# DanielBrosch/SDPSymmetryReduction.jl

Hardware: AMD Instinct MI355X
Metric: N x N SDP reductions/sec (admissible_subspace+blockDiagonalize) at N=4096 (higher is better)
Workload: dtype int8 square (int32 acc) + f64 eigen

## Files before the change

### include/sdpsr.h

```cpp
#ifndef SDPSR_H
#define SDPSR_H

#include <stddef.h>
#include <stdint.h>

#ifdef __cplusplus
extern "C" {
#endif

#define SDPSR_VERSION_MAJOR 0
#define SDPSR_VERSION_MINOR 5

typedef struct sdpsr_ctx sdpsr_ctx;
typedef struct sdpsr_problem sdpsr_problem;

typedef enum sdpsr_status {
    SDPSR_OK = 0,
    SDPSR_INVALID_DECOMPOSITION_FIELD = 1,
    SDPSR_NUMERICAL_INCONSISTENCY = 2,
    SDPSR_DIMENSION_MISMATCH = 3,
    SDPSR_LABEL_OVERFLOW = 4,
    SDPSR_BAD_ARGUMENT = 5,
    SDPSR_HIP_ERROR = 6,
    SDPSR_SOLVER_ERROR = 7,
    SDPSR_OUT_OF_MEMORY = 8,
    SDPSR_NOT_CONVERGED = 9,
    SDPSR_BAD_STATE = 10
} sdpsr_status;

typedef enum sdpsr_mem { SDPSR_MEM_HOST = 0, SDPSR_MEM_DEVICE = 1 } sdpsr_mem;

typedef enum sdpsr_square_mode {
    SDPSR_SQUARE_AUTO = 0,
    SDPSR_SQUARE_I8 = 1,
    SDPSR_SQUARE_F32 = 2,
    SDPSR_SQUARE_F64 = 3
} sdpsr_square_mode;

typedef enum sdpsr_round_mode {
    SDPSR_ROUND_NEAREST = 0,
    SDPSR_ROUND_TRUNC = 1
} sdpsr_round_mode;

enum {
    SDPSR_FLAG_SEPARATE_REFINEMENTS = 1u << 0,
    SDPSR_FLAG_FRESH_IRREDUCIBLE_ELEMENT = 1u << 1,
    SDPSR_FLAG_ALWAYS_REORTHOGONALIZE = 1u << 2,
    SDPSR_FLAG_REFINE_NO_FUSE = 1u << 3,
    SDPSR_FLAG_UNPACK_EVERY_STEP = 1u << 4,
    SDPSR_FLAG_SPMM_ONE_BY_ONE = 1u << 5,
    SDPSR_FLAG_SINGLE_COUPLING_ELEMENT = 1u << 6,
    SDPSR_FLAG_SMALL_EIGEN_ON_DEVICE = 1u << 7,
    SDPSR_FLAG_NO_GRAPH = 1u << 8,
    SDPSR_FLAG_NO_VERIFY_SHORTCUT = 1u << 9,
    SDPSR_FLAG_FULL_BASIS_IMAGE = 1u << 10,
    SDPSR_FLAG_ALWAYS_PROJECT = 1u << 11,
    SDPSR_FLAG_SYTRD_PANELS = 1u << 12,
    SDPSR_FLAG_COUPLING_ON_HOST = 1u << 13,
    SDPSR_FLAG_SYTRD_ONE_LAUNCH = 1u << 14,
    SDPSR_FLAG_WAIT_FOR_EVERY_VERDICT = 1u << 15,
    SDPSR_FLAG_WIDE_LOOP_LABELS = 1u << 16,
    SDPSR_FLAG_MODULE_SCRATCH_FILLS = 1u << 17,
    SDPSR_FLAG_SQUARE_EVERY_VERDICT = 1u << 18
};

typedef struct sdpsr_opts {
    uint32_t struct_size;
    int32_t square_mode;
    int32_t channels;
    int32_t max_iters;
    int32_t confirm_rounds;
    int32_t eig_driver;
    uint32_t flags;
    int32_t round_mode;
    int32_t basis_image_kernel;
    int32_t refine_path;
    int32_t label_bits;
    int32_t insert_wgs_per_cu;
    int32_t square_kernel;
    int32_t reserved[3];
} sdpsr_opts;

enum {
    SDPSR_T_TOTAL = 0,
    SDPSR_T_PROJECT = 1,
    SDPSR_T_SQUARE = 2,
    SDPSR_T_REFINE = 3,
    SDPSR_T_EIGEN = 4,
    SDPSR_T_ISO = 5,
    SDPSR_T_IRRED = 6,
    SDPSR_T_IMAGE = 7,
    SDPSR_T_COUNT = 8
};

int sdpsr_create(int device_id, uint64_t seed, const sdpsr_opts* opts, sdpsr_ctx** out);
void sdpsr_destroy(sdpsr_ctx* ctx);
const char* sdpsr_last_error(const sdpsr_ctx* ctx);
const char* sdpsr_status_string(int status);
int sdpsr_version(void);
int sdpsr_set_stream(sdpsr_ctx* ctx, void* hip_stream);
int sdpsr_synchronize(sdpsr_ctx* ctx);
int sdpsr_wait_stream(sdpsr_ctx* ctx, void* hip_stream);
int sdpsr_hint_symmetric_basis(sdpsr_ctx* ctx, int yes);
int sdpsr_set_seed(sdpsr_ctx* ctx, uint64_t seed);
int sdpsr_dimension_trajectory(sdpsr_ctx* ctx, int64_t* dims, int32_t capacity, int32_t* count);

int sdpsr_set_label_width(sdpsr_ctx* ctx, int bits);
int sdpsr_label_width(sdpsr_ctx* ctx);
int sdpsr_labels_convert(sdpsr_ctx* ctx, int64_t len, const void* in, int in_bits, void* out, int out_bits, int mem);

int sdpsr_partition_from_f64(sdpsr_ctx* ctx, int64_t len, const double* M,
                             uint32_t* labels, int64_t* nparts, int mem);
int sdpsr_partition_from_u32(sdpsr_ctx* ctx, int64_t len, const uint32_t* in,
                             uint32_t* labels, int64_t* nparts, int mem);
int sdpsr_partition_from_u64(sdpsr_ctx* ctx, int64_t len, const uint64_t* in,
                             uint32_t* labels, int64_t* nparts, int mem);
int sdpsr_refine(sdpsr_ctx* ctx, int64_t len, uint32_t* p1, int64_t* d1,
                 const uint32_t* p2, int64_t d2, int mem);
int sdpsr_partition_checksum(sdpsr_ctx* ctx, int64_t len, const uint32_t* labels, uint64_t* out, int mem);
int sdpsr_fill(sdpsr_ctx* ctx, int64_t len, const uint32_t* labels, const double* values,
               int64_t d, double* M, int mem);
int sdpsr_randomize(sdpsr_ctx* ctx, int64_t len, const uint32_t* labels, double* M, int mem);
int sdpsr_clamp_round(sdpsr_ctx* ctx, int64_t len, double* a, double atol, int mem);
int sdpsr_project_out(sdpsr_ctx* ctx, int64_t len, double* x, const double* U, int64_t r,
                      int mem);

int sdpsr_square_f64(sdpsr_ctx* ctx, int64_t n, const double* X, double* X2, int mem);
int sdpsr_square_f32(sdpsr_ctx* ctx, int64_t n, const float* X, float* X2, int mem);
int sdpsr_square_i8(sdpsr_ctx* ctx, int64_t n, const int8_t* X, int32_t* X2, int mem);
int sdpsr_square_i8_symmetric(sdpsr_ctx* ctx, int64_t n, int64_t batch, const int8_t* X, int32_t* X2, int mem);
int sdpsr_gemm_tn_f64(sdpsr_ctx* ctx, int64_t m, int64_t n, int64_t k, const double* A,
                      int64_t lda, const double* B, int64_t ldb, double* C, int64_t ldc,
                      int mem);

int sdpsr_admissible_subspace(sdpsr_ctx* ctx, int64_t n, const double* CL, const double* X0L,
                              const double* U, int64_t r, double atol, uint32_t* P_out,
                              int64_t* dim_out, int32_t* iters_out, double* phase_ms, int mem);
int sdpsr_admissible_subspace_dense(sdpsr_ctx* ctx, int64_t n, int64_t m, const double* C,
                                    const double* A, const double* b, double atol,
                                    uint32_t* P_out, int64_t* dim_out, int32_t* iters_out,
                                    double* phase_ms, int mem_out);

typedef enum sdpsr_setup_path {
    SDPSR_SETUP_NO_CONSTRAINTS = 0,
    SDPSR_SETUP_CHOLESKY_QR2 = 1,
    SDPSR_SETUP_MGS = 2
} sdpsr_setup_path;
int sdpsr_admissible_setup_csr(sdpsr_ctx* ctx, int64_t n, int64_t m, const int64_t* rowptr, const int64_t* colind,
                               const double* val, int index_base, const double* b, const double* C, double atol,
                               double* CL, double* X0L, double* U, int64_t* r_out, int* hint_out, int32_t* info_out,
                               int mem_out);
int sdpsr_admissible_subspace_csr(sdpsr_ctx* ctx, int64_t n, int64_t m, const int64_t* rowptr, const int64_t* colind,
                                  const double* val, int index_base, const double* b, const double* C, double atol,
                                  uint32_t* P_out, int64_t* dim_out, int32_t* iters_out, double* phase_ms, int mem_out);

int sdpsr_desymmetrize(sdpsr_ctx* ctx, int64_t n, uint32_t* P, int64_t* dim, int32_t* iters, int mem);

int sdpsr_reduce_constraints(sdpsr_ctx* ctx, int64_t len, const uint32_t* labels, int64_t d, int64_t m,
                             const double* A, double* out, int mem);
int sdpsr_reduce_constraints_csr(sdpsr_ctx* ctx, int64_t len, const uint32_t* labels, int64_t d, int64_t m,
                                 const int64_t* rowptr, const int64_t* colind, const double* val, int index_base,
                                 double* out, int mem);

typedef struct sdpsr_sparse sdpsr_sparse;
int sdpsr_sparse_create(sdpsr_ctx* ctx, int64_t len, int64_t m, int64_t nnz, const int64_t* rowptr, const int64_t* colind,
                        const double* val, int index_base, int mem, sdpsr_sparse** out);
int sdpsr_sparse_destroy(sdpsr_sparse* A);
int sdpsr_sparse_info(const sdpsr_sparse* A, int64_t* len, int64_t* m, int64_t* nnz_canonical, int* rows_symmetric);
int sdpsr_sparse_export(sdpsr_ctx* ctx, const sdpsr_sparse* A, int index_base, int64_t* rowptr, int64_t* colind, double* val,
                        int mem);
int sdpsr_admissible_setup_sparse(sdpsr_ctx* ctx, int64_t n, const sdpsr_sparse* A, const double* b, const double* C,
                                  double atol, double* CL, double* X0L, double* U, int64_t* r_out, int* hint_out,
                                  int32_t* info_out, int mem_out);
int sdpsr_admissible_subspace_sparse(sdpsr_ctx* ctx, int64_t n, const sdpsr_sparse* A, const double* b, const double* C,
                                     double atol, uint32_t* P_out, int64_t* dim_out, int32_t* iters_out, double* phase_ms,
                                     int mem_out);
int sdpsr_reduce_constraints_sparse(sdpsr_ctx* ctx, const sdpsr_sparse* A, const uint32_t* labels, int64_t d, double* out,
                                    int mem);

int sdpsr_compress_constraints(sdpsr_ctx* ctx, int64_t m, int64_t d, const double* newA, const double* b, double rtol,
                               double droptol, double* out, int64_t* rank_out, double* sv, int64_t* nnz_out,
                               int32_t* passes_out, int mem);

int sdpsr_block_diagonalize(sdpsr_ctx* ctx, int64_t n, const uint32_t* P, int64_t d,
                            double epsilon, int32_t* nblocks, int64_t* sum_sq, int64_t* sum_s,
                            double* phase_ms, int mem);
int sdpsr_block_sizes(sdpsr_ctx* ctx, int32_t* blk_sizes);
int sdpsr_q_hat(sdpsr_ctx* ctx, double* Q_hat, int mem);
int sdpsr_block_images(sdpsr_ctx* ctx, double* blks, double* Q_hat, double* phase_ms, int mem);
enum {
    SDPSR_BI_ROUTE_COMMUTATIVE = 1,
    SDPSR_BI_ROUTE_BLOCKS = 2,
    SDPSR_BI_ROUTE_TWO_STAGE = 3,
    SDPSR_BI_ROUTE_OUTER = 4,
    SDPSR_BI_ROUTE_CHUNK = 5,
    SDPSR_BI_ROUTE_REPAIRED = 0x100,
    SDPSR_BI_ROUTE_SHORTCUT_REFUSED = 0x200
};
int sdpsr_basis_image(sdpsr_ctx* ctx, int64_t n, const uint32_t* P, int64_t d, int32_t nblocks, const int32_t* blk_sizes,
                      const double* Q_hat, int64_t class_first, int64_t class_count, double atol, double* blks, int32_t* route,
                      double* phase_ms, int mem);
int sdpsr_jordan_reduce(sdpsr_ctx* ctx, int64_t n, const double* CL, const double* X0L, const double* U, int64_t r,
                        double atol, double epsilon, uint32_t* P_out, int64_t* dim_out, int32_t* iters_out,
                        int32_t* nblocks, int64_t* sum_sq, int64_t* sum_s, double* blks, int64_t blks_capacity,
                        double* Q_hat, int64_t qhat_capacity, double* phase_ms, int mem);

int sdpsr_jordan_reduce_batch(sdpsr_ctx* ctx, int32_t R, const uint64_t* seeds, int64_t n, const double* CL, const double* X0L,
                              const double* U, int64_t r, double atol, double epsilon, uint32_t* const* P_out, int64_t* dim_out,
                              int32_t* iters_out, int32_t* nblocks, int64_t* sum_sq, int64_t* sum_s, double* const* blks,
                              const int64_t* blks_capacity, int32_t* status, int mem);
int sdpsr_batch_block_sizes(sdpsr_ctx* ctx, int32_t restart, int32_t* blk_sizes);

int sdpsr_problem_create(sdpsr_ctx* ctx, int64_t n, const double* CL, const double* X0L, const double* U, int64_t r, int hint,
                         int mem, sdpsr_problem** out);
int sdpsr_problem_destroy(sdpsr_problem* problem);
int sdpsr_problem_reduce(sdpsr_ctx* ctx, const sdpsr_problem* problem, double atol, double epsilon, uint32_t* P_out,
// ... 64 lines not shown
```

### include/sdpsr_prof.h

```cpp
#ifndef SDPSR_PROF_H
#define SDPSR_PROF_H

#include "sdpsr.h"

#ifdef __cplusplus
extern "C" {
#endif

int sdpsr_profile_kernel(sdpsr_ctx* ctx, int kind, int64_t n, int64_t aux, int reps,
                         double* ms_per_launch);
int sdpsr_profile_clock(sdpsr_ctx* ctx, int kind, int64_t n, int64_t aux, int reps, double* out);
int sdpsr_profile_host_waits(sdpsr_ctx* ctx, uint64_t* out);
int sdpsr_profile_loop_counts(sdpsr_ctx* ctx, int32_t restart, uint64_t* out);
int sdpsr_profile_band_chase(sdpsr_ctx* ctx, int64_t n, int b, const double* A_host, double* d_host, double* e_host, double* out);
int sdpsr_profile_band_reduce(sdpsr_ctx* ctx, int64_t n, int b, double* A_host, double* out);
int sdpsr_profile_sytrd_graphs(sdpsr_ctx* ctx, double* out);
int sdpsr_profile_gather_packed(sdpsr_ctx* ctx, int64_t n, int T, int64_t d, uint64_t key, const uint32_t* Lp_host, const uint32_t* Lfull_host,
                                int8_t* X_plain, int8_t* X_writing, int8_t* X_full, uint32_t* L_inout, int64_t guard);
int sdpsr_profile_verify(sdpsr_ctx* ctx, int64_t n, int T, int64_t d, int mode, const uint32_t* Lp_host, const uint32_t* first_idx_host,
                         const int32_t* C_host, const double* U_host, double coef, uint64_t key, double atol, uint32_t* out);
int sdpsr_profile_basis_constant(sdpsr_ctx* ctx, int64_t n, int r, int64_t d, const uint32_t* Lp_host, const uint32_t* first_idx_host,
                                 const double* U_host, double atol, uint32_t* out);
int sdpsr_profile_verify_pair(sdpsr_ctx* ctx, int64_t n, int64_t d, const uint32_t* Lp_host, const uint32_t* first_idx_host,
                              const double* a_host, const double* b_host, uint32_t* out);
int sdpsr_profile_initial_guess(sdpsr_ctx* ctx, int32_t restart, uint64_t* out);
int sdpsr_profile_narrow_labels(sdpsr_ctx* ctx, int32_t restart, uint64_t* out);
int sdpsr_profile_gather_packed_w(sdpsr_ctx* ctx, int64_t n, int T, int64_t d, uint64_t key, int width, const uint32_t* Lp_host, int8_t* X_plain,
                                  int8_t* X_writing, uint32_t* L_inout, int64_t guard);
int sdpsr_profile_verify_w(sdpsr_ctx* ctx, int64_t n, int T, int64_t d, int r, int width, const uint32_t* Lp_host, const uint32_t* first_idx_host,
                           const int32_t* C_host, const double* U_host, const double* coef_host, uint64_t key, double atol, uint32_t* out);
int sdpsr_profile_verify_pair_w(sdpsr_ctx* ctx, int64_t n, int64_t d, int width, const uint32_t* Lp_host, const uint32_t* first_idx_host,
                                const double* a_host, const double* b_host, uint32_t* out);
int sdpsr_profile_proj_coef_lower(sdpsr_ctx* ctx, int64_t n, int64_t r, uint64_t key, int width, const uint32_t* Lp_host, const double* U_host,
                                  double* partial_out, double* coef_out);
int sdpsr_profile_refine_source(sdpsr_ctx* ctx, int kind, int what, int64_t n, int64_t ld, int T, int r, int packed, int lab_packed, uint64_t key,
                                double atol, const double* a_host, const double* b_host, const double* U_host, const double* coef_host,
                                const void* C_host, uint32_t* L_inout, uint32_t* Lnew_inout, int64_t guard, int64_t prev_classes, int sym,
                                uint64_t* sig_out, int64_t* nparts, uint32_t* first_out, int32_t* report);
int sdpsr_profile_square_checks(sdpsr_ctx* ctx, int32_t restart, uint64_t* out);
int sdpsr_profile_square_check(sdpsr_ctx* ctx, int64_t n, int64_t d, int G, int T, const uint64_t* keys, int width, int write_full,
                               const uint32_t* Lp_host, const uint32_t* first_idx_host, uint8_t* ws_inout, uint64_t* layout,
                               uint32_t* verdicts_out, uint32_t* L_inout, int64_t guard);


int sdpsr_profile_gram(sdpsr_ctx* ctx, int mode, int64_t k, int64_t ma, int64_t nb, int64_t lda, int64_t ldb, int64_t mp, int64_t np,
                       const double* A_host, const double* B_host, double* C_inout, double* pinned_inout, int64_t guard, int32_t* report);
int sdpsr_profile_tall_times_small(sdpsr_ctx* ctx, int64_t n, int64_t ldi, int64_t kk, int64_t lds, int64_t ncols, double alpha, double beta,
                                   int64_t ldo, const double* In_host, const double* S_host, double* out_inout, int64_t guard);
int sdpsr_profile_label_product(sdpsr_ctx* ctx, int64_t n, int64_t d, int G, int64_t w, int64_t ldw, int64_t ldy, const uint64_t* keys,
                                const uint32_t* L_host, const double* W_host, double* Y_inout, int64_t guard, int32_t* report);
int sdpsr_profile_label_product_pair(sdpsr_ctx* ctx, int64_t n, int64_t d, int64_t w, int64_t ldw, int64_t ldy, const uint64_t* keys,
                                     const uint32_t* L_host, const double* W_host, double* Y0_inout, double* Y1_inout, int64_t guard,
                                     int32_t* report);
int sdpsr_profile_class_sums2(sdpsr_ctx* ctx, int64_t n, int64_t d, uint32_t first, int plain, const uint32_t* L_host, const double* X_host,
                              double* Y_inout, int64_t guard, int32_t* report);
int sdpsr_profile_class_sums(sdpsr_ctx* ctx, int64_t n, int64_t d, int64_t ldo, const uint32_t* L_host, const double* x_host,
                             double* out_inout, int64_t guard, int32_t* report);
int sdpsr_profile_symmetrize(sdpsr_ctx* ctx, int64_t m, int64_t ld, double* B_inout, int64_t guard);
int sdpsr_profile_extract_symmetric(sdpsr_ctx* ctx, int64_t m, int64_t mp, int64_t lds, const double* src_host, double* dst_inout, int64_t guard);
int sdpsr_profile_normalize_columns(sdpsr_ctx* ctx, int64_t n, int64_t ldx, int64_t hstride, int64_t nruns, const double* X_host,
                                    double* H_inout, double* norm_inout, int64_t guard);
int sdpsr_profile_random_vector(sdpsr_ctx* ctx, int64_t n, uint64_t key, double* x_inout, int64_t guard);


int sdpsr_profile_poison_scratch(sdpsr_ctx* ctx);
int sdpsr_profile_stacked_in_place(sdpsr_ctx* ctx, int64_t n, int64_t ldi, int64_t kk, int64_t lds, int64_t ncols, int64_t w, int64_t mcols,
                                   double* M_inout, const double* S_host, int64_t guard, int32_t* report);
int sdpsr_profile_lift(sdpsr_ctx* ctx, int64_t n, int64_t ldi, int64_t kk, int64_t lds, int64_t S1, double atol, const double* In_host,
                       const double* S_host, double* Qcm_inout, double* Qrm_inout, int64_t guard);
int sdpsr_profile_seed_vector(sdpsr_ctx* ctx, int64_t n, uint64_t key, double* x_inout, double* h_inout, double* norm_inout, int64_t guard);
int sdpsr_profile_qrm_current(sdpsr_ctx* ctx, int32_t* current);


int sdpsr_profile_cx_gather_herm(sdpsr_ctx* ctx, int64_t n, const uint32_t* L_host, uint64_t key, double* Hr_inout, double* Hi_inout, int64_t guard);
int sdpsr_profile_cx_heev(sdpsr_ctx* ctx, int route, int64_t n, const double* Hr_host, const double* Hi_host, double atol, double* w_inout,
                          double* Vr_inout, double* Vi_inout, int64_t guard, int32_t* info_out);
int sdpsr_profile_cx_block_norms(sdpsr_ctx* ctx, int route, int64_t n, const double* Hr_host, const double* Hi_host, const double* Vr_host,
                                 const double* Vi_host, const int32_t* space_of, int32_t neig, double* norms_inout, int64_t guard);
int sdpsr_profile_cx_irreducible(sdpsr_ctx* ctx, int route, int64_t n, int64_t vcols, const double* Hr_host, const double* Hi_host,
                                 const double* Vr_host, const double* Vi_host, const int32_t* desc, int32_t ncols, double atol,
                                 double* Qhat_inout, int64_t guard);


int sdpsr_profile_dense_block_norms(sdpsr_ctx* ctx, int route, int64_t n, int64_t ld, const double* A_host, const double* Q_host,
                                    const int32_t* space_of, int32_t neig, double* norms_inout, double* M_inout, double* T_inout, int64_t guard);
int sdpsr_profile_dense_cluster_norms(sdpsr_ctx* ctx, int64_t n, int64_t ld, const double* A_host, const double* Q_host,
                                      const double* evals_host, double atol, const int32_t* einfo, void* pack_inout, double* T_inout, int64_t guard);
int sdpsr_profile_dense_classes(sdpsr_ctx* ctx, int32_t neig, double* norms_inout, const int32_t* dims_host, double atol, uint64_t* stat_out,
                                double* edges_out, double* thr_out, uint64_t* bits_inout, int32_t* kpart_out, int64_t guard);
int sdpsr_profile_dense_irreducible(sdpsr_ctx* ctx, int route, int64_t n, int64_t ldq, int64_t vcols, const double* Q_host, const double* Bf_host,
                                    int64_t nf, const int32_t* desc, int32_t npairs, double* Qhat_inout, int64_t ncols, int64_t guard,
                                    int32_t* report);
int sdpsr_profile_copy_cols(sdpsr_ctx* ctx, int64_t n, int64_t count, const int32_t* src_cols, const int32_t* dst_cols, const double* src_host,
                            int64_t ld_src, int64_t scols, double* dst_inout, int64_t ld_dst, int64_t dcols, int64_t guard);
int sdpsr_profile_clamptol(sdpsr_ctx* ctx, int64_t len, double* a_inout, double atol, int64_t guard);


int sdpsr_profile_sytrd(sdpsr_ctx* ctx, int64_t n, int64_t ld, double* A_inout, double* d_inout, double* e_inout, double* tau_inout,
                        int64_t guard);
int sdpsr_profile_backtransform(sdpsr_ctx* ctx, int64_t n, int64_t ld, const double* A_host, const double* tau_host, double* Z_inout,
                                int64_t guard);
int sdpsr_profile_stedc(sdpsr_ctx* ctx, int64_t n, int64_t ld, const double* d_host, const double* e_host, double* w_inout, double* Z_inout,
                        int64_t guard);

#ifdef __cplusplus
}
#endif
#endif
```

### sdpsymmetryreduction.jl_amd/_lib.py

```python
from __future__ import annotations

import ctypes as C
import os
import re

import numpy as np

_HERE = os.path.dirname(os.path.abspath(__file__))
LIB_PATH = os.path.join(_HERE, "libsdpsr_hip.so")
PROF_LIB_PATH = os.path.join(_HERE, "libsdpsr_prof.so")
HEADER_PATH = os.path.join(os.path.dirname(_HERE), "include", "sdpsr.h")
PROF_HEADER_PATH = os.path.join(os.path.dirname(_HERE), "include", "sdpsr_prof.h")

MEM_HOST, MEM_DEVICE = 0, 1
SQUARE_AUTO, SQUARE_I8, SQUARE_F32, SQUARE_F64 = 0, 1, 2, 3
T_TOTAL, T_PROJECT, T_SQUARE, T_REFINE, T_EIGEN, T_ISO, T_IRRED, T_IMAGE, T_COUNT = range(9)
ROUND_NEAREST, ROUND_TRUNC = 0, 1
SETUP_NO_CONSTRAINTS, SETUP_CHOLESKY_QR2, SETUP_MGS = 0, 1, 2
FLAG_SEPARATE_REFINEMENTS = 1 << 0
FLAG_FRESH_IRREDUCIBLE_ELEMENT = 1 << 1
FLAG_ALWAYS_REORTHOGONALIZE = 1 << 2
FLAG_REFINE_NO_FUSE = 1 << 3
FLAG_UNPACK_EVERY_STEP = 1 << 4
FLAG_SPMM_ONE_BY_ONE = 1 << 5
FLAG_SINGLE_COUPLING_ELEMENT = 1 << 6
FLAG_SMALL_EIGEN_ON_DEVICE = 1 << 7
FLAG_NO_GRAPH = 1 << 8
FLAG_NO_VERIFY_SHORTCUT = 1 << 9
FLAG_FULL_BASIS_IMAGE = 1 << 10
FLAG_ALWAYS_PROJECT = 1 << 11
FLAG_SYTRD_PANELS = 1 << 12
FLAG_COUPLING_ON_HOST = 1 << 13
FLAG_SYTRD_ONE_LAUNCH = 1 << 14
FLAG_WAIT_FOR_EVERY_VERDICT = 1 << 15
FLAG_WIDE_LOOP_LABELS = 1 << 16
FLAG_MODULE_SCRATCH_FILLS = 1 << 17
FLAG_SQUARE_EVERY_VERDICT = 1 << 18
BASIS_IMAGE_KERNELS = {"auto": 0, "two_stage": 1, "outer": 2, "chunk": 3}
BI_ROUTE_COMMUTATIVE, BI_ROUTE_BLOCKS, BI_ROUTE_TWO_STAGE, BI_ROUTE_OUTER, BI_ROUTE_CHUNK = 1, 2, 3, 4, 5
BI_ROUTE_REPAIRED, BI_ROUTE_SHORTCUT_REFUSED = 0x100, 0x200
TRI_UPPER, TRI_FULL = 0, 1
REFINE_PATHS = {"auto": 0, "hash": 1, "sort": 2, "bucket": 3, "no_mid": 4, "mid_no_first": 6}

LABEL_DTYPES = {8: np.dtype(np.uint8), 16: np.dtype(np.uint16), 32: np.dtype(np.uint32)}


def label_dtype(bits):
    try:
        return LABEL_DTYPES[int(bits)]
    except KeyError:
        raise ValueError(f"label width must be 8, 16 or 32, not {bits!r}") from None


STATUS = {
    0: "OK", 1: "INVALID_DECOMPOSITION_FIELD", 2: "NUMERICAL_INCONSISTENCY", 3: "DIMENSION_MISMATCH",
    4: "LABEL_OVERFLOW", 5: "BAD_ARGUMENT", 6: "HIP_ERROR", 7: "SOLVER_ERROR", 8: "OUT_OF_MEMORY",
    9: "NOT_CONVERGED", 10: "BAD_STATE",
}


class Opts(C.Structure):
    _fields_ = [
        ("struct_size", C.c_uint32),
        ("square_mode", C.c_int32),
        ("channels", C.c_int32),
        ("max_iters", C.c_int32),
        ("confirm_rounds", C.c_int32),
        ("eig_driver", C.c_int32),
        ("flags", C.c_uint32),
        ("round_mode", C.c_int32),
        ("basis_image_kernel", C.c_int32),
        ("refine_path", C.c_int32),
        ("label_bits", C.c_int32),
        ("insert_wgs_per_cu", C.c_int32),
        ("square_kernel", C.c_int32),
        ("reserved", C.c_int32 * 3),
    ]


def declared_symbols(header_path=HEADER_PATH):
    txt = open(header_path).read()
    txt = re.sub(r"/\*.*?\*/", "", txt, flags=re.S)
    return sorted(set(re.findall(r"\b(sdpsr_[a-z0-9_]+)\s*\(", txt)))


_lib = None


def load_library():
    global _lib
    if _lib is not None:
        return _lib
    if not os.path.exists(LIB_PATH):
        raise RuntimeError(
            f"{LIB_PATH} is missing: build it with `make -C sdpsymmetryreduction.jl_amd/csrc` "
            "(there is no CPU fallback for the HIP path)")
    try:
        import torch
    except ImportError:
        pass
    lib = C.CDLL(LIB_PATH)
    vp, i64, i32, dbl = C.c_void_p, C.c_int64, C.c_int32, C.c_double
    pi64, pi32 = C.POINTER(C.c_int64), C.POINTER(C.c_int32)
    sigs = {
        "sdpsr_create": (C.c_int, [C.c_int, C.c_uint64, C.POINTER(Opts), C.POINTER(vp)]),
        "sdpsr_destroy": (None, [vp]),
        "sdpsr_last_error": (C.c_char_p, [vp]),
        "sdpsr_status_string": (C.c_char_p, [C.c_int]),
        "sdpsr_version": (C.c_int, []),
        "sdpsr_set_stream": (C.c_int, [vp, vp]),
        "sdpsr_synchronize": (C.c_int, [vp]),
        "sdpsr_wait_stream": (C.c_int, [vp, vp]),
        "sdpsr_set_seed": (C.c_int, [vp, C.c_uint64]),
        "sdpsr_dimension_trajectory": (C.c_int, [vp, vp, i32, pi32]),
        "sdpsr_partition_from_f64": (C.c_int, [vp, i64, vp, vp, pi64, C.c_int]),
        "sdpsr_partition_from_u32": (C.c_int, [vp, i64, vp, vp, pi64, C.c_int]),
        "sdpsr_partition_from_u64": (C.c_int, [vp, i64, vp, vp, pi64, C.c_int]),
        "sdpsr_refine": (C.c_int, [vp, i64, vp, pi64, vp, i64, C.c_int]),
        "sdpsr_partition_checksum": (C.c_int, [vp, i64, vp, vp, C.c_int]),
        "sdpsr_fill": (C.c_int, [vp, i64, vp, vp, i64, vp, C.c_int]),
        "sdpsr_randomize": (C.c_int, [vp, i64, vp, vp, C.c_int]),
        "sdpsr_clamp_round": (C.c_int, [vp, i64, vp, dbl, C.c_int]),
        "sdpsr_project_out": (C.c_int, [vp, i64, vp, vp, i64, C.c_int]),
        "sdpsr_square_f64": (C.c_int, [vp, i64, vp, vp, C.c_int]),
        "sdpsr_square_f32": (C.c_int, [vp, i64, vp, vp, C.c_int]),
        "sdpsr_square_i8": (C.c_int, [vp, i64, vp, vp, C.c_int]),
        "sdpsr_square_i8_symmetric": (C.c_int, [vp, i64, i64, vp, vp, C.c_int]),
        "sdpsr_gemm_tn_f64": (C.c_int, [vp, i64, i64, i64, vp, i64, vp, i64, vp, i64, C.c_int]),
        "sdpsr_admissible_subspace": (C.c_int, [vp, i64, vp, vp, vp, i64, dbl, vp, pi64, pi32, vp, C.c_int]),
        "sdpsr_admissible_subspace_dense": (C.c_int, [vp, i64, i64, vp, vp, vp, dbl, vp, pi64, pi32, vp, C.c_int]),
        "sdpsr_admissible_setup_csr": (C.c_int, [vp, i64, i64, vp, vp, vp, C.c_int, vp, vp, dbl, vp, vp, vp, pi64, C.POINTER(C.c_int),
                                                 pi32, C.c_int]),
        "sdpsr_admissible_subspace_csr": (C.c_int, [vp, i64, i64, vp, vp, vp, C.c_int, vp, vp, dbl, vp, pi64, pi32, vp, C.c_int]),
        "sdpsr_jordan_reduce": (C.c_int, [vp, i64, vp, vp, vp, i64, dbl, dbl, vp, pi64, pi32, pi32, pi64, pi64, vp, i64, vp, i64, vp, C.c_int]),
        "sdpsr_jordan_reduce_batch": (C.c_int, [vp, C.c_int32, vp, i64, vp, vp, vp, i64, dbl, dbl, vp, pi64, pi32, pi32, pi64, pi64, vp, vp, pi32,
                                                C.c_int]),
        "sdpsr_problem_create": (C.c_int, [vp, i64, vp, vp, vp, i64, C.c_int, C.c_int, C.POINTER(vp)]),
        "sdpsr_problem_destroy": (C.c_int, [vp]),
        "sdpsr_problem_reduce": (C.c_int, [vp, vp, dbl, dbl, vp, pi64, pi32, pi32, pi64, pi64, vp, i64, vp, i64, vp, C.c_int]),
        "sdpsr_problem_reduce_batch": (C.c_int, [vp, vp, C.c_int32, vp, dbl, dbl, vp, pi64, pi32, pi32, pi64, pi64, vp, vp, pi32, C.c_int]),
        "sdpsr_batch_block_sizes": (C.c_int, [vp, C.c_int32, vp]),
        "sdpsr_transfer_bytes": (C.c_int, [vp, C.POINTER(C.c_uint64), C.POINTER(C.c_uint64)]),
        "sdpsr_reduce_constraints": (C.c_int, [vp, i64, vp, i64, i64, vp, vp, C.c_int]),
        "sdpsr_reduce_constraints_csr": (C.c_int, [vp, i64, vp, i64, i64, vp, vp, vp, C.c_int, vp, C.c_int]),
        "sdpsr_sparse_create": (C.c_int, [vp, i64, i64, i64, vp, vp, vp, C.c_int, C.c_int, C.POINTER(vp)]),
        "sdpsr_sparse_destroy": (C.c_int, [vp]),
        "sdpsr_sparse_info": (C.c_int, [vp, pi64, pi64, pi64, C.POINTER(C.c_int)]),
        "sdpsr_sparse_export": (C.c_int, [vp, vp, C.c_int, vp, vp, vp, C.c_int]),
        "sdpsr_admissible_setup_sparse": (C.c_int, [vp, i64, vp, vp, vp, dbl, vp, vp, vp, pi64, C.POINTER(C.c_int), pi32, C.c_int]),
        "sdpsr_admissible_subspace_sparse": (C.c_int, [vp, i64, vp, vp, vp, dbl, vp, pi64, pi32, vp, C.c_int]),
        "sdpsr_reduce_constraints_sparse": (C.c_int, [vp, vp, vp, i64, vp, C.c_int]),
        "sdpsr_compress_constraints": (C.c_int, [vp, i64, i64, vp, vp, dbl, dbl, vp, pi64, vp, pi64, pi32, C.c_int]),
        "sdpsr_desymmetrize": (C.c_int, [vp, i64, vp, pi64, pi32, C.c_int]),
        "sdpsr_block_diagonalize": (C.c_int, [vp, i64, vp, i64, dbl, pi32, pi64, pi64, vp, C.c_int]),
        "sdpsr_block_sizes": (C.c_int, [vp, vp]),
        "sdpsr_q_hat": (C.c_int, [vp, vp, C.c_int]),
        "sdpsr_block_images": (C.c_int, [vp, vp, vp, vp, C.c_int]),
        "sdpsr_basis_image": (C.c_int, [vp, i64, vp, i64, i32, vp, vp, i64, i64, dbl, vp, pi32, vp, C.c_int]),
        "sdpsr_eigen_decomposition": (C.c_int, [vp, i64, vp, i64, dbl, pi32, pi32, C.c_int]),
        "sdpsr_block_diagonalize_complex": (C.c_int, [vp, i64, vp, i64, dbl, vp, pi64, pi32, pi64, pi64, C.c_int]),
        "sdpsr_block_sizes_complex": (C.c_int, [vp, vp]),
        "sdpsr_block_images_complex": (C.c_int, [vp, vp, vp, C.c_int]),
        "sdpsr_basis_image_complex": (C.c_int, [vp, i64, vp, i64, i32, vp, vp, i64, i64, dbl, vp, pi32, vp, C.c_int]),
        "sdpsr_block_images_sparse": (C.c_int, [vp, i32, vp, i64, vp, C.c_int, C.c_int, dbl, C.c_int, i64, vp, vp, vp, vp, vp, pi64,
                                                C.POINTER(C.c_double), C.c_int]),
        "sdpsr_eigen_decomposition_batched": (C.c_int, [vp, i64, vp, i64, dbl, i64, vp, vp, vp, vp, C.c_int]),
        "sdpsr_syev_f64": (C.c_int, [vp, i64, vp, vp, vp, C.c_int]),
        "sdpsr_hint_symmetric_basis": (C.c_int, [vp, C.c_int]),
        "sdpsr_set_label_width": (C.c_int, [vp, C.c_int]),
        "sdpsr_label_width": (C.c_int, [vp]),
        "sdpsr_labels_convert": (C.c_int, [vp, i64, vp, C.c_int, vp, C.c_int, C.c_int]),
        "sdpsr_meet_keys": (C.c_int, [vp, i32, vp, vp, i64, i64, vp, C.c_int]),
        "sdpsr_agree_partitions": (C.c_int, [vp, vp, i32, vp, vp, i64, pi64, pi32, C.c_int]),
        "sdpsr_agree_block_diagonalization": (C.c_int, [vp, vp, i32, i32, vp, pi32, pi32, vp, i32]),
        "sdpsr_comm_unique_id": (C.c_int, [vp]),
        "sdpsr_comm_create": (C.c_int, [vp, i32, i32, vp, C.POINTER(vp)]),
        "sdpsr_comm_rank": (C.c_int, [vp]),
        "sdpsr_comm_world": (C.c_int, [vp]),
        "sdpsr_comm_broadcast": (C.c_int, [vp, vp, vp, i64, i32, C.c_int]),
        "sdpsr_comm_destroy": (C.c_int, [vp]),
        "sdpsr_blockop_create": (C.c_int, [vp, i32, vp, i64, i64, vp, vp, vp, vp, vp, C.c_int, C.c_int, C.c_int, C.POINTER(vp)]),
        "sdpsr_blockop_destroy": (C.c_int, [vp]),
        "sdpsr_blockop_info": (C.c_int, [vp, pi64, pi32, pi64, pi64]),
        "sdpsr_blockop_apply": (C.c_int, [vp, vp, vp, vp, C.c_int]),
        "sdpsr_blockop_adjoint": (C.c_int, [vp, vp, vp, vp, C.c_int]),
        "sdpsr_blocks_syev": (C.c_int, [vp, i32, vp, vp, vp, vp, C.c_int]),
    }
    missing = [s for s in declared_symbols() if not hasattr(lib, s)]
    if missing:
        raise RuntimeError(f"libsdpsr_hip.so lacks symbols declared in include/sdpsr.h: {missing}")
    for name, (res, args) in sigs.items():
        fn = getattr(lib, name)
        fn.restype = res
        fn.argtypes = args
    _lib = lib
    return lib


_prof = None


def load_prof_library():
    global _prof
    if _prof is not None:
        return _prof
    load_library()
    if not os.path.exists(PROF_LIB_PATH):
        raise RuntimeError(f"{PROF_LIB_PATH} is missing: build it with `make -C sdpsymmetryreduction.jl_amd/csrc`")
    lib = C.CDLL(PROF_LIB_PATH)
    vp, i64 = C.c_void_p, C.c_int64
    for name in ("sdpsr_profile_kernel", "sdpsr_profile_clock"):
        fn = getattr(lib, name)
        fn.restype = C.c_int
        fn.argtypes = [vp, C.c_int, i64, i64, C.c_int, C.POINTER(C.c_double)]
    lib.sdpsr_profile_band_chase.restype = C.c_int
    lib.sdpsr_profile_band_chase.argtypes = [vp, i64, C.c_int, vp, vp, vp, C.POINTER(C.c_double)]
    lib.sdpsr_profile_band_reduce.restype = C.c_int
    lib.sdpsr_profile_band_reduce.argtypes = [vp, i64, C.c_int, vp, C.POINTER(C.c_double)]
    lib.sdpsr_profile_host_waits.restype = C.c_int
    lib.sdpsr_profile_host_waits.argtypes = [vp, C.POINTER(C.c_uint64)]
    lib.sdpsr_profile_loop_counts.restype = C.c_int
    lib.sdpsr_profile_loop_counts.argtypes = [vp, C.c_int32, C.POINTER(C.c_uint64)]
    lib.sdpsr_profile_sytrd_graphs.restype = C.c_int
    lib.sdpsr_profile_sytrd_graphs.argtypes = [vp, C.POINTER(C.c_double)]
    lib.sdpsr_profile_gather_packed.restype = C.c_int
    lib.sdpsr_profile_gather_packed.argtypes = [vp, i64, C.c_int, i64, C.c_uint64, vp, vp, vp, vp, vp, vp, i64]
    lib.sdpsr_profile_verify.restype = C.c_int
    lib.sdpsr_profile_verify.argtypes = [vp, i64, C.c_int, i64, C.c_int, vp, vp, vp, vp, C.c_double, C.c_uint64, C.c_double,
                                         C.POINTER(C.c_uint32)]
    lib.sdpsr_profile_basis_constant.restype = C.c_int
    lib.sdpsr_profile_basis_constant.argtypes = [vp, i64, C.c_int, i64, vp, vp, vp, C.c_double, C.POINTER(C.c_uint32)]
    lib.sdpsr_profile_verify_pair.restype = C.c_int
    lib.sdpsr_profile_verify_pair.argtypes = [vp, i64, i64, vp, vp, vp, vp, C.POINTER(C.c_uint32)]
    lib.sdpsr_profile_initial_guess.restype = C.c_int
    lib.sdpsr_profile_initial_guess.argtypes = [vp, C.c_int32, C.POINTER(C.c_uint64)]
    lib.sdpsr_profile_narrow_labels.restype = C.c_int
    lib.sdpsr_profile_narrow_labels.argtypes = [vp, C.c_int32, C.POINTER(C.c_uint64)]
    lib.sdpsr_profile_gather_packed_w.restype = C.c_int
    lib.sdpsr_profile_gather_packed_w.argtypes = [vp, i64, C.c_int, i64, C.c_uint64, C.c_int, vp, vp, vp, vp, i64]
    lib.sdpsr_profile_verify_w.restype = C.c_int
    lib.sdpsr_profile_verify_w.argtypes = [vp, i64, C.c_int, i64, C.c_int, C.c_int, vp, vp, vp, vp, vp, C.c_uint64, C.c_double, C.POINTER(C.c_uint32)]
    lib.sdpsr_profile_verify_pair_w.restype = C.c_int
    lib.sdpsr_profile_verify_pair_w.argtypes = [vp, i64, i64, C.c_int, vp, vp, vp, vp, C.POINTER(C.c_uint32)]
    lib.sdpsr_profile_square_checks.restype = C.c_int
    lib.sdpsr_profile_square_checks.argtypes = [vp, C.c_int32, C.POINTER(C.c_uint64)]
    lib.sdpsr_profile_square_check.restype = C.c_int
    lib.sdpsr_profile_square_check.argtypes = [vp, i64, i64, C.c_int, C.c_int, vp, C.c_int, C.c_int, vp, vp, vp, vp, vp, vp, i64]
    lib.sdpsr_profile_proj_coef_lower.restype = C.c_int
    lib.sdpsr_profile_proj_coef_lower.argtypes = [vp, i64, i64, C.c_uint64, C.c_int, vp, vp, vp, vp]
    lib.sdpsr_profile_refine_source.restype = C.c_int
    lib.sdpsr_profile_refine_source.argtypes = [vp, C.c_int, C.c_int, i64, i64, C.c_int, C.c_int, C.c_int, C.c_int, C.c_uint64, C.c_double,
                                                vp, vp, vp, vp, vp, vp, vp, i64, i64, C.c_int, vp, C.POINTER(i64), vp, C.POINTER(C.c_int32)]
    f64, rep = C.c_double, C.POINTER(C.c_int32)
    lib.sdpsr_profile_gram.restype = C.c_int
    lib.sdpsr_profile_gram.argtypes = [vp, C.c_int, i64, i64, i64, i64, i64, i64, i64, vp, vp, vp, vp, i64, rep]
    lib.sdpsr_profile_tall_times_small.restype = C.c_int
    lib.sdpsr_profile_tall_times_small.argtypes = [vp, i64, i64, i64, i64, i64, f64, f64, i64, vp, vp, vp, i64]
    lib.sdpsr_profile_label_product.restype = C.c_int
    lib.sdpsr_profile_label_product.argtypes = [vp, i64, i64, C.c_int, i64, i64, i64, vp, vp, vp, vp, i64, rep]
    lib.sdpsr_profile_label_product_pair.restype = C.c_int
    lib.sdpsr_profile_label_product_pair.argtypes = [vp, i64, i64, i64, i64, i64, vp, vp, vp, vp, vp, i64, rep]
    lib.sdpsr_profile_class_sums2.restype = C.c_int
    lib.sdpsr_profile_class_sums2.argtypes = [vp, i64, i64, C.c_uint32, C.c_int, vp, vp, vp, i64, rep]
    lib.sdpsr_profile_class_sums.restype = C.c_int
    lib.sdpsr_profile_class_sums.argtypes = [vp, i64, i64, i64, vp, vp, vp, i64, rep]
    lib.sdpsr_profile_symmetrize.restype = C.c_int
    lib.sdpsr_profile_symmetrize.argtypes = [vp, i64, i64, vp, i64]
    lib.sdpsr_profile_extract_symmetric.restype = C.c_int
    lib.sdpsr_profile_extract_symmetric.argtypes = [vp, i64, i64, i64, vp, vp, i64]
    lib.sdpsr_profile_normalize_columns.restype = C.c_int
    lib.sdpsr_profile_normalize_columns.argtypes = [vp, i64, i64, i64, i64, vp, vp, vp, i64]
    lib.sdpsr_profile_random_vector.restype = C.c_int
    lib.sdpsr_profile_random_vector.argtypes = [vp, i64, C.c_uint64, vp, i64]
    lib.sdpsr_profile_poison_scratch.restype = C.c_int
    lib.sdpsr_profile_poison_scratch.argtypes = [vp]
    lib.sdpsr_profile_stacked_in_place.restype = C.c_int
    lib.sdpsr_profile_stacked_in_place.argtypes = [vp, i64, i64, i64, i64, i64, i64, i64, vp, vp, i64, rep]
    lib.sdpsr_profile_lift.restype = C.c_int
    lib.sdpsr_profile_lift.argtypes = [vp, i64, i64, i64, i64, i64, f64, vp, vp, vp, vp, i64]
    lib.sdpsr_profile_seed_vector.restype = C.c_int
    lib.sdpsr_profile_seed_vector.argtypes = [vp, i64, C.c_uint64, vp, vp, vp, i64]
    lib.sdpsr_profile_qrm_current.restype = C.c_int
    lib.sdpsr_profile_qrm_current.argtypes = [vp, rep]
    lib.sdpsr_profile_cx_gather_herm.restype = C.c_int
    lib.sdpsr_profile_cx_gather_herm.argtypes = [vp, i64, vp, C.c_uint64, vp, vp, i64]
    lib.sdpsr_profile_cx_heev.restype = C.c_int
    lib.sdpsr_profile_cx_heev.argtypes = [vp, C.c_int, i64, vp, vp, f64, vp, vp, vp, i64, rep]
    lib.sdpsr_profile_cx_block_norms.restype = C.c_int
    lib.sdpsr_profile_cx_block_norms.argtypes = [vp, C.c_int, i64, vp, vp, vp, vp, vp, C.c_int32, vp, i64]
    lib.sdpsr_profile_cx_irreducible.restype = C.c_int
    lib.sdpsr_profile_cx_irreducible.argtypes = [vp, C.c_int, i64, i64, vp, vp, vp, vp, vp, C.c_int32, f64, vp, i64]
    lib.sdpsr_profile_dense_block_norms.restype = C.c_int
    lib.sdpsr_profile_dense_block_norms.argtypes = [vp, C.c_int, i64, i64, vp, vp, vp, C.c_int32, vp, vp, vp, i64]
    lib.sdpsr_profile_dense_cluster_norms.restype = C.c_int
    lib.sdpsr_profile_dense_cluster_norms.argtypes = [vp, i64, i64, vp, vp, vp, f64, vp, vp, vp, i64]
    lib.sdpsr_profile_dense_classes.restype = C.c_int
    lib.sdpsr_profile_dense_classes.argtypes = [vp, C.c_int32, vp, vp, f64, vp, vp, vp, vp, vp, i64]
    lib.sdpsr_profile_dense_irreducible.restype = C.c_int
    lib.sdpsr_profile_dense_irreducible.argtypes = [vp, C.c_int, i64, i64, i64, vp, vp, i64, vp, C.c_int32, vp, i64, i64, rep]
    lib.sdpsr_profile_copy_cols.restype = C.c_int
    lib.sdpsr_profile_copy_cols.argtypes = [vp, i64, i64, vp, vp, vp, i64, i64, vp, i64, i64, i64]
    lib.sdpsr_profile_clamptol.restype = C.c_int
    lib.sdpsr_profile_clamptol.argtypes = [vp, i64, vp, f64, i64]
    lib.sdpsr_profile_sytrd.restype = C.c_int
    lib.sdpsr_profile_sytrd.argtypes = [vp, i64, i64, vp, vp, vp, vp, i64]
    lib.sdpsr_profile_backtransform.restype = C.c_int
    lib.sdpsr_profile_backtransform.argtypes = [vp, i64, i64, vp, vp, vp, i64]
    lib.sdpsr_profile_stedc.restype = C.c_int
    lib.sdpsr_profile_stedc.argtypes = [vp, i64, i64, vp, vp, vp, vp, i64]
    _prof = lib
    return lib
```

### sdpsymmetryreduction.jl_amd/csrc/compress.cpp

```cpp
#include <algorithm>
#include <cmath>
#include <cstdio>
#include <cstring>
#include <functional>

#include "host_internal.h"
#include "module_select.h"

using namespace sdpsr;

namespace {

struct Rider { double *dBs, *gps; bool have_t; };

struct Module {
    sdpsr_ctx* c;
    int64_t n, ld, d;
    const uint32_t* L;
    int wmax;
    int64_t wcap, ycap, wtot;
    double *W = nullptr, *T = nullptr, *zy = nullptr, *dout = nullptr, *Cc = nullptr, *dSm = nullptr, *Q1 = nullptr;
    int w = 1;
    std::vector<double> hG;
    int64_t saved_ld = 0;
    bool first_product_intact = false;
    bool have_saved = false;
    bool spec_b2 = false;
    bool sym_pre = false, sym_trusted = false, sym_checked = false;
    bool forked = false;
    bool lean = false;
    int live = 0;
    bool parent_form() const { return (c->opts.flags & SDPSR_FLAG_MODULE_SCRATCH_FILLS) != 0; }
    int restore_fills();

    bool fused_product(int wcols) const { return wcols <= 64 && d <= 4000; }
    bool small_on_host() const { return w <= 64 && !(c->opts.flags & SDPSR_FLAG_SMALL_EIGEN_ON_DEVICE) && (c->opts.eig_driver == 0 || c->opts.eig_driver >= 4); }
    size_t spec_b2_offset() const { return ((size_t)round_up(2 * w, 128) * (size_t)round_up(w, 128) * 8 + 255) & ~size_t(255); }
    double* spec_b2_pinned() const { return (double*)((char*)c->pinned + spec_b2_offset()); }

    int setup();
    int seed_basis();
    int apply_generic(int wcols, double* dst);
    int ortho_step(int mc, double tol, bool take_ref, const Rider* rider, Selection& sel);
    int apply_stacked(int mc, const Selection& sel);
    int absorb(int m, const Rider* rider, int& got);
    int class_sum_round();
    int growth_round(int& got);
    int grow(PhaseTimer& tm);
    int small_host_tail(PhaseTimer& tm, double atol, std::vector<int32_t>& sizes, int64_t& S1, int64_t& S, std::vector<double>& Qs);
    int make_element(double* dst);
    int prefetch_element(double* dst);
    int device_tail(PhaseTimer& tm, double atol, EigInfo& info, std::vector<int32_t>& sizes, int64_t& S1, int64_t& S);
    int lift(PhaseTimer& tm, const double* Qs_host, int64_t S1, double atol);
};

int Module::setup() {
    uint32_t* flag = (uint32_t*)ctx_buf(c, "bd_flag", 64);
    W = (double*)ctx_buf(c, "cm_w", (size_t)ld * wtot * 8);
    T = (double*)ctx_buf(c, "cm_t", (size_t)ld * wcap * 8);
    zy = (double*)ctx_buf(c, "cm_zy", (size_t)ld * 2 * 8);
    dout = (double*)ctx_buf(c, "cm_out", 64);
    if (!flag || !W || !T || !zy || !dout) return SDPSR_OUT_OF_MEMORY;
    if (!c->pinned_small) return SDPSR_OUT_OF_MEMORY;
    sym_pre = c->bd_sym_epoch != 0 && c->bd_sym_labels == L;
    sym_trusted = c->bd_trusted_symmetric == L;
    c->pinned_small[0] = 0;
    if (!sym_trusted) {
        if (!sym_pre) launch_check_symmetric(c->stream, n, L, flag);
        HIP_TRY(c, hipMemcpyAsync(c->pinned_small, sym_pre ? (const uint32_t*)ctx_buf(c, "bd_symflag", 64) : flag, 4,
                                  hipMemcpyDeviceToHost, c->stream));
    }
    sym_checked = sym_trusted;
    dbg_mark(c, "compressed: buffers + symmetric check done");
    return SDPSR_OK;
}

int Module::restore_fills() {
    if (!lean) return SDPSR_OK;
    lean = false;
    HIP_TRY(c, hipMemsetAsync(W + (size_t)(w + live) * ld, 0, (size_t)ld * (wtot - w - live) * 8, c->stream));
    HIP_TRY(c, hipMemsetAsync(Q1, 0, (size_t)ld * ycap * 8, c->stream));
    return SDPSR_OK;
}

int Module::seed_basis() {
    lean = !parent_form() && small_on_host();
    if (lean) launch_pad_rows(c->stream, n, ld, wtot, W);
    else HIP_TRY(c, hipMemsetAsync(W, 0, (size_t)ld * wtot * 8, c->stream));
    if (parent_form()) {
        launch_random_vector(c->stream, n, next_key(c), zy);
        launch_normalize_columns(c->stream, n, ld, W, 0, zy, ld, 1, dout);
    } else {
        launch_seed_vector(c->stream, n, next_key(c), zy, W, dout);
    }
    Cc = (double*)ctx_buf(c, "cm_c", (size_t)(wcap + ycap + 128) * ycap * 8);
    dSm = (double*)ctx_buf(c, "cm_sm", (size_t)(wcap + ycap) * ycap * 8);
    Q1 = (double*)ctx_buf(c, "cm_q1", (size_t)ld * ycap * 8);
    if (!Cc || !dSm || !Q1) return SDPSR_OUT_OF_MEMORY;
    if (!lean) HIP_TRY(c, hipMemsetAsync(Q1, 0, (size_t)ld * ycap * 8, c->stream));
    return SDPSR_OK;
}

int Module::apply_generic(int wcols, double* dst) {
    const uint64_t key = next_key(c);
    if (fused_product(wcols)) {
        double* part = (double*)ctx_buf(c, "cm_part", label_spmm_pair_partial_doubles(n) * 8);
        if (!part) return SDPSR_OUT_OF_MEMORY;
        if (launch_label_spmm(c->stream, n, L, key, d, W, ld, wcols, part, dst, ld)) return SDPSR_OK;
    }
    { int e0 = restore_fills(); if (e0) return e0; }
    double* Afull = (double*)ctx_buf(c, "cm_a", (size_t)ld * ld * 8);
    const int64_t wcp = round_up(wcols, 128);
    double* tmpo = (double*)ctx_buf(c, "cm_tmpo", (size_t)ld * wcp * 8);
    if (!Afull || !tmpo) return SDPSR_OUT_OF_MEMORY;
    launch_gather_f64_padded(c->stream, n, ld, L, key, Afull);
    int e3 = gemm_tn_splitk(c, ld, wcp, ld, Afull, ld, W, ld, tmpo, ld);
    if (e3) return e3;
    HIP_TRY(c, hipMemcpyAsync(dst, tmpo, (size_t)ld * wcols * 8, hipMemcpyDeviceToDevice, c->stream));
    return SDPSR_OK;
}

int Module::ortho_step(int mc, double tol, bool take_ref, const Rider* rider, Selection& sel) {
    const int64_t ap = round_up(w + mc, 128), mp = round_up(mc, 128);
    double* hpin = (double*)ctx_pinned(c, (size_t)ap * mp * 8);
    bool host_filled = false;
    const bool ride = take_ref && hpin && deferred_tail_pending(c) && small_on_host() && gram_tn_is_skinny(w + mc, mc);
    if (!ride) flush_deferred_tail(c);
    if (lean && !gram_tn_is_skinny(w + mc, mc)) {
        const int e0 = restore_fills();
        if (e0) return e0;
    }
    int st = hpin ? gram_tn(c, w + mc, mc, ld, W, ld, W + (size_t)w * ld, ld, Cc, ap, mp, hpin, &host_filled) : SDPSR_OUT_OF_MEMORY;
    if (st) return st;
    if (rider && (rider->have_t || apply_generic(w, T) == SDPSR_OK)) {
        launch_gram_small(c->stream, n, w, w, W, ld, T, ld, rider->gps, rider->dBs, w, w, w, spec_b2_pinned());
        spec_b2 = true;
    }
    hG.resize((size_t)ap * mp);
    if (host_filled && ride) {
        uint32_t* stamp = c->pinned_small + PINNED_SMALL_GRAM_STAMP.first;
        const uint32_t seq = ++c->report_seq ? c->report_seq : ++c->report_seq;
        *(volatile uint32_t*)stamp = 0;
        launch_report_stamp(c->stream, stamp, seq);
        flush_deferred_tail(c, 1);
        if (ctx_wait_word(c, c->stream, stamp, seq) != hipSuccess) return ctx_fail(c, SDPSR_HIP_ERROR, "report wait (module growth)");
        memcpy(hG.data(), hpin, (size_t)ap * mc * 8);
    } else if (host_filled) {
        if (ctx_sync_stream(c, c->stream) != hipSuccess) return ctx_fail(c, SDPSR_HIP_ERROR, "hipStreamSynchronize (module growth)");
        memcpy(hG.data(), hpin, (size_t)ap * mc * 8);
    } else {
        st = d2h_sync(c, hG.data(), Cc, (size_t)ap * mc * 8);
        if (st) return st;
    }
    if (!sym_checked) {
        sym_checked = true;
        if (sym_pre ? c->pinned_small[0] == c->bd_sym_epoch : c->pinned_small[0] != 0)
            return ctx_fail(c, SDPSR_INVALID_DECOMPOSITION_FIELD,
                            "partition is not symmetric: decomposition over Float64 requested but the generic element has a complex spectrum");
    }
    sel = select_directions(hG.data(), ap, w, mc, tol, take_ref);
    return SDPSR_OK;
}

int Module::apply_stacked(int mc, const Selection& sel) {
    int e2 = h2d_sync(c, dSm, sel.coef.data(), (size_t)(w + mc) * sel.rank * 8);
    if (e2) return e2;
    double* V = W + (size_t)w * ld;
    const bool in_place = !parent_form() && launch_tall_times_small_rows(c->stream, n, ld, W, w + mc, dSm, w + mc, sel.rank, 1.0, 0.0, V, ld);
    if (!in_place) {
        live = mc;
        e2 = restore_fills();
        if (e2) return e2;
        launch_tall_times_small(c->stream, n, ld, W, w + mc, dSm, w + mc, sel.rank, 1.0, 0.0, Q1, ld);
        HIP_TRY(c, hipMemcpyAsync(V, Q1, (size_t)ld * sel.rank * 8, hipMemcpyDeviceToDevice, c->stream));
    }
    live = sel.rank;
    return SDPSR_OK;
}

int Module::absorb(int m, const Rider* rider, int& got) {
    got = 0;
    Selection s1, s2;
    int st = ortho_step(m, 1e-10, true, rider, s1);
    if (st) return st;
    if (dbg_on() && s1.rank > 0) fprintf(stderr, "[sdpsr] absorb(%d): rank %d, pivots %.3e .. %.3e (ratio %.1e)\n", m, s1.rank, s1.piv_max, s1.piv_min, s1.piv_max / s1.piv_min);
    first_product_intact = (s1.rank == 0);
    if (s1.rank == 0) return SDPSR_OK;
    if (w + s1.rank >= wmax) return driver_fallback(c, "module dimension exceeds " + std::to_string(wmax));
    st = apply_stacked(m, s1);
    if (st) return st;
    const double worst = std::max(s1.piv_max, s1.ref) / s1.piv_min;
    got = s1.rank;
    if (!(worst <= 1e3) || (c->opts.flags & SDPSR_FLAG_ALWAYS_REORTHOGONALIZE)) {
        st = ortho_step(s1.rank, 1e-6, false, nullptr, s2);
        got = s2.rank;
        if (st || got == 0) return st;
        st = apply_stacked(s1.rank, s2);
        if (st) return st;
    }
    w += got;
    live = 0;
    return SDPSR_OK;
}

int Module::class_sum_round() {
    if (!(class_sums_supports(n, d, ld) && basis_image_two_stage_fits(n, d, 1) && d <= ycap && d + 1 < wmax)) {
        flush_deferred_tail(c);
        return SDPSR_OK;
    }
    launch_class_sums(c->stream, n, d, L, W, W + (size_t)w * ld, ld);
    int got;
    live = (int)d;
    return absorb((int)d, nullptr, got);
}

int Module::growth_round(int& got) {
    const bool fused = fused_product(w);
    int G = (fused && w <= 16) ? 4 : 2;
    while (G > 2 && (int64_t)G * w > ycap) --G;
    if ((int64_t)G * w > ycap || w >= d) G = 1;
    const int m = G * w;
    double* Y = W + (size_t)w * ld;
    live = 0;
    if (lean && !(fused && small_on_host())) {
        const int e0 = restore_fills();
        if (e0) return e0;
    }
    if (!lean) HIP_TRY(c, hipMemsetAsync(Y, 0, (size_t)ld * round_up(m, 128) * 8, c->stream));
    bool batched = false;
    if (fused && G > 1 && G != 3 && G * w <= 64 && !(c->opts.flags & SDPSR_FLAG_SPMM_ONE_BY_ONE)) {
        double* part = (double*)ctx_buf(c, "cm_part", label_spmm_pair_partial_doubles(n) * 8);
        if (!part) return SDPSR_OUT_OF_MEMORY;
        uint64_t keys[4];
        const uint64_t save = c->stream_counter;
        for (int gidx = 0; gidx < G; ++gidx) keys[gidx] = next_key(c);
        batched = launch_label_spmm_multi(c->stream, n, L, keys, G, d, W, ld, w, part, Y, ld);
        if (!batched) c->stream_counter = save;
    }
    spec_b2 = false;
    Rider rider{};
    bool armed = false;
    if (G == 1 && small_on_host()) {
        char* pinb = (char*)ctx_pinned(c, spec_b2_offset() + (size_t)w * w * 8);
        rider.dBs = (double*)ctx_buf(c, "cm_bsmall", (size_t)64 * 64 * 8);
        rider.gps = (double*)ctx_buf(c, "gram_partials", gram_small_partial_doubles(n, 128, 128) * 8);
        armed = pinb && rider.dBs && rider.gps;
    }
    if (armed && fused && !(c->opts.flags & SDPSR_FLAG_SPMM_ONE_BY_ONE)) {
        double* part = (double*)ctx_buf(c, "cm_part", label_spmm_pair_partial_doubles(n) * 8);
        if (!part) return SDPSR_OUT_OF_MEMORY;
        uint64_t keys[2];
        const uint64_t save = c->stream_counter;
        keys[0] = next_key(c);
        keys[1] = next_key(c);
        rider.have_t = launch_label_spmm_pair(c->stream, n, L, keys, d, W, ld, w, part, Y, ld, T, ld);
        if (!rider.have_t) c->stream_counter = save;
    }
    for (int gidx = 0; gidx < G && !batched && !rider.have_t; ++gidx) {
        live = gidx * w;
        int e2 = apply_generic(w, Y + (size_t)gidx * w * ld);
        if (e2) return e2;
    }
    live = m;
    int st = absorb(m, armed ? &rider : nullptr, got);
    if (st) return st;
    if (got != 0) spec_b2 = false;
    if (got == 0) {
        saved_ld = round_up(w + m, 128);
        have_saved = first_product_intact;
    }
    return SDPSR_OK;
}

int Module::grow(PhaseTimer& tm) {
    PhaseScope phase{tm, SDPSR_T_EIGEN, true};
    int st = seed_basis(), got = 1;
    if (!st) st = class_sum_round();
    for (int round = 0; round < 40 && !st && got != 0; ++round) {
        if (round >= 1) flush_deferred_tail(c);
        st = growth_round(got);
    }
    flush_deferred_tail(c);
    if (st) return st;
    if (got != 0) return driver_fallback(c, "module growth did not close within 40 rounds");
    live = 0;
    if (!small_on_host()) {
        st = restore_fills();
        if (st) return st;
        HIP_TRY(c, hipMemsetAsync(W + (size_t)w * ld, 0, (size_t)ld * (wtot - w) * 8, c->stream));
    }
    return SDPSR_OK;
}

int Module::small_host_tail(PhaseTimer& tm, double atol, std::vector<int32_t>& sizes, int64_t& S1, int64_t& S, std::vector<double>& Qs) {
    PhaseScope phase{tm, SDPSR_T_ISO, false};
    const size_t bbytes = (size_t)w * w * 8;
    double* dB = (double*)ctx_buf(c, "cm_bsmall", bbytes);
    double* gp = (double*)ctx_buf(c, "gram_partials", gram_small_partial_doubles(n, w, w) * 8);
    double* pin = (double*)ctx_pinned(c, bbytes);
    if (!dB || !gp || !pin) return SDPSR_OUT_OF_MEMORY;
    auto enqueue_element = [&]() -> int {
        const int e2 = apply_generic(w, T);
        if (e2) return e2;
        launch_gram_small(c->stream, n, w, w, W, ld, T, ld, gp, dB, w, w, w, pin);
        return SDPSR_OK;
    };
    auto fetch = [&](double* dst) -> int {
        HIP_TRY(c, ctx_sync_stream(c, c->stream));
        symmetrize_copy(pin, w, w, dst);
        return SDPSR_OK;
    };
    std::vector<double> B1((size_t)w * w);
    if (have_saved) {
        symmetrize_copy(hG.data(), saved_ld, w, B1.data());
    } else {
        int e2 = enqueue_element();
        if (!e2) e2 = fetch(B1.data());
        if (e2) return e2;
    }
    bool spec_avail = spec_b2 && have_saved;
    bool pending = spec_avail ? false : enqueue_element() == SDPSR_OK;
    const std::function<int(double*)> next_element = [&](double* dst) -> int {
        if (spec_avail) {
            spec_avail = false;
            symmetrize_copy(spec_b2_pinned(), w, w, dst);
            return SDPSR_OK;
        }
        if (!pending) {
            const int e2 = enqueue_element();
            if (e2) return e2;
        }
        pending = false;
        return fetch(dst);
    };
    const int st = murota_small_host(c, w, B1.data(), next_element, atol, d, sizes, S1, S, Qs);
    if (pending) ctx_sync_stream(c, c->stream);
    phase.collect = st != 0;
    return st;
}

int Module::make_element(double* dst) {
    const int64_t wp = round_up(w, 128);
    if (have_saved) {
        have_saved = false;
        launch_extract_symmetric(c->stream, w, wp, Cc, saved_ld, dst);
        return SDPSR_OK;
    }
    HIP_TRY(c, hipMemsetAsync(T, 0, (size_t)ld * wp * 8, c->stream));
    { int e2 = apply_generic(w, T); if (e2) return e2; }
    gram_tn(c, w, w, ld, W, ld, T, ld, dst, wp, wp);
    launch_symmetrize(c->stream, w, wp, dst);
    return SDPSR_OK;
}

int Module::prefetch_element(double* dst) {
    if (!ctx_ensure_side(c)) return SDPSR_HIP_ERROR;
    if (have_saved) return SDPSR_BAD_STATE;
    hipStream_t main_stream = c->stream;
    if (!forked && hipEventRecord(c->ev_fork, main_stream) != hipSuccess) return SDPSR_HIP_ERROR;
    forked = false;
    if (hipStreamWaitEvent(c->side_stream, c->ev_fork, 0) != hipSuccess) return SDPSR_HIP_ERROR;
    c->stream = c->side_stream;
    c->main_shadow = main_stream;
    const int e2 = make_element(dst);
    const bool rec = hipEventRecord(c->ev_join, c->side_stream) == hipSuccess;
    c->stream = main_stream;
    c->main_shadow = nullptr;
    if (e2 || !rec) {
        ctx_sync_stream(c, c->side_stream);
        return e2 ? e2 : SDPSR_HIP_ERROR;
    }
    return SDPSR_OK;
}

int Module::device_tail(PhaseTimer& tm, double atol, EigInfo& info, std::vector<int32_t>& sizes, int64_t& S1, int64_t& S) {
    if (dbg_on()) fprintf(stderr, "[sdpsr] module compression: n=%lld dim(P)=%lld -> w=%d\n", (long long)n, (long long)d, w);
    dbg_mark(c, "compressed: module grown");
    ElemGen gen;
    gen.make = [this](double* dst) { return make_element(dst); };
    gen.prefetch = [this](double* dst) { return prefetch_element(dst); };
    gen.fork = [this]() -> int {
        forked = false;
        if (have_saved) return SDPSR_BAD_STATE;
        if (!ctx_ensure_side(c) || hipEventRecord(c->ev_fork, c->stream) != hipSuccess) return SDPSR_HIP_ERROR;
        forked = true;
        return SDPSR_OK;
    };
    gen.join = [this]() -> int {
        HIP_TRY(c, hipStreamWaitEvent(c->stream, c->ev_join, 0));
        return SDPSR_OK;
    };
    if (!ctx_buf(c, "bd_qhat", (size_t)n * wmax * 8)) return SDPSR_OUT_OF_MEMORY;
    int st = dense_diagonalize(c, w, nullptr, &gen, atol, info, sizes, S1, S, tm, d);
    if (st) return st;
    dbg_mark(c, "compressed: small dense diagonalize done");
    st = lift(tm, nullptr, S1, atol);
    if (st) return st;
    HIP_TRY(c, ctx_sync_stream(c, c->stream));
    HIP_TRY(c, hipGetLastError());
    dbg_mark(c, "compressed: lifted");
    return SDPSR_OK;
}

int Module::lift(PhaseTimer& tm, const double* Qs_host, int64_t S1, double atol) {
    PhaseScope phase{tm, SDPSR_T_IRRED, false};
    double* qs = (double*)ctx_buf(c, "cm_qsmall", (size_t)w * S1 * 8);
    double* Qhat = (double*)ctx_buf(c, "bd_qhat", (size_t)n * S1 * 8);
    if (!qs || !Qhat) return SDPSR_OUT_OF_MEMORY;
    if (Qs_host) {
        const int st = h2d_sync(c, qs, Qs_host, (size_t)w * S1 * 8);
        if (st) return st;
    } else {
        HIP_TRY(c, hipMemcpyAsync(qs, Qhat, (size_t)w * S1 * 8, hipMemcpyDeviceToDevice, c->stream));
    }
    if (!parent_form() && tall_times_small_rows_supports((int)S1)) {
        double* Qrm = (double*)ctx_buf(c, "bd_qrm", (size_t)n * S1 * 8);
        if (!Qrm) return SDPSR_OUT_OF_MEMORY;
        launch_lift_clamped(c->stream, n, ld, W, w, qs, w, (int)S1, atol, Qhat, Qrm);
        c->bd_qrm_current = true;
        return SDPSR_OK;
    }
    launch_tall_times_small(c->stream, n, ld, W, w, qs, w, (int)S1, 1.0, 0.0, Qhat, n);
    launch_clamptol(c->stream, n * S1, Qhat, atol);
    return SDPSR_OK;
}

}

namespace sdpsr {

int compressed_diagonalize(sdpsr_ctx* c, int64_t n, const uint32_t* L, int64_t d, double atol, EigInfo& info,
                           std::vector<int32_t>& sizes, int64_t& S1, int64_t& S, PhaseTimer& tm) {
    const int wmax = (int)std::min<int64_t>(std::min<int64_t>(n / 2, 500), 2 * d + 8);
    if (wmax < 2) return driver_fallback(c, "module too small to compress");
    const int64_t wcap = round_up(wmax + 2, 128), ycap = 2 * wcap;
    Module m{c, n, round_up(n, 128), d, L, wmax, wcap, ycap, wcap + ycap + 128};
    int st = m.setup();
    if (!st) st = m.grow(tm);
    if (st) return st;
    if (!m.small_on_host()) return m.device_tail(tm, atol, info, sizes, S1, S);
    std::vector<double> Qs;
    st = m.small_host_tail(tm, atol, sizes, S1, S, Qs);
    if (!st) st = m.lift(tm, Qs.data(), S1, atol);
    if (st) return st;
    HIP_TRY(c, hipGetLastError());
    dbg_mark(c, "compressed: small problem solved on the host, lift enqueued");
    return SDPSR_OK;
}

bool compression_eligible(const sdpsr_ctx* c, int64_t n, int64_t d) {
    if (c->opts.eig_driver == 6) return true;
    if (c->opts.eig_driver != 0) return false;
    return n >= 512 && 2 * d + 8 <= std::min<int64_t>(n / 2, 500);
}

}
```

### sdpsymmetryreduction.jl_amd/csrc/ctx.cpp

```cpp
#include <algorithm>
#include <cmath>
#include <complex>
#include <cstdio>
#include <cstdlib>
#include <cstring>
#include <chrono>
#include <functional>
#include <numeric>

#include "host_internal.h"

using namespace sdpsr;
int ctx_fail(sdpsr_ctx* c, int status, const std::string& msg) {
    if (c) c->err = std::string(sdpsr_status_string(status)) + ": " + msg;
    return status;
}

void* ctx_buf(sdpsr_ctx* c, const char* name, size_t bytes) {
    if (bytes == 0) bytes = 16;
    auto it = c->bufs.find(std::string_view(name));
    if (it != c->bufs.end() && it->second.bytes >= bytes) return it->second.p;
    DevBuf& b = it != c->bufs.end() ? it->second : c->bufs[std::string(name)];
    const std::string_view nm(name);
    if (nm == "adm_lpacked" || nm == "adm_lpacked8" || nm == "ref_first") c->initial_record = InitialRecord{};
    if (nm == "adm_symflag") c->symflag_zero = false;
    if (nm == "bd_qhat" || nm == "bd_qrm") c->bd_qrm_current = false;
    if (b.p) {
        ctx_sync_stream(c, c->stream);
        hipFree(b.p);
        b.p = nullptr;
        b.bytes = 0;
    }
    size_t want = bytes + (bytes >> 3);
    want = (want + 255) & ~size_t(255);
    if (hipMalloc(&b.p, want) != hipSuccess) {
        b.p = nullptr;
        if (hipMalloc(&b.p, bytes) != hipSuccess) {
            b.p = nullptr;
            ctx_fail(c, SDPSR_OUT_OF_MEMORY, std::string("hipMalloc ") + name + " " + std::to_string(bytes));
            return nullptr;
        }
        want = bytes;
    }
    b.bytes = want;
    return b.p;
}


namespace sdpsr {
void* ctx_pinned(sdpsr_ctx* c, size_t bytes) {
    if (c->pinned_bytes >= bytes) return c->pinned;
    ctx_sync_stream(c, c->stream);
    if (c->pinned) hipHostFree(c->pinned);
    c->pinned = nullptr;
    c->pinned_bytes = 0;
    size_t want = std::max<size_t>(bytes + bytes / 4, 1 << 16);
    if (hipHostMalloc(&c->pinned, want, hipHostMallocCoherent) != hipSuccess) {
        c->pinned = nullptr;
        return nullptr;
    }
    c->pinned_bytes = want;
    return c->pinned;
}

bool ctx_ensure_side(sdpsr_ctx* c) {
    if (!c->side_stream && hipStreamCreateWithFlags(&c->side_stream, hipStreamNonBlocking) != hipSuccess) {
        c->side_stream = nullptr;
        (void)hipGetLastError();
        return false;
    }
    hipEvent_t* evs[] = {&c->ev_fork, &c->ev_join, &c->ev_bt_fork, &c->ev_bt_join};
    for (hipEvent_t* e : evs)
        if (!*e && hipEventCreateWithFlags(e, hipEventDisableTiming) != hipSuccess) {
            *e = nullptr;
            (void)hipGetLastError();
            return false;
        }
    return true;
}

bool dbg_on() { return getenv("SDPSR_DEBUG") != nullptr; }
void dbg_mark(sdpsr_ctx* c, const char* what) {
    if (!dbg_on()) return;
    const double now = std::chrono::duration<double, std::milli>(std::chrono::steady_clock::now().time_since_epoch()).count();
    fprintf(stderr, "[sdpsr] +%8.3f ms  %s\n", c && c->dbg_last_ms > 0 ? now - c->dbg_last_ms : 0.0, what);
    if (c) c->dbg_last_ms = now;
}

int d2h_sync(sdpsr_ctx* c, void* host, const void* dev, size_t bytes) {
    void* p = ctx_pinned(c, bytes);
    if (!p) return ctx_fail(c, SDPSR_OUT_OF_MEMORY, "pinned staging");
    HIP_TRY(c, hipMemcpyAsync(p, dev, bytes, hipMemcpyDeviceToHost, c->stream));
    HIP_TRY(c, ctx_sync_stream(c, c->stream));
    c->d2h_bytes += bytes;
    memcpy(host, p, bytes);
    return SDPSR_OK;
}
constexpr size_t H2D_SLOT = 32 * 1024;
constexpr int H2D_SLOTS = 32;
int h2d_sync(sdpsr_ctx* c, void* dev, const void* host, size_t bytes) {
    c->h2d_bytes += bytes;
    if (bytes <= H2D_SLOT) {
        if (!c->h2d_ring && hipHostMalloc(&c->h2d_ring, H2D_SLOT * H2D_SLOTS, hipHostMallocDefault) != hipSuccess) {
            c->h2d_ring = nullptr;
            return ctx_fail(c, SDPSR_OUT_OF_MEMORY, "pinned upload ring");
        }
        if (c->h2d_ring_next == H2D_SLOTS) {
            HIP_TRY(c, ctx_sync_stream(c, c->stream));
            if (c->side_stream && c->side_stream != c->stream) HIP_TRY(c, ctx_sync_stream(c, c->side_stream));
            if (c->main_shadow && c->main_shadow != c->stream) HIP_TRY(c, ctx_sync_stream(c, c->main_shadow));
            c->h2d_ring_next = 0;
        }
        void* slot = (char*)c->h2d_ring + (size_t)c->h2d_ring_next++ * H2D_SLOT;
        memcpy(slot, host, bytes);
        HIP_TRY(c, hipMemcpyAsync(dev, slot, bytes, hipMemcpyHostToDevice, c->stream));
        return SDPSR_OK;
    }
    void* p = ctx_pinned(c, bytes);
    if (!p) return ctx_fail(c, SDPSR_OUT_OF_MEMORY, "pinned staging");
    memcpy(p, host, bytes);
    HIP_TRY(c, hipMemcpyAsync(dev, p, bytes, hipMemcpyHostToDevice, c->stream));
    HIP_TRY(c, ctx_sync_stream(c, c->stream));
    return SDPSR_OK;
}
double round_scale(const sdpsr_ctx* c, double atol) {
    const double sc = std::pow(10.0, std::floor(-std::log10(atol)));
    return c->opts.round_mode == SDPSR_ROUND_TRUNC ? -sc : sc;
}

bool label_overflows(const sdpsr_ctx* c, uint64_t value) {
    const int b = c->opts.label_bits;
    return b > 0 && b < 64 && value > ((uint64_t(1) << b) - 1);
}
int label_overflow_fail(sdpsr_ctx* c, const char* where, uint64_t value) {
    return ctx_fail(c, SDPSR_LABEL_OVERFLOW, std::string(where) + ": " + std::to_string(value) + " does not fit the " +
                                                 std::to_string(c->opts.label_bits) + "-bit label type (InexactError in the reference)");
}

uint64_t next_key(sdpsr_ctx* c) { return sdpsr_stream_key(c->seed, c->stream_counter++); }

int check_len(sdpsr_ctx* c, int64_t len) {
    if (len < 1 || len >= (int64_t)0xFFFFFFF0ll)
        return ctx_fail(c, SDPSR_BAD_ARGUMENT, "len out of range [1, 2^32-16)");
    return SDPSR_OK;
}

}

extern "C" {

const char* sdpsr_status_string(int s) {
    switch (s) {
        case SDPSR_OK: return "OK";
        case SDPSR_INVALID_DECOMPOSITION_FIELD: return "INVALID_DECOMPOSITION_FIELD";
        case SDPSR_NUMERICAL_INCONSISTENCY: return "NUMERICAL_INCONSISTENCY";
        case SDPSR_DIMENSION_MISMATCH: return "DIMENSION_MISMATCH";
        case SDPSR_LABEL_OVERFLOW: return "LABEL_OVERFLOW";
        case SDPSR_BAD_ARGUMENT: return "BAD_ARGUMENT";
        case SDPSR_HIP_ERROR: return "HIP_ERROR";
        case SDPSR_SOLVER_ERROR: return "SOLVER_ERROR";
        case SDPSR_OUT_OF_MEMORY: return "OUT_OF_MEMORY";
        case SDPSR_NOT_CONVERGED: return "NOT_CONVERGED";
        case SDPSR_BAD_STATE: return "BAD_STATE";
    }
    return "UNKNOWN";
}

int sdpsr_version(void) { return SDPSR_VERSION_MAJOR * 1000 + SDPSR_VERSION_MINOR; }

int sdpsr_create(int device_id, uint64_t seed, const sdpsr_opts* opts, sdpsr_ctx** out) {
    if (!out) return SDPSR_BAD_ARGUMENT;
    *out = nullptr;
    int ndev = 0;
    if (hipGetDeviceCount(&ndev) != hipSuccess || ndev <= 0) return SDPSR_HIP_ERROR;
    if (device_id < 0 || device_id >= ndev) return SDPSR_BAD_ARGUMENT;
    sdpsr_ctx* c = new sdpsr_ctx();
    c->device = device_id;
    c->seed = seed;
    if (opts) {
        size_t sz = std::min<size_t>(opts->struct_size ? opts->struct_size : sizeof(sdpsr_opts), sizeof(sdpsr_opts));
        memcpy(&c->opts, opts, sz);
    }
    c->opts.struct_size = sizeof(sdpsr_opts);
    if (c->opts.square_mode == SDPSR_SQUARE_AUTO) c->opts.square_mode = SDPSR_SQUARE_I8;
    if (c->opts.channels <= 0) {
        c->opts.channels = 2;
        if (c->opts.confirm_rounds < 1 && c->opts.square_mode != SDPSR_SQUARE_F64) c->opts.confirm_rounds = 1;
    }
    if (c->opts.channels > 8) c->opts.channels = 8;
    if (c->opts.confirm_rounds < 0) c->opts.confirm_rounds = 0;
    if (c->opts.round_mode != SDPSR_ROUND_NEAREST && c->opts.round_mode != SDPSR_ROUND_TRUNC) {
        delete c;
        return SDPSR_BAD_ARGUMENT;
    }
    if (c->opts.label_bits != 0 && c->opts.label_bits != 8 && c->opts.label_bits != 16 && c->opts.label_bits != 32) {
        delete c;
        return SDPSR_BAD_ARGUMENT;
    }
    if (c->opts.max_iters <= 0) c->opts.max_iters = 10000;
    DeviceGuard dg(device_id);
    if (hipStreamCreateWithFlags(&c->stream, hipStreamNonBlocking) != hipSuccess) {
        delete c;
        return SDPSR_HIP_ERROR;
    }
    c->own_stream = true;
    if (hipDeviceGetAttribute(&c->num_cus, hipDeviceAttributeMultiprocessorCount, device_id) != hipSuccess || c->num_cus < 1)
        c->num_cus = 256;
    bool attrs_ok = true;
    attrs_ok &= gemm_set_device_attributes();
    attrs_ok &= gemm_sym_set_device_attributes();
    attrs_ok &= refine_bucket_set_device_attributes();
    attrs_ok &= blockdiag_set_device_attributes();
    attrs_ok &= module_set_device_attributes();
    attrs_ok &= dense_setup_set_device_attributes();
    attrs_ok &= insert_array_pair_set_device_attributes();
    attrs_ok &= insert_proj_set_device_attributes();
    attrs_ok &= insert_chan_set_device_attributes();
    attrs_ok &= insert_joint_set_device_attributes();
    attrs_ok &= sytrd_set_device_attributes();
    attrs_ok &= small_syev_set_device_attributes();
    attrs_ok &= stedc_set_device_attributes();
    attrs_ok &= batched_set_device_attributes();
    attrs_ok &= backtransform_set_device_attributes();
    attrs_ok &= complex_set_device_attributes();
    if (hipGetLastError() != hipSuccess || !attrs_ok) {
        hipStreamDestroy(c->stream);
        delete c;
        return SDPSR_HIP_ERROR;
    }
    c->pinned_bytes = 1 << 16;
    if (hipHostMalloc((void**)&c->pinned_small, 256, hipHostMallocCoherent) != hipSuccess) c->pinned_small = nullptr;
    if (hipHostMalloc(&c->pinned, c->pinned_bytes, hipHostMallocCoherent) != hipSuccess) {
        hipStreamDestroy(c->stream);
        delete c;
        return SDPSR_OUT_OF_MEMORY;
    }
    *out = c;
    return SDPSR_OK;
}

void sdpsr_destroy(sdpsr_ctx* c) {
    if (!c) return;
    for (sdpsr_ctx* ch : c->batch_children) sdpsr_destroy(ch);
    c->batch_children.clear();
    DeviceGuard dg(c->device);
    ctx_sync_stream(c, c->stream);
    destroy_handle(c);
    sytrd_graph_cache_destroy(c->sytrd_graphs);
    for (auto& kv : c->bufs)
        if (kv.second.p) hipFree(kv.second.p);
    if (c->pinned) hipHostFree(c->pinned);
    if (c->h2d_ring) hipHostFree(c->h2d_ring);
    if (c->pinned_small) hipHostFree(c->pinned_small);
// ... 76 lines not shown
```

### sdpsymmetryreduction.jl_amd/csrc/loop.cpp

```cpp
#include <algorithm>
#include <cmath>

#include "host_internal.h"

using namespace sdpsr;

namespace {
class LoopLabels {
public:
    uint32_t* L = nullptr;
    uint32_t* Lp = nullptr;
    uint8_t* Lp8 = nullptr;
    int sym = 0;
    void init(sdpsr_ctx* ctx, int64_t order, uint32_t* symflag_dev, bool keep, bool early) { c = ctx, n = order, symflag = symflag_dev, keep_packed = keep, early_ok = early; }
    bool packed() const { return packed_valid; }
    const uint32_t* current(bool from_packed) const { return from_packed ? Lp : L; }
    void need_full() {
        if (!full_valid) launch_unpack_symmetric_labels(c->stream, n, Lp, L);
        full_valid = true;
    }
    uint32_t* full_from_gather() {
        if (full_valid || !packed_valid) return nullptr;
        full_valid = true;
        return L;
    }
    void packed_refined() { packed_valid = true, full_valid = false, narrow_valid = false; }
    void shadow_current() { narrow_valid = packed_valid && Lp8 != nullptr; }
    bool narrow() const { return narrow_valid; }
    const uint8_t* shadow(bool from_packed = true) const { return from_packed && packed_valid && narrow_valid ? Lp8 : nullptr; }
    int refine_packed(const SigSource& src, int64_t* d) {
        const int st = refine_signatures(c, n * (n + 1) / 2, src, Lp, d, 0, nullptr, nullptr, early_ok);
        packed_refined();
        if (!st && !keep_packed) need_full();
        return st;
    }
    int refine_full(const SigSource& src, int64_t* d, bool with_symmetry_verdict) {
        if (with_symmetry_verdict) c->symflag_zero = false;
        const int st = with_symmetry_verdict ? refine_signatures(c, n * n, src, L, d, n, symflag, &sym) : refine_signatures(c, n * n, src, L, d);
        full_valid = true, packed_valid = false, narrow_valid = false;
        return st;
    }
private:
    sdpsr_ctx* c = nullptr;
    int64_t n = 0;
    uint32_t* symflag = nullptr;
    bool keep_packed = false, early_ok = false, full_valid = true, packed_valid = false, narrow_valid = false;
};

bool another_confirm_round(bool refined, int& confirm_left, bool spec_confirmed = false) {
    if (refined || confirm_left <= 0) return false;
    --confirm_left;
    if (!spec_confirmed) return true;
    if (confirm_left == 0) return false;
    --confirm_left;
    return true;
}

struct Verdict {
    bool unchanged = false;
    bool spec_confirmed = false;
};

struct Loop {
    Loop(sdpsr_ctx* ctx, PhaseTimer& timer) : c(ctx), s(ctx->stream), tm(timer) {}
    sdpsr_ctx* c;
    hipStream_t s;
    PhaseTimer& tm;
    int64_t n, len, ld, r;
    double atol, scale;
    int mode, T, vmax = 0;
    bool int_mode, keep_packed, early_ok;
    const double* dU;
    uint64_t* sig;
    static constexpr int nblk = 2048;
    double *partial, *coef, *Y = nullptr;
    void *Xp = nullptr, *Cp = nullptr;
    uint32_t* symflag;
    const uint32_t* zero_flag;
    LoopLabels lab;
    int64_t current = 0;
    int it = 0, confirm_left = 0;
    uint64_t key = 0;
    bool packed_proj = false;
    bool proj_dead = false;
    bool basis_sym = false, probe_pending = false;
    SigSource proj_source(const uint32_t* labels, int packed, int lab_packed) {
        SigSource q;
        q.kind = SIG_PROJ, q.sig = sig, q.U = dU, q.coef = coef, q.r = (int)r, q.key = key, q.atol = atol, q.scale = scale, q.n = n;
        q.L = labels, q.packed = packed, q.lab_packed = lab_packed;
        return q;
    }
    SigSource chan_source(int kind, const uint32_t* labels, int packed, int lab_packed) {
        SigSource q;
        q.kind = kind, q.sig = sig, q.n = n, q.ld = ld, q.T = T, q.C = Cp;
        q.L = labels, q.packed = packed, q.lab_packed = lab_packed;
        return q;
    }
    SigSource joint_source(bool from_packed) {
        SigSource q = proj_source(lab.current(from_packed), 1, from_packed ? 1 : 0);
        q.kind = proj_dead ? SIG_CHAN_I32 : SIG_JOINT_I32, q.ld = ld, q.T = T, q.C = Cp;
        q.L8 = lab.shadow(from_packed);
        return q;
    }
    void launch_square(bool from_packed, uint64_t key, void* X, void* C, int64_t dim, bool write_full = false, bool gather_only = false) {
        if (from_packed) launch_gather_i8_sym_packed(s, n, ld, T, lab.Lp, key, (int8_t*)X, dim, write_full ? lab.full_from_gather() : nullptr, lab.shadow());
        else launch_gather_i8(s, n, ld, T, lab.L, key, (int8_t*)X, dim);
        if (gather_only) return;
        launch_gemm_tn_i8_sym(s, ld, ld, (const int8_t*)X, ld, (int32_t*)C, ld, T, ld * ld, ld * ld, zero_flag, c->num_cus, c->opts.square_kernel);
        ++c->squares_launched;
    }
    int check_projection_dead() {
        void* uref = ctx_buf(c, "adm_uref", uconst_ref_bytes(current, r));
        const uint32_t* first = (const uint32_t*)ctx_buf(c, "ref_first", (size_t)refine_first_cap() * 4);
        uint32_t* hv = pinned_report(c, PINNED_BASIS_CONSTANT);
        if (!uref || !first || !hv) return SDPSR_OUT_OF_MEMORY;
        if (launch_basis_constant_on_classes(s, n, r, dU, lab.Lp, current, first, atol, scale, uref, hv)) {
            HIP_TRY(c, ctx_sync_stream(c, s));
            HIP_TRY(c, hipGetLastError());
            proj_dead = hv[0] == 0;
        }
        return SDPSR_OK;
    }
    bool verify_applies(bool confirming, bool from_packed) const {
        return (it == 1 || confirming) && from_packed && c->first_idx_labels == lab.Lp && current >= 1 && current <= (int64_t)refine_first_cap() &&
               !(c->opts.flags & SDPSR_FLAG_NO_VERIFY_SHORTCUT);
    }
    bool guess_applies(bool confirming) const { return it == 1 && !confirming && confirm_left > 0 && c->predict_closed && c->predict_n == n && early_ok; }
    bool tail_applies(const SigSource& qj, bool confirming, bool from_packed) {
        if (!verify_applies(confirming, from_packed) || !guess_applies(confirming) || confirm_left != 1 || !c->allow_deferred_verdict || !c->pinned_small || tm.enabled) return false;
        SigSource q2 = qj;
        q2.kind = SIG_CHAN_I32;
        if (!verify_no_split_supports(qj, current) || !verify_no_split_supports(q2, current)) return false;
        return ctx_buf(c, "adm_vref", verify_ref_bytes(current)) && ctx_buf(c, "ref_first", (size_t)refine_first_cap() * 4) &&
               pinned_report(c, PINNED_VERIFY) && ctx_buf(c, "adm_xi8_spec", (size_t)T * ld * ld) &&
               ctx_buf(c, "adm_ci32_spec", (size_t)T * ld * ld * 4) && ctx_buf(c, "adm_vref2", verify_ref_bytes(current));
    }
    bool check_applies(bool confirming, bool from_packed) const {
        return guess_applies(confirming) && verify_applies(confirming, from_packed) && lab.sym && mode == SDPSR_SQUARE_I8 &&
               square_check_supports(n, current, 2, T) && !(c->opts.flags & SDPSR_FLAG_SQUARE_EVERY_VERDICT) &&
               (proj_dead || r == 0 || current <= (int64_t)verify_lds_cap());
    }
    int check_round(const SigSource& qj, uint64_t key2, Verdict* v) {
        SquareCheck q;
        q.n = n, q.d = current, q.G = 2, q.T = T;
        void* ws = ctx_buf(c, "adm_sqcheck", square_check_ws_bytes(n, current, 2, T));
        const uint32_t* first = (const uint32_t*)ctx_buf(c, "ref_first", (size_t)refine_first_cap() * 4);
        uint32_t* hv = pinned_report(c, PINNED_VERIFY);
        uint32_t* hv2 = pinned_report(c, PINNED_SPECULATIVE);
        if (!ws || !first || !hv || !hv2) return SDPSR_OUT_OF_MEMORY;
        const bool defer = c->allow_deferred_verdict && c->pinned_small != nullptr;
        if (defer) hv = c->pinned_small + PINNED_SMALL_DEFERRED_VERIFY.first, hv2 = c->pinned_small + PINNED_SMALL_DEFERRED_SPECULATIVE.first;
        square_check_ws_carve(q, ws);
        q.key[0] = key2, q.key[1] = next_key(c);
        q.Lp = lab.Lp, q.Lp8 = lab.shadow(), q.first_idx = first, q.Lfull = lab.full_from_gather();
        q.flag[0] = hv, q.flag[1] = hv2;
        *(volatile uint32_t*)hv = 0u;
        *(volatile uint32_t*)hv2 = 0u;
        launch_square_check_ref_and_pass(s, q);
        if (qj.kind == SIG_JOINT_I32 && r >= 1) launch_verify_projection(s, qj, current, first, hv);
        launch_square_check_verdict(s, q);
        c->squares_launched += 2, ++c->squares_speculative, ++c->square_checks;
        if (defer) {
            c->deferred_verdict = true;
            HIP_TRY(c, hipGetLastError());
            v->unchanged = v->spec_confirmed = true;
            return SDPSR_OK;
        }
        HIP_TRY(c, ctx_sync_stream(c, s));
        HIP_TRY(c, hipGetLastError());
        v->unchanged = hv[0] == 0;
        v->spec_confirmed = v->unchanged && hv2[0] == 0;
        if (!v->spec_confirmed) --c->stream_counter;
        if (!v->unchanged) {
            ++c->square_check_fallbacks;
            --c->squares_launched;
            launch_square(true, key2, Xp, Cp, current);
        }
        return SDPSR_OK;
    }
    int verify_round(const SigSource& qj, bool confirming, bool from_packed, bool tail, Verdict* v) {
        if (!verify_applies(confirming, from_packed)) return SDPSR_OK;
        SigSource qv = qj;
        if (confirming) qv.kind = SIG_CHAN_I32;
        void* vref = ctx_buf(c, "adm_vref", verify_ref_bytes(current));
        const uint32_t* first = (const uint32_t*)ctx_buf(c, "ref_first", (size_t)refine_first_cap() * 4);
        uint32_t* hv = pinned_report(c, PINNED_VERIFY);
        uint32_t* hv2 = pinned_report(c, PINNED_SPECULATIVE);
        if (!vref || !first || !hv) return SDPSR_OUT_OF_MEMORY;
        const bool guess = guess_applies(confirming);
        const bool defer = guess && c->allow_deferred_verdict && c->pinned_small != nullptr;
        if (defer) hv = c->pinned_small + PINNED_SMALL_DEFERRED_VERIFY.first, hv2 = c->pinned_small + PINNED_SMALL_DEFERRED_SPECULATIVE.first;
        if (tail) {
            int8_t* Xs = (int8_t*)ctx_buf(c, "adm_xi8_spec", (size_t)T * ld * ld);
            int32_t* Cs = (int32_t*)ctx_buf(c, "adm_ci32_spec", (size_t)T * ld * ld * 4);
            void* vref2 = ctx_buf(c, "adm_vref2", verify_ref_bytes(current));
            if (!Xs || !Cs || !vref2) return SDPSR_OUT_OF_MEMORY;
            launch_square(true, next_key(c), Xs, Cs, current, true, true);
            DeferredTail& t = c->deferred_tail;
            t.ld = ld, t.d = current, t.T = T, t.zero_flag = zero_flag, t.first = first;
            t.seg[0].X = (const int8_t*)Xp, t.seg[0].C = (int32_t*)Cp, t.seg[0].q = qv, t.seg[0].vref = vref, t.seg[0].flag = hv, t.seg[0].speculative = false;
            t.seg[1].X = Xs, t.seg[1].C = Cs, t.seg[1].q = qj, t.seg[1].vref = vref2, t.seg[1].flag = hv2, t.seg[1].speculative = true;
            t.seg[1].q.kind = SIG_CHAN_I32, t.seg[1].q.C = Cs;
            *(volatile uint32_t*)hv = DEFERRED_NEVER_RAN;
            *(volatile uint32_t*)hv2 = DEFERRED_NEVER_RAN;
            t.next = 0, t.count = DEFERRED_SEGMENTS;
            c->deferred_verdict = true;
            HIP_TRY(c, hipGetLastError());
            v->unchanged = v->spec_confirmed = true;
            return SDPSR_OK;
        }
        if (!launch_verify_no_split(s, qv, current, first, vref, hv)) return SDPSR_OK;
        bool spec = false;
        if (guess) {
            void* Xs = ctx_buf(c, "adm_xi8_spec", (size_t)T * ld * ld);
            void* Cs = ctx_buf(c, "adm_ci32_spec", (size_t)T * ld * ld * 4);
            void* vref2 = ctx_buf(c, "adm_vref2", verify_ref_bytes(current));
            if (Xs && Cs && vref2) {
                launch_square(true, next_key(c), Xs, Cs, current, true);
                ++c->squares_speculative;
                SigSource q2 = qj;
                q2.kind = SIG_CHAN_I32, q2.C = Cs;
                spec = launch_verify_no_split(s, q2, current, first, vref2, hv2);
            }
        }
        if (defer && spec) {
            c->deferred_verdict = true;
            HIP_TRY(c, hipGetLastError());
            v->unchanged = v->spec_confirmed = true;
        } else {
            HIP_TRY(c, ctx_sync_stream(c, s));
            HIP_TRY(c, hipGetLastError());
            v->unchanged = hv[0] == 0;
            v->spec_confirmed = spec && v->unchanged && hv2[0] == 0;
            if (spec && !v->spec_confirmed) --c->stream_counter;
        }
        return SDPSR_OK;
    }
    int joint_iteration(int64_t* d_out) {
        int st = SDPSR_OK;
        const bool jl = lab.packed();
        if (!jl) lab.need_full();
        if (!proj_dead && it >= 2 && it <= 4 && r >= 1 && jl && c->first_idx_labels == lab.Lp && current >= 1 &&
            current <= (int64_t)refine_first_cap() && !(c->opts.flags & SDPSR_FLAG_ALWAYS_PROJECT)) {
            st = check_projection_dead();
            if (st) return st;
        }
        if (!proj_dead) launch_proj_coef_lower(s, n, r, dU, lab.current(jl), jl ? 1 : 0, key, partial, nblk, coef, lab.shadow(jl));
        tm.end();
        int64_t dj = current;
        bool confirming = false;
        for (;;) {
            flush_deferred_tail(c);
            tm.begin(SDPSR_T_SQUARE);
            const uint64_t key2 = next_key(c);
            const bool jl2 = lab.packed();
            const SigSource qj = joint_source(jl2);
            const bool check = check_applies(confirming, jl2);
            const bool tail = !check && tail_applies(qj, confirming, jl2);
            if (!check) launch_square(jl2, key2, Xp, Cp, current, confirming && verify_applies(confirming, jl2), tail);
            tm.end();
            tm.begin(SDPSR_T_REFINE);
            Verdict v;
            st = check ? check_round(qj, key2, &v) : verify_round(qj, confirming, jl2, tail, &v);
            if (st) return st;
            if (v.unchanged) dj = current;
            else if (!(st = initial_guess_settled())) st = lab.refine_packed(qj, &dj);
            tm.end();
            if (st) return st;
            tm.collect();
            if (!another_confirm_round(dj != current, confirm_left, v.spec_confirmed)) break;
            confirming = true;
        }
        *d_out = dj;
        return SDPSR_OK;
    }
    int launch_separate_square(uint64_t key2, int64_t d1, int64_t d2, SigSource* qs) {
        const bool slab = keep_packed && lab.sym && lab.packed();
        if (!slab) lab.need_full();
        const uint32_t* L = lab.L;
        *qs = chan_source(SIG_ARRAY, lab.current(slab), lab.sym, slab ? 1 : 0);
        const uint32_t* Lleft = L;
        if (int_mode && !lab.sym) {
            uint32_t* Lt = (uint32_t*)ctx_buf(c, "des_lt", len * 4);
            if (!Lt) return SDPSR_OUT_OF_MEMORY;
            launch_transpose_labels(s, n, L, Lt);
            Lleft = Lt;
        }
        switch (mode) {
        case SDPSR_SQUARE_I8:
            qs->kind = SIG_CHAN_I32;
            if (lab.sym) return launch_square(slab, key2, Xp, Cp, d2), SDPSR_OK;
            launch_gather_i8(s, n, ld, T, L, key2, (int8_t*)Xp, d2);
            if (int8_t* Xl = (int8_t*)ctx_buf(c, "des_yi8", (size_t)T * ld * ld)) {
                launch_gather_i8(s, n, ld, T, Lleft, key2, Xl, d2);
                launch_gemm_tn_i8(s, ld, ld, ld, Xl, ld, (const int8_t*)Xp, ld, (int32_t*)Cp, ld, T, ld * ld, ld * ld, ld * ld);
                break;
            }
            return SDPSR_OUT_OF_MEMORY;
        case SDPSR_SQUARE_F32:
            qs->kind = SIG_CHAN_F32;
            launch_gather_f32(s, n, ld, T, vmax, L, key2, (float*)Xp);
            if (!lab.sym) {
                float* Xl = (float*)ctx_buf(c, "adm_xlf32", (size_t)T * ld * ld * 4);
                if (!Xl) return SDPSR_OUT_OF_MEMORY;
                launch_gather_f32(s, n, ld, T, vmax, Lleft, key2, Xl);
                launch_gemm_tn_f32(s, ld, ld, ld, Xl, ld, (const float*)Xp, ld, (float*)Cp, ld, T, ld * ld, ld * ld, ld * ld);
            } else {
                launch_gemm_tn_f32_sym(s, ld, ld, (const float*)Xp, ld, (float*)Cp, ld, T, ld * ld, ld * ld, zero_flag);
            }
            break;
        default:
            if (d1 != current || confirm_left != c->opts.confirm_rounds) launch_gather_f64_padded(s, n, ld, L, key2, (double*)Xp);
            else launch_pad_copy(s, n, ld, Y, Xp, 8);
            launch_gemm_tn_f64(s, ld, ld, ld, (const double*)Xp, ld, (const double*)Xp, ld, (double*)Cp, ld, 1, 0, 0, 0);
            launch_sig_f64_rounded(s, n, ld, L, (const double*)Cp, atol, scale, sig);
        }
        ++c->squares_launched;
        return SDPSR_OK;
    }
    int separate_iteration(int64_t* d_out) {
        int st = SDPSR_OK;
        double* probe_host = nullptr;
        const bool plab = packed_proj && lab.packed();
        if (!plab) lab.need_full();
        if (packed_proj) {
            launch_proj_coef_lower(s, n, r, dU, lab.current(plab), plab ? 1 : 0, key, partial, nblk, coef);
        } else if (probe_pending && int_mode && len < (int64_t(1) << 32)) {
            launch_proj_coef_probe(s, len, n, r, dU, lab.L, key, partial, nblk, coef);
            if (PINNED_FIXED_BYTES + (size_t)r * 8 <= c->pinned_bytes) {
                probe_host = (double*)((char*)c->pinned + PINNED_FIXED_BYTES);
                HIP_TRY(c, hipMemcpyAsync(probe_host, coef + r, (size_t)r * 8, hipMemcpyDeviceToHost, s));
            }
        } else {
            launch_proj_coef(s, len, r, dU, lab.L, key, nullptr, partial, nblk, coef);
        }
        SigSource qp;
        if (Y) {
            qp.sig = sig;
            launch_proj_apply(s, len, r, dU, lab.L, key, nullptr, coef, atol, scale, 1, Y, sig);
        } else {
            qp = proj_source(lab.current(plab), packed_proj ? 1 : 0, plab ? 1 : 0);
        }
        tm.end();
        tm.begin(SDPSR_T_REFINE);
        int64_t d1 = 0;
        st = packed_proj ? lab.refine_packed(qp, &d1) : lab.refine_full(qp, &d1, int_mode);
        tm.end();
        if (st) return st;
        if (probe_host) {
            probe_pending = false, basis_sym = true;
            for (int64_t k = 0; k < r; ++k)
                if (!(std::fabs(probe_host[k]) <= 1e-10)) basis_sym = false;
        }
        int64_t d2 = d1;
        for (;;) {
            tm.begin(SDPSR_T_SQUARE);
            SigSource qs;
            st = launch_separate_square(next_key(c), d1, d2, &qs);
            if (st) return st;
            tm.end();
            tm.begin(SDPSR_T_REFINE);
            st = (int_mode && lab.sym) ? lab.refine_packed(qs, &d2) : lab.refine_full(qs, &d2, false);
            tm.end();
            if (st) return st;
            tm.collect();
            if (!another_confirm_round(d2 != current, confirm_left)) break;
        }
        *d_out = d2;
        return SDPSR_OK;
    }
    int initial_partition(const double* dCL, const double* dX0, int hint, const InitialRecord* guess, int64_t* d) {
        SigSource q;
        q.kind = SIG_PAIR, q.sig = sig, q.a = dCL, q.b = dX0;
        if (!((hint & 2) && lab.Lp && len < (int64_t(1) << 32))) return lab.refine_full(q, d, true);
        q.n = n, q.packed = 1, lab.sym = 1;
        initial_packed = true;
        const uint8_t* Lp8 = guess ? lab.Lp8 : nullptr;
        if (guess) {
            uint32_t* over = c->pinned_small + PINNED_SMALL_DEFERRED_NARROW.first;
            *(volatile uint32_t*)over = 0u;
            if (Lp8 && !(guess->narrow && guess->Lp8 == Lp8)) {
                launch_labels_narrow(s, n * (n + 1) / 2, lab.Lp, lab.Lp8, 8, over, c->num_cus);
                ++c->label_narrowings;
            }
        }
        if (guess && launch_verify_pair(s, n, dCL, dX0, lab.Lp, guess->d0, guess->first, c->pinned_small + PINNED_SMALL_DEFERRED_INITIAL.first, Lp8)) {
            c->initial_guess_pending = true;
            ++c->initial_guesses;
            HIP_TRY(c, hipGetLastError());
            *d = guess->d0;
            lab.packed_refined();
            lab.shadow_current();
            c->table_log2_hint = refine_table_hint(n * (n + 1) / 2, (uint64_t)guess->d0);
            return SDPSR_OK;
        }
        return lab.refine_packed(q, d);
    }
    int initial_guess_settled() {
        if (!c->initial_guess_pending) return SDPSR_OK;
        HIP_TRY(c, ctx_sync_stream(c, s));
        HIP_TRY(c, hipGetLastError());
        if (initial_guess_violated(c) != 0) return STATUS_REPEAT_REDUCTION;
        c->initial_guess_pending = false;
        return SDPSR_OK;
    }
    bool initial_packed = false;
    int square_buffers() {
        static const struct { const char *x, *c; size_t xb, cb; } B[] = {{"adm_xi8", "adm_ci32", 1, 4}, {"adm_xf32", "adm_cf32", 4, 4}, {"adm_xf64", "adm_cf64", 8, 8}};
        if (mode < SDPSR_SQUARE_I8 || mode > SDPSR_SQUARE_F64) return ctx_fail(c, SDPSR_BAD_ARGUMENT, "unknown square_mode");
        const size_t e = (size_t)T * ld * ld;
        Xp = ctx_buf(c, B[mode - SDPSR_SQUARE_I8].x, e * B[mode - SDPSR_SQUARE_I8].xb);
        Cp = ctx_buf(c, B[mode - SDPSR_SQUARE_I8].c, e * B[mode - SDPSR_SQUARE_I8].cb);
        if (mode == SDPSR_SQUARE_F32) {
            vmax = std::min(127, (int)std::floor(std::sqrt(16777216.0 / (double)n)));
            if (vmax < 1) return ctx_fail(c, SDPSR_BAD_ARGUMENT, "n too large for the exact fp32 square");
        }
        if (mode == SDPSR_SQUARE_F64 && !(Y = (double*)ctx_buf(c, "adm_y", (size_t)len * 8))) return SDPSR_OUT_OF_MEMORY;
        return (Xp && Cp) ? SDPSR_OK : SDPSR_OUT_OF_MEMORY;
    }
};
}

namespace sdpsr {
void flush_deferred_tail(sdpsr_ctx* c, int max_segments) {
    DeferredTail& t = c->deferred_tail;
    for (; max_segments > 0 && t.next < t.count; --max_segments, ++t.next) {
        const DeferredSegment& g = t.seg[t.next];
        launch_gemm_tn_i8_sym(c->stream, t.ld, t.ld, g.X, t.ld, g.C, t.ld, t.T, t.ld * t.ld, t.ld * t.ld, t.zero_flag, c->num_cus, c->opts.square_kernel);
        ++c->squares_launched;
        if (g.speculative) ++c->squares_speculative;
        launch_verify_no_split(c->stream, g.q, t.d, t.first, g.vref, g.flag);
    }
}

int admissible_subspace_impl(sdpsr_ctx* c, int64_t n, const double* CL, const double* X0L, const double* U, int64_t r, double atol,
                             uint32_t* P_out, int64_t* dim_out, int32_t* iters_out, double* phase_ms, int mem, int mem_out,
                             bool final_sync, int* labels_sym_out) {
    CHECK_CTX(c);
    const int hint = c->hint_symmetric_basis;
    c->hint_symmetric_basis = 0;
    c->hint_used = hint;
    c->adm_dims.clear();
    const InitialRecord rec = c->initial_record;
    c->initial_record = InitialRecord{};
    if (!CL || !X0L || !P_out || !dim_out || n < 1 || r < 0 || (r > 0 && !U) || !(atol > 0))
        return ctx_fail(c, SDPSR_BAD_ARGUMENT, "bad arguments");
    const int64_t len = n * n;
    int st = check_len(c, len);
    if (st) return st;
    hipStream_t s = c->stream;
    PhaseTimer tm(c, phase_ms != nullptr);
    TotalEvents ev_total(phase_ms != nullptr, s);

    c->table_log2_hint = 12;
    Loop lp(c, tm);
    lp.n = n, lp.len = len, lp.ld = round_up(n, 128), lp.r = r, lp.atol = atol;
    lp.early_ok = !(c->opts.flags & SDPSR_FLAG_WAIT_FOR_EVERY_VERDICT);
    const double* dCL = in_dev(c, "adm_cl", CL, len, mem, &st);
    const double* dX0 = in_dev(c, "adm_x0", X0L, len, mem, &st);
    lp.dU = in_dev(c, "adm_u", U, (size_t)len * std::max<int64_t>(r, 1), mem, &st);
    lp.lab.L = out_dev(c, "adm_labels", P_out, len, mem_out, &st);
    lp.sig = (uint64_t*)ctx_buf(c, "sig", len * 8);
    lp.partial = (double*)ctx_buf(c, "proj_partial", (size_t)2 * std::max<int64_t>(r, 1) * lp.nblk * 8);
    lp.coef = (double*)ctx_buf(c, "proj_coef", (size_t)2 * std::max<int64_t>(r, 1) * 8);
    lp.symflag = (uint32_t*)ctx_buf(c, "adm_symflag", 64);
    if (st || !lp.sig || !lp.partial || !lp.coef || !lp.symflag) return st ? st : SDPSR_OUT_OF_MEMORY;
    if (!c->symflag_zero) HIP_TRY(c, hipMemsetAsync(lp.symflag, 0, 64, s));
    c->symflag_zero = true;
    lp.zero_flag = lp.symflag + 8;
    lp.mode = c->opts.square_mode, lp.T = (lp.mode == SDPSR_SQUARE_F64) ? 1 : c->opts.channels;
    st = lp.square_buffers();
    if (st) return st;
    lp.scale = round_scale(c, atol);
    lp.int_mode = (lp.mode == SDPSR_SQUARE_I8 || lp.mode == SDPSR_SQUARE_F32);
    lp.lab.Lp = lp.int_mode ? (uint32_t*)ctx_buf(c, "adm_lpacked", (size_t)(n * (n + 1) / 2) * 4) : nullptr;
    if (lp.int_mode && !lp.lab.Lp) return SDPSR_OUT_OF_MEMORY;
    lp.keep_packed = lp.mode == SDPSR_SQUARE_I8 && (lp.T == 1 || lp.T == 2 || lp.T == 4) && !(c->opts.flags & SDPSR_FLAG_UNPACK_EVERY_STEP);
    lp.lab.init(c, n, lp.symflag, lp.keep_packed, lp.early_ok);

    const bool first_joint = !(c->opts.flags & (SDPSR_FLAG_SEPARATE_REFINEMENTS | SDPSR_FLAG_NO_VERIFY_SHORTCUT)) && lp.keep_packed && (lp.T == 2 || lp.T == 4) &&
                             (r == 0 || (hint & 1)) && r <= 4 && len < (int64_t(1) << 32) && c->opts.max_iters >= 1;
    const bool guess_initial = c->allow_deferred_verdict && c->pinned_small && lp.early_ok && c->predict_closed && c->predict_n == n && (hint & 2) && first_joint &&
                               rec.valid && rec.n == n && rec.Lp == lp.lab.Lp && rec.sym == 1 && rec.d0 >= 1 && rec.d0 <= (int64_t)verify_lds_cap() &&
                               c->first_idx_labels == lp.lab.Lp && rec.first == (const uint32_t*)ctx_buf(c, "ref_first", (size_t)refine_first_cap() * 4);
    if (dbg_on() && c->allow_deferred_verdict && !guess_initial)
        fprintf(stderr, "[sdpsr] loop: initial partition not guessed (predicted closed %d at n %lld, hint %d, joint first iteration %d, record %d: n %lld, d0 %lld, "
                        "labels %d, representatives of them %d)\n", (int)c->predict_closed, (long long)c->predict_n, hint, (int)first_joint, (int)rec.valid,
                (long long)rec.n, (long long)rec.d0, (int)(rec.Lp == lp.lab.Lp), (int)(c->first_idx_labels == lp.lab.Lp));
    if (guess_initial && rec.d0 <= 255 && !(c->opts.flags & SDPSR_FLAG_WIDE_LOOP_LABELS))
        lp.lab.Lp8 = (uint8_t*)ctx_buf(c, "adm_lpacked8", (size_t)(n * (n + 1) / 2));
    int64_t d = 0;
    tm.begin(SDPSR_T_REFINE);
    st = lp.initial_partition(dCL, dX0, hint, guess_initial ? &rec : nullptr, &d);
    tm.end();
    if (st) return st;
    tm.collect();
    c->adm_dims.assign(1, d);
    if (label_overflows(c, (uint64_t)d)) return label_overflow_fail(c, "admissible_subspace: dim(S)", (uint64_t)d);
    lp.basis_sym = (r == 0) || (hint & 1) != 0, lp.probe_pending = !lp.basis_sym;

    const int64_t maximal = (len + n) / 2;
    lp.current = d, lp.confirm_left = c->opts.confirm_rounds;
    bool converged = lp.current >= maximal;
    const bool separate = (c->opts.flags & SDPSR_FLAG_SEPARATE_REFINEMENTS) != 0;
    while (lp.current < maximal) {
        if (lp.it >= c->opts.max_iters) break;
        ++lp.it;
        tm.begin(SDPSR_T_PROJECT);
        lp.key = next_key(c);
        lp.packed_proj = lp.int_mode && lp.lab.sym && lp.basis_sym && r <= 4 && len < (int64_t(1) << 32);
        const bool joint = !separate && lp.packed_proj && lp.keep_packed && (lp.T == 2 || lp.T == 4) && c->table_log2_hint < 21;
        int64_t dn = lp.current;
        st = joint ? lp.joint_iteration(&dn) : lp.separate_iteration(&dn);
        if (st) return st;
        c->adm_dims.push_back(dn);
        if (label_overflows(c, (uint64_t)dn)) return label_overflow_fail(c, "admissible_subspace: dim(S)", (uint64_t)dn);
        if (dn == lp.current) {
            converged = true;
            break;
        }
        lp.confirm_left = c->opts.confirm_rounds;
        lp.current = dn;
        if (lp.current >= maximal) converged = true;
    }
    lp.lab.need_full();
    HIP_TRY(c, hipGetLastError());
    c->predict_closed = converged && lp.it == 1 && c->adm_dims.size() == 2 && c->adm_dims[0] == c->adm_dims[1];
    c->predict_n = n;
    if (converged && lp.initial_packed && c->first_idx_labels == lp.lab.Lp && c->adm_dims[0] >= 1 && c->adm_dims[0] <= (int64_t)verify_lds_cap() &&
        std::all_of(c->adm_dims.begin(), c->adm_dims.end(), [&](int64_t x) { return x == c->adm_dims[0]; })) {
        InitialRecord& ir = c->initial_record;
        ir.first = (const uint32_t*)ctx_buf(c, "ref_first", (size_t)refine_first_cap() * 4);
        ir.n = n, ir.d0 = c->adm_dims[0], ir.Lp = lp.lab.Lp, ir.sym = lp.lab.sym;
        ir.narrow = lp.lab.narrow(), ir.Lp8 = ir.narrow ? lp.lab.Lp8 : nullptr;
        ir.valid = ir.first != nullptr;
    }
    *dim_out = lp.current;
    if (iters_out) *iters_out = lp.it;
    if (labels_sym_out) *labels_sym_out = lp.lab.sym;
    if (final_sync || mem_out != SDPSR_MEM_DEVICE) {
        st = out_finish(c, P_out, lp.lab.L, len, mem_out);
        if (st) return st;
    }
    if (phase_ms) {
        const float ms = ev_total.stop(s);
        tm.collect();
        for (int i = 0; i < SDPSR_T_COUNT; ++i) phase_ms[i] = tm.acc[i];
        phase_ms[SDPSR_T_TOTAL] = ms;
    }
    if (!converged) return ctx_fail(c, SDPSR_NOT_CONVERGED, "max_iters reached");
    return SDPSR_OK;
}
}

extern "C" {
int sdpsr_admissible_subspace(sdpsr_ctx* c, int64_t n, const double* CL, const double* X0L,
                              const double* U, int64_t r, double atol, uint32_t* P_out,
                              int64_t* dim_out, int32_t* iters_out, double* phase_ms, int mem) {
    if (!c || c->label_width == 32 || !P_out || !dim_out || n < 1)
        return admissible_subspace_impl(c, n, CL, X0L, U, r, atol, P_out, dim_out, iters_out, phase_ms, mem, mem, true, nullptr);
    CHECK_CTX(c);
    uint32_t* L = (uint32_t*)ctx_buf(c, "adm_labels", (size_t)n * n * 4);
    if (!L) return SDPSR_OUT_OF_MEMORY;
    const int st = admissible_subspace_impl(c, n, CL, X0L, U, r, atol, L, dim_out, iters_out, phase_ms, mem, SDPSR_MEM_DEVICE, true, nullptr);
    if (st && st != SDPSR_NOT_CONVERGED) return st;
    if (label_width_overflows(c, (uint64_t)*dim_out)) return label_width_fail(c, "admissible_subspace", (uint64_t)*dim_out);
    const int st_out = labels_out_finish(c, P_out, L, (size_t)n * n, mem);
    return st_out ? st_out : st;
}

int sdpsr_desymmetrize(sdpsr_ctx* c, int64_t n, uint32_t* P, int64_t* dim, int32_t* iters, int mem) {
    CHECK_CTX(c);
    if (!P || !dim || n < 1) return ctx_fail(c, SDPSR_BAD_ARGUMENT, "bad arguments");
    const int64_t len = n * n;
    int st = check_len(c, len);
    if (st) return st;
    uint32_t* L = (mem == SDPSR_MEM_DEVICE && c->label_width == 32) ? P : (uint32_t*)labels_in_dev(c, "adm_labels", (const uint32_t*)P, len, mem, &st);
    if (st) return st;
    st = desymmetrize_device(c, n, L, dim, iters);
    if (st) return st;
// ... 44 lines not shown
```

### sdpsymmetryreduction.jl_amd/csrc/prof/prof.cpp

```cpp
#include <algorithm>
#include <cmath>
#include <complex>
#include <cstdio>
#include <cstdlib>
#include <cstring>
#include <chrono>
#include <functional>
#include <numeric>

#include <rocblas/rocblas.h>
#include <rocsolver/rocsolver.h>

#include "../host_internal.h"
#include "../../../include/sdpsr_prof.h"

using namespace sdpsr;

namespace sdpsr {
void launch_fill_test_sig(hipStream_t s, int64_t len, int64_t nclasses, uint64_t* sig);
void launch_clock_sampler(hipStream_t s, long long* buf, int ns, const unsigned* flag, long long max_ticks, int* count);
void launch_wall_marker(hipStream_t s, long long* out);
bool launch_band_chase(hipStream_t s, int n, int b, double* A, int64_t ld, unsigned* progress, unsigned* abort_flag, double* d, double* e, int max_wgs);
void launch_band_panel_split(hipStream_t s, int64_t m, int b, double* P, int64_t ldp, double* V, int64_t ldv);
}
// ... 178 lines not shown
    if (!p->Lp || !p->first || !p->flag) return SDPSR_OUT_OF_MEMORY;
    HIP_TRY(c, hipMemcpyAsync(p->Lp, Lp_host, (size_t)np * 4, hipMemcpyHostToDevice, c->stream));
    HIP_TRY(c, hipMemcpyAsync(p->first, first_idx_host, (size_t)d * 4, hipMemcpyHostToDevice, c->stream));
    const int st = prof_label_shadow(c, p->Lp, np, d, width, &p->Lp8);
    if (st) return st;
    HIP_TRY(c, hipStreamSynchronize(c->stream));
    p->flag[0] = 0xDEADu;
    return SDPSR_OK;
}
int prof_verdict_down(sdpsr_ctx* c, bool ran, const ProfClasses& p, uint32_t* out) {
    HIP_TRY(c, hipStreamSynchronize(c->stream));
    HIP_TRY(c, hipGetLastError());
    if (!ran) return ctx_fail(c, SDPSR_BAD_ARGUMENT, "no check for this shape");
    out[0] = ((const volatile uint32_t*)p.flag)[0];
    out[1] = (uint32_t)verify_lds_cap();
    return SDPSR_OK;
}

int prof_gather_packed(sdpsr_ctx* c, int64_t n, int T, int64_t d, uint64_t key, int width, const uint32_t* Lp_host, const uint32_t* Lfull_host,
                       int8_t* X_plain, int8_t* X_writing, int8_t* X_full, uint32_t* L_inout, int64_t guard) {
    CHECK_CTX(c);
    if (!Lp_host || !X_plain || !X_writing || !L_inout || !Lfull_host != !X_full || n < 1 || n > 8192 || d < 0 || guard < 0 ||
        (T != 1 && T != 2 && T != 4))
        return ctx_fail(c, SDPSR_BAD_ARGUMENT, "bad arguments");
    hipStream_t s = c->stream;
    const int64_t ld = round_up(n, 128), np = n * (n + 1) / 2;
    const size_t xb = (size_t)T * ld * ld;
    uint32_t* Lp = (uint32_t*)ctx_buf(c, "prof_lp", (size_t)np * 4);
    uint32_t* Lf = (uint32_t*)ctx_buf(c, "prof_lfull", (size_t)n * n * 4);
    uint32_t* Lw = (uint32_t*)ctx_buf(c, "prof_lwritten", (size_t)(n * n + guard) * 4);
    int8_t* X = (int8_t*)ctx_buf(c, "prof_gx", 3 * xb);
    if (!Lp || !Lf || !Lw || !X) return SDPSR_OUT_OF_MEMORY;
    HIP_TRY(c, hipMemcpyAsync(Lp, Lp_host, (size_t)np * 4, hipMemcpyHostToDevice, s));
    HIP_TRY(c, hipMemcpyAsync(Lw, L_inout, (size_t)(n * n + guard) * 4, hipMemcpyHostToDevice, s));
    HIP_TRY(c, hipMemsetAsync(X, 0x5A, 3 * xb, s));
    const uint8_t* Lp8 = nullptr;
    const int st = prof_label_shadow(c, Lp, np, d, width, &Lp8);
    if (st) return st;
    launch_gather_i8_sym_packed(s, n, ld, T, Lp, key, X, d, nullptr, Lp8);
    launch_gather_i8_sym_packed(s, n, ld, T, Lp, key, X + xb, d, Lw, Lp8);
    if (X_full) {
        HIP_TRY(c, hipMemcpyAsync(Lf, Lfull_host, (size_t)n * n * 4, hipMemcpyHostToDevice, s));
        launch_gather_i8(s, n, ld, T, Lf, key, X + 2 * xb, d);
        HIP_TRY(c, hipMemcpyAsync(X_full, X + 2 * xb, xb, hipMemcpyDeviceToHost, s));
    }
    HIP_TRY(c, hipMemcpyAsync(X_plain, X, xb, hipMemcpyDeviceToHost, s));
    HIP_TRY(c, hipMemcpyAsync(X_writing, X + xb, xb, hipMemcpyDeviceToHost, s));
    HIP_TRY(c, hipMemcpyAsync(L_inout, Lw, (size_t)(n * n + guard) * 4, hipMemcpyDeviceToHost, s));
    HIP_TRY(c, hipStreamSynchronize(s));
    HIP_TRY(c, hipGetLastError());
    return SDPSR_OK;
}

int prof_verify(sdpsr_ctx* c, int64_t n, int T, int64_t d, int r, int width, const uint32_t* Lp_host, const uint32_t* first_idx_host,
                const int32_t* C_host, const double* U_host, const double* coef_host, uint64_t key, double atol, uint32_t* out) {
    CHECK_CTX(c);
    if (!Lp_host || !first_idx_host || !C_host || !out || n < 1 || n > 8192 || d < 1 || d > (int64_t)refine_first_cap() || r < -1 || r > 4 ||
        (T != 2 && T != 4) || (r > 0 && (!U_host || !coef_host)) || !(atol > 0))
        return ctx_fail(c, SDPSR_BAD_ARGUMENT, "bad arguments");
    hipStream_t s = c->stream;
    const int64_t ld = round_up(n, 128), rr = r > 0 ? r : 0;
    const size_t cb = (size_t)T * ld * ld * 4;
    int32_t* Cd = (int32_t*)ctx_buf(c, "prof_vc", cb);
    double* Ud = (double*)ctx_buf(c, "prof_vu", (size_t)(n * n + 1) * 4 * 8);
    void* ref = ctx_buf(c, "prof_vref", verify_ref_bytes(d));
    if (!Cd || !Ud || !ref) return SDPSR_OUT_OF_MEMORY;
    double* coef = Ud + 4 * n * n;
    ProfClasses p;
    const int st = prof_classes_up(c, n, d, width, Lp_host, first_idx_host, &p);
    if (st) return st;
    HIP_TRY(c, hipMemcpyAsync(Cd, C_host, cb, hipMemcpyHostToDevice, s));
    if (rr > 0) {
        HIP_TRY(c, hipMemcpyAsync(Ud, U_host, (size_t)rr * n * n * 8, hipMemcpyHostToDevice, s));
        HIP_TRY(c, hipMemcpyAsync(coef, coef_host, (size_t)rr * 8, hipMemcpyHostToDevice, s));
    }
    SigSource q;
    q.kind = r >= 0 ? SIG_JOINT_I32 : SIG_CHAN_I32, q.U = Ud, q.coef = coef, q.r = (int)rr, q.key = key, q.atol = atol, q.scale = round_scale(c, atol);
    q.n = n, q.ld = ld, q.T = T, q.C = Cd, q.L = p.Lp, q.L8 = p.Lp8, q.packed = 1, q.lab_packed = 1;
    return prof_verdict_down(c, launch_verify_no_split(s, q, d, p.first, ref, p.flag), p, out);
}

int prof_basis_constant(sdpsr_ctx* c, int64_t n, int r, int64_t d, const uint32_t* Lp_host, const uint32_t* first_idx_host, const double* U_host,
                        double atol, uint32_t* out) {
    CHECK_CTX(c);
    if (!Lp_host || !first_idx_host || !U_host || !out || n < 1 || n > 8192 || d < 1 || d > (int64_t)refine_first_cap() || r < 1 || r > 4 ||
        !(atol > 0))
        return ctx_fail(c, SDPSR_BAD_ARGUMENT, "bad arguments");
    double* Ud = (double*)ctx_buf(c, "prof_vu", (size_t)(n * n + 1) * 4 * 8);
    void* ref = ctx_buf(c, "prof_vref", uconst_ref_bytes(d, r));
    if (!Ud || !ref) return SDPSR_OUT_OF_MEMORY;
    HIP_TRY(c, hipMemcpyAsync(Ud, U_host, (size_t)r * n * n * 8, hipMemcpyHostToDevice, c->stream));
    ProfClasses p;
    const int st = prof_classes_up(c, n, d, 32, Lp_host, first_idx_host, &p);
    if (st) return st;
    const bool ran = launch_basis_constant_on_classes(c->stream, n, r, Ud, p.Lp, d, p.first, atol, round_scale(c, atol), ref, p.flag);
    return prof_verdict_down(c, ran, p, out);
}

int prof_verify_pair(sdpsr_ctx* c, int64_t n, int64_t d, int width, const uint32_t* Lp_host, const uint32_t* first_idx_host, const double* a_host,
                     const double* b_host, uint32_t* out) {
    CHECK_CTX(c);
    if (!Lp_host || !first_idx_host || !a_host || !b_host || !out || n < 1 || n > 8192 || d < 1 || d > (int64_t)verify_lds_cap())
        return ctx_fail(c, SDPSR_BAD_ARGUMENT, "bad arguments");
    double* ab = (double*)ctx_buf(c, "prof_pair_ab", (size_t)2 * n * n * 8);
    if (!ab) return SDPSR_OUT_OF_MEMORY;
    HIP_TRY(c, hipMemcpyAsync(ab, a_host, (size_t)n * n * 8, hipMemcpyHostToDevice, c->stream));
    HIP_TRY(c, hipMemcpyAsync(ab + n * n, b_host, (size_t)n * n * 8, hipMemcpyHostToDevice, c->stream));
    ProfClasses p;
    const int st = prof_classes_up(c, n, d, width, Lp_host, first_idx_host, &p);
    if (st) return st;
    return prof_verdict_down(c, launch_verify_pair(c->stream, n, ab, ab + n * n, p.Lp, d, p.first, p.flag, p.Lp8), p, out);
}
}

extern "C" int sdpsr_profile_gather_packed(sdpsr_ctx* c, int64_t n, int T, int64_t d, uint64_t key, const uint32_t* Lp_host, const uint32_t* Lfull_host,
                                           int8_t* X_plain, int8_t* X_writing, int8_t* X_full, uint32_t* L_inout, int64_t guard) {
    if (!Lfull_host || !X_full) return c ? ctx_fail(c, SDPSR_BAD_ARGUMENT, "bad arguments") : SDPSR_BAD_ARGUMENT;
    return prof_gather_packed(c, n, T, d, key, 32, Lp_host, Lfull_host, X_plain, X_writing, X_full, L_inout, guard);
}
extern "C" int sdpsr_profile_gather_packed_w(sdpsr_ctx* c, int64_t n, int T, int64_t d, uint64_t key, int width, const uint32_t* Lp_host,
                                             int8_t* X_plain, int8_t* X_writing, uint32_t* L_inout, int64_t guard) {
    return prof_gather_packed(c, n, T, d, key, width, Lp_host, nullptr, X_plain, X_writing, nullptr, L_inout, guard);
}
extern "C" int sdpsr_profile_verify(sdpsr_ctx* c, int64_t n, int T, int64_t d, int mode, const uint32_t* Lp_host, const uint32_t* first_idx_host,
                                    const int32_t* C_host, const double* U_host, double coef, uint64_t key, double atol, uint32_t* out) {
    if (mode == 2) return prof_basis_constant(c, n, 1, d, Lp_host, first_idx_host, U_host, atol, out);
    if (mode != 0 && mode != 1) return c ? ctx_fail(c, SDPSR_BAD_ARGUMENT, "bad arguments") : SDPSR_BAD_ARGUMENT;
    return prof_verify(c, n, T, d, mode == 1 ? 1 : -1, 32, Lp_host, first_idx_host, C_host, U_host, &coef, key, atol, out);
}
extern "C" int sdpsr_profile_verify_w(sdpsr_ctx* c, int64_t n, int T, int64_t d, int r, int width, const uint32_t* Lp_host,
                                      const uint32_t* first_idx_host, const int32_t* C_host, const double* U_host, const double* coef_host,
                                      uint64_t key, double atol, uint32_t* out) {
    return prof_verify(c, n, T, d, r, width, Lp_host, first_idx_host, C_host, U_host, coef_host, key, atol, out);
}
extern "C" int sdpsr_profile_basis_constant(sdpsr_ctx* c, int64_t n, int r, int64_t d, const uint32_t* Lp_host, const uint32_t* first_idx_host,
                                            const double* U_host, double atol, uint32_t* out) {
    return prof_basis_constant(c, n, r, d, Lp_host, first_idx_host, U_host, atol, out);
}
extern "C" int sdpsr_profile_verify_pair(sdpsr_ctx* c, int64_t n, int64_t d, const uint32_t* Lp_host, const uint32_t* first_idx_host,
                                         const double* a_host, const double* b_host, uint32_t* out) {
    return prof_verify_pair(c, n, d, 32, Lp_host, first_idx_host, a_host, b_host, out);
}
extern "C" int sdpsr_profile_verify_pair_w(sdpsr_ctx* c, int64_t n, int64_t d, int width, const uint32_t* Lp_host, const uint32_t* first_idx_host,
                                           const double* a_host, const double* b_host, uint32_t* out) {
    return prof_verify_pair(c, n, d, width, Lp_host, first_idx_host, a_host, b_host, out);
}

extern "C" int sdpsr_profile_square_checks(sdpsr_ctx* c, int32_t restart, uint64_t* out) {
    CHECK_CTX(c);
    if (!out || restart < 0 || restart > (int32_t)c->batch_children.size()) return ctx_fail(c, SDPSR_BAD_ARGUMENT, "bad arguments");
    const sdpsr_ctx* ci = restart == 0 ? c : c->batch_children[restart - 1];
    out[0] = ci->square_checks;
    out[1] = ci->square_check_fallbacks;
    return SDPSR_OK;
}

extern "C" int sdpsr_profile_square_check(sdpsr_ctx* c, int64_t n, int64_t d, int G, int T, const uint64_t* keys, int width, int write_full,
                                          const uint32_t* Lp_host, const uint32_t* first_idx_host, uint8_t* ws_inout, uint64_t* layout,
                                          uint32_t* verdicts_out, uint32_t* L_inout, int64_t guard) {
    CHECK_CTX(c);
    constexpr size_t gap = 64;
    if (!layout || !square_check_supports(n, d, G, T) || n > 8192 || (width != 8 && width != 32) || guard < 0 || guard > (int64_t(1) << 20))
        return ctx_fail(c, SDPSR_BAD_ARGUMENT, "bad arguments");
    SquareCheck q;
    q.n = n, q.d = d, q.G = G, q.T = T;
    const size_t bytes = square_check_ws_carve(q, nullptr, gap);
    void* ws = ctx_buf(c, "prof_sqcheck", bytes);
    if (!ws) return SDPSR_OUT_OF_MEMORY;
    square_check_ws_carve(q, ws, gap);
    const void* parts[7] = {q.c, q.part_x, q.part_c, q.y, q.w, q.esum, q.bits};
    for (int k = 0; k < 7; ++k) layout[k] = (uint64_t)((const char*)parts[k] - (const char*)ws);
    layout[7] = bytes;
    if (!ws_inout) return SDPSR_OK;
    if (!keys || !Lp_host || !first_idx_host || !verdicts_out || (write_full && !L_inout)) return ctx_fail(c, SDPSR_BAD_ARGUMENT, "null pointer");
    hipStream_t s = c->stream;
    uint32_t* Lw = write_full ? (uint32_t*)ctx_buf(c, "prof_lwritten", (size_t)(n * n + guard) * 4) : nullptr;
    uint32_t* flag1 = pinned_report(c, PINNED_SPECULATIVE);
    if ((write_full && !Lw) || !flag1) return SDPSR_OUT_OF_MEMORY;
    ProfClasses p;
    const int st = prof_classes_up(c, n, d, width, Lp_host, first_idx_host, &p);
    if (st) return st;
    HIP_TRY(c, hipMemcpyAsync(ws, ws_inout, bytes, hipMemcpyHostToDevice, s));
    if (write_full) HIP_TRY(c, hipMemcpyAsync(Lw, L_inout, (size_t)(n * n + guard) * 4, hipMemcpyHostToDevice, s));
    for (int g = 0; g < G; ++g) q.key[g] = keys[g];
    q.Lp = p.Lp, q.Lp8 = p.Lp8, q.first_idx = p.first, q.Lfull = Lw;
    q.flag[0] = p.flag, q.flag[1] = flag1;
    *(volatile uint32_t*)q.flag[0] = 0u;
    *(volatile uint32_t*)q.flag[1] = 0u;
    launch_square_check_ref_and_pass(s, q);
    launch_square_check_verdict(s, q);
    HIP_TRY(c, hipMemcpyAsync(ws_inout, ws, bytes, hipMemcpyDeviceToHost, s));
    if (write_full) HIP_TRY(c, hipMemcpyAsync(L_inout, Lw, (size_t)(n * n + guard) * 4, hipMemcpyDeviceToHost, s));
    HIP_TRY(c, hipStreamSynchronize(s));
    HIP_TRY(c, hipGetLastError());
    verdicts_out[0] = ((const volatile uint32_t*)q.flag[0])[0];
    verdicts_out[1] = ((const volatile uint32_t*)q.flag[1])[0];
    return SDPSR_OK;
}

extern "C" int sdpsr_profile_proj_coef_lower(sdpsr_ctx* c, int64_t n, int64_t r, uint64_t key, int width, const uint32_t* Lp_host,
                                             const double* U_host, double* partial_out, double* coef_out) {
    CHECK_CTX(c);
    if (!Lp_host || !U_host || !partial_out || !coef_out || n < 1 || n > 8192 || r < 1 || r > 4) return ctx_fail(c, SDPSR_BAD_ARGUMENT, "bad arguments");
    constexpr int nblk = 2048;
    hipStream_t s = c->stream;
    const int64_t np = n * (n + 1) / 2;
    uint32_t* Lp = (uint32_t*)ctx_buf(c, "prof_lp", (size_t)np * 4);
    double* Ud = (double*)ctx_buf(c, "prof_vu", (size_t)(n * n + 1) * 4 * 8);
    double* partial = (double*)ctx_buf(c, "prof_partial", (size_t)(r * nblk + r) * 8);
    if (!Lp || !Ud || !partial) return SDPSR_OUT_OF_MEMORY;
    double* coef = partial + r * nblk;
    HIP_TRY(c, hipMemcpyAsync(Lp, Lp_host, (size_t)np * 4, hipMemcpyHostToDevice, s));
    HIP_TRY(c, hipMemcpyAsync(Ud, U_host, (size_t)r * n * n * 8, hipMemcpyHostToDevice, s));
    HIP_TRY(c, hipMemsetAsync(partial, 0xFF, (size_t)(r * nblk + r) * 8, s));
    const uint8_t* Lp8 = nullptr;
    const int st = prof_label_shadow(c, Lp, np, 0, width, &Lp8);
    if (st) return st;
    launch_proj_coef_lower(s, n, r, Ud, Lp, 1, key, partial, nblk, coef, Lp8);
    HIP_TRY(c, hipMemcpyAsync(partial_out, partial, (size_t)r * nblk * 8, hipMemcpyDeviceToHost, s));
    HIP_TRY(c, hipMemcpyAsync(coef_out, coef, (size_t)r * 8, hipMemcpyDeviceToHost, s));
    HIP_TRY(c, hipStreamSynchronize(s));
    HIP_TRY(c, hipGetLastError());
    return SDPSR_OK;
}

extern "C" int sdpsr_profile_refine_source(sdpsr_ctx* c, int kind, int what, int64_t n, int64_t ld, int T, int r, int packed, int lab_packed,
                                           uint64_t key, double atol, const double* a_host, const double* b_host, const double* U_host,
                                           const double* coef_host, const void* C_host, uint32_t* L_inout, uint32_t* Lnew_inout, int64_t guard,
                                           int64_t prev_classes, int sym, uint64_t* sig_out, int64_t* nparts, uint32_t* first_out, int32_t* report) {
    CHECK_CTX(c);
    enum { RS_PAIR = 0, RS_PROJ = 1, RS_CHAN_I32 = 2, RS_CHAN_F32 = 3, RS_JOINT = 4 };
    const bool pair = kind == RS_PAIR, proj = kind == RS_PROJ || kind == RS_JOINT, chan = kind == RS_CHAN_I32 || kind == RS_CHAN_F32 || kind == RS_JOINT;
    if (kind < RS_PAIR || kind > RS_JOINT || (what != 0 && what != 1) || n < 1 || n > 2048 || guard < 0 || guard > (int64_t(1) << 20) ||
        prev_classes < 0 || prev_classes > (int64_t(1) << 32) || !L_inout || !nparts || !report || (packed != 0 && packed != 1) ||
        (lab_packed != 0 && lab_packed != 1) || (lab_packed && !packed) || (sym && packed))
        return ctx_fail(c, SDPSR_BAD_ARGUMENT, "refine_source: bad arguments");
    if (pair && (!a_host || !b_host || lab_packed != packed)) return ctx_fail(c, SDPSR_BAD_ARGUMENT, "refine_source: bad pair source");
    if (proj && (r < 0 || r > 8 || (r > 0 && (!U_host || !coef_host)) || !(atol > 0))) return ctx_fail(c, SDPSR_BAD_ARGUMENT, "refine_source: bad projection");
    if (chan && (!C_host || T < 1 || T > 8 || ld < n || ld > 2048 || ld % 128)) return ctx_fail(c, SDPSR_BAD_ARGUMENT, "refine_source: bad channels");
    const bool apart = !pair && packed && !lab_packed;
    if (apart != (Lnew_inout != nullptr)) return ctx_fail(c, SDPSR_BAD_ARGUMENT, "refine_source: Lnew_inout goes with packed and not lab_packed");
    hipStream_t s = c->stream;
    const int64_t np = n * (n + 1) / 2, len = packed ? np : n * n, lablen = lab_packed ? np : n * n;
    const int64_t rr = proj ? r : 0;
    const size_t cb = chan ? (size_t)T * ld * ld * 4 : 0;
    double* ab = pair ? (double*)ctx_buf(c, "prof_rs_ab", (size_t)2 * n * n * 8) : nullptr;
    double* Ud = proj ? (double*)ctx_buf(c, "prof_rs_u", (size_t)(rr * n * n + rr + 1) * 8) : nullptr;
    void* Cd = chan ? ctx_buf(c, "prof_rs_c", cb) : nullptr;
    uint32_t* Ld = (uint32_t*)ctx_buf(c, "prof_rs_l", (size_t)(lablen + guard) * 4);
    uint32_t* Lnew = apart ? (uint32_t*)ctx_buf(c, "prof_rs_lnew", (size_t)(np + guard) * 4) : nullptr;
    uint64_t* sig = (uint64_t*)ctx_buf(c, "prof_rs_sig", (size_t)len * 8);
    uint64_t* sig2 = (sig_out && what == 0) ? (uint64_t*)ctx_buf(c, "prof_rs_sig2", (size_t)len * 8) : nullptr;
    uint32_t* symflag = sym ? (uint32_t*)ctx_buf(c, "prof_rs_symflag", 64) : nullptr;
    if ((pair && !ab) || (proj && !Ud) || (chan && !Cd) || !Ld || (apart && !Lnew) || !sig || (sig_out && what == 0 && !sig2) || (sym && !symflag))
        return SDPSR_OUT_OF_MEMORY;
    double* coef = proj ? Ud + rr * n * n : nullptr;
    SigSource q;
    q.sig = sig;
    if (pair) {
        q.kind = SIG_PAIR, q.a = ab, q.b = ab + n * n;
        if (packed) q.n = n, q.packed = 1;
    } else {
        if (proj) q.kind = SIG_PROJ, q.U = Ud, q.coef = coef, q.r = (int)rr, q.key = key, q.atol = atol, q.scale = round_scale(c, atol), q.n = n;
        if (chan) q.kind = kind == RS_JOINT ? SIG_JOINT_I32 : (kind == RS_CHAN_F32 ? SIG_CHAN_F32 : SIG_CHAN_I32), q.n = n, q.ld = ld, q.T = T, q.C = Cd;
        q.L = Ld, q.packed = packed, q.lab_packed = lab_packed;
    }
    const bool standalone = (chan && kind != RS_JOINT) || (kind == RS_PROJ && !packed);
    if (what == 0 ? !(sig_source_fusable(q) || standalone) : !standalone)
        return ctx_fail(c, SDPSR_BAD_ARGUMENT, "refine_source: no kernel for this source's shape");
    if (pair) {
        HIP_TRY(c, hipMemcpyAsync(ab, a_host, (size_t)n * n * 8, hipMemcpyHostToDevice, s));
        HIP_TRY(c, hipMemcpyAsync(ab + n * n, b_host, (size_t)n * n * 8, hipMemcpyHostToDevice, s));
    }
    if (rr > 0) {
        HIP_TRY(c, hipMemcpyAsync(Ud, U_host, (size_t)rr * n * n * 8, hipMemcpyHostToDevice, s));
        HIP_TRY(c, hipMemcpyAsync(coef, coef_host, (size_t)rr * 8, hipMemcpyHostToDevice, s));
    }
    if (chan) HIP_TRY(c, hipMemcpyAsync(Cd, C_host, cb, hipMemcpyHostToDevice, s));
    HIP_TRY(c, hipMemcpyAsync(Ld, L_inout, (size_t)(lablen + guard) * 4, hipMemcpyHostToDevice, s));
    if (apart) HIP_TRY(c, hipMemcpyAsync(Lnew, Lnew_inout, (size_t)(np + guard) * 4, hipMemcpyHostToDevice, s));
    uint32_t* labels = apart ? Lnew : Ld;
    c->table_log2_hint = refine_table_hint(len, (uint64_t)prev_classes);
    const uint64_t passes0 = c->refine_passes;
    int64_t d = 0;
    int symv = -1, st;
    if (what == 0) {
        if (sig_out) {
            if (!launch_sig_materialize(s, len, q, sig2)) return ctx_fail(c, SDPSR_BAD_ARGUMENT, "refine_source: nothing writes this source out");
            HIP_TRY(c, hipMemcpyAsync(sig_out, sig2, (size_t)len * 8, hipMemcpyDeviceToHost, s));
        }
        st = sym ? refine_signatures(c, len, q, labels, &d, n, symflag, &symv) : refine_signatures(c, len, q, labels, &d);
    } else {
        if (kind == RS_PROJ) launch_proj_apply(s, len, rr, Ud, Ld, key, nullptr, coef, atol, q.scale, 1, nullptr, sig);
        else if (kind == RS_CHAN_I32) launch_sig_i32(s, n, ld, T, Ld, (const int32_t*)Cd, sig, packed, lab_packed);
        else launch_sig_f32(s, n, ld, T, Ld, (const float*)Cd, sig, packed, lab_packed);
        if (sig_out) HIP_TRY(c, hipMemcpyAsync(sig_out, sig, (size_t)len * 8, hipMemcpyDeviceToHost, s));
        st = sym ? refine_signatures(c, len, sig, labels, &d, n, symflag, &symv) : refine_signatures(c, len, sig, labels, &d);
    }
    if (st) return st;
    HIP_TRY(c, hipMemcpyAsync(L_inout, Ld, (size_t)(lablen + guard) * 4, hipMemcpyDeviceToHost, s));
    if (apart) HIP_TRY(c, hipMemcpyAsync(Lnew_inout, Lnew, (size_t)(np + guard) * 4, hipMemcpyDeviceToHost, s));
    const uint32_t* first = (const uint32_t*)ctx_buf(c, "ref_first", (size_t)refine_first_cap() * 4);
    if (first_out && first && d > 0)
        HIP_TRY(c, hipMemcpyAsync(first_out, first, (size_t)std::min<int64_t>(d, refine_first_cap()) * 4, hipMemcpyDeviceToHost, s));
    HIP_TRY(c, hipStreamSynchronize(s));
    HIP_TRY(c, hipGetLastError());
// ... 1059 lines not shown
```

### sdpsymmetryreduction.jl_amd/csrc/reduce.cpp

```cpp
#include <algorithm>
#include <cstring>
#include <new>

#include "host_internal.h"

using namespace sdpsr;

namespace sdpsr {
int jordan_reduce_impl(sdpsr_ctx* c, int64_t n, const double* CL, const double* X0L, const double* U, int64_t r, double atol, double epsilon,
                       uint32_t* P_out, int64_t* dim_out, int32_t* iters_out, int32_t* nblocks, int64_t* sum_sq, int64_t* sum_s, double* blks,
                       int64_t blks_capacity, double* Q_hat, int64_t qhat_capacity, double* phase_ms, int mem_in, int mem_out) {
    const int mem = mem_out;
    CHECK_CTX(c);
    if (!dim_out || n < 1 || !(epsilon > 0) || blks_capacity < 0 || qhat_capacity < 0 || (blks_capacity > 0 && !blks) ||
        (qhat_capacity > 0 && !Q_hat))
        return ctx_fail(c, SDPSR_BAD_ARGUMENT, "bad arguments");
    const int64_t len = n * n;
    int st = check_len(c, len);
    if (st) return st;
    hipStream_t s = c->stream;
    const uint64_t stream_at_entry = c->stream_counter;
    const int hint_at_entry = c->hint_symmetric_basis;
    const bool in_place = mem == SDPSR_MEM_DEVICE && P_out != nullptr && c->label_width == 32;
    uint32_t* L = in_place ? P_out : (uint32_t*)ctx_buf(c, "bd_labels", (size_t)len * 4);
    if (!L) return SDPSR_OUT_OF_MEMORY;
    c->bd_valid = false;
    c->bd_q_valid = false;
    c->bd_qrm_current = false;
    c->bd_labels_ext = nullptr;
    double pm_a[SDPSR_T_COUNT] = {}, pm_b[SDPSR_T_COUNT] = {}, pm_i[SDPSR_T_COUNT] = {};
    int labels_sym = 0;
    c->deferred_verdict = false;
    c->initial_guess_pending = false;
    struct DropTail {
        sdpsr_ctx* c;
        ~DropTail() { c->deferred_tail.count = c->deferred_tail.next = 0; }
    } drop_tail{c};
    auto repeat_without_guesses = [&](uint32_t dv, uint32_t dv_spec, uint32_t dv_init) -> int {
        c->predict_closed = false;
        c->initial_record = InitialRecord{};
        if (dv_init != 0) ++c->initial_guesses_violated;
        if (dbg_on())
            fprintf(stderr, "[sdpsr] jordan_reduce: %s%s%s (deferred verdicts: verify %u, speculative %u, initial partition %u): reduction repeated\n",
                    dv_init != 0 ? "the initial partition was not the recorded one" : "", dv_init != 0 && (dv != 0 || dv_spec != 0) ? "; " : "",
                    dv != 0 ? "the input was not closed after all" : (dv_spec != 0 ? "the confirm round found a split" : ""), dv, dv_spec, dv_init);
        c->stream_counter = stream_at_entry;
        c->hint_symmetric_basis = hint_at_entry;
        if (mem_in != SDPSR_MEM_DEVICE) {
            CL = (const double*)ctx_buf(c, "adm_cl", (size_t)len * 8);
            X0L = (const double*)ctx_buf(c, "adm_x0", (size_t)len * 8);
            if (U) U = (const double*)ctx_buf(c, "adm_u", (size_t)len * std::max<int64_t>(r, 1) * 8);
            if (!CL || !X0L || (r > 0 && !U)) return SDPSR_OUT_OF_MEMORY;
            mem_in = SDPSR_MEM_DEVICE;
        }
        return jordan_reduce_impl(c, n, CL, X0L, U, r, atol, epsilon, P_out, dim_out, iters_out, nblocks, sum_sq, sum_s, blks, blks_capacity, Q_hat,
                                  qhat_capacity, phase_ms, mem_in, mem_out);
    };
    auto leave = [&](int st_err) -> int {
        if (!c->initial_guess_pending) return st_err;
        c->initial_guess_pending = false;
        c->deferred_verdict = false;
        flush_deferred_tail(c);
        if (ctx_sync_stream(c, s) != hipSuccess) return st_err == STATUS_REPEAT_REDUCTION ? ctx_fail(c, SDPSR_HIP_ERROR, "hipStreamSynchronize failed") : st_err;
        const uint32_t dv_init = initial_guess_violated(c);
        if (dv_init != 0) return repeat_without_guesses(0, 0, dv_init);
        return st_err == STATUS_REPEAT_REDUCTION ? ctx_fail(c, SDPSR_BAD_STATE, "jordan_reduce: a repeat was asked for without a violated verdict") : st_err;
    };
    c->allow_deferred_verdict = !(c->opts.flags & SDPSR_FLAG_WAIT_FOR_EVERY_VERDICT);
    st = admissible_subspace_impl(c, n, CL, X0L, U, r, atol, L, dim_out, iters_out, phase_ms ? pm_a : nullptr, mem_in, SDPSR_MEM_DEVICE,
                                  false, &labels_sym);
    c->allow_deferred_verdict = false;
    const int st_loop = st;
    if (st && st != SDPSR_NOT_CONVERGED) return leave(st);
    const bool overflow = P_out && label_width_overflows(c, (uint64_t)*dim_out);
    if (P_out && !in_place && !overflow) {
        st = labels_deliver(c, P_out, L, (size_t)len, mem);
        if (st) return leave(st);
    }
    const int64_t d = *dim_out;
    int32_t nb = 0;
    int64_t S = 0, S1 = 0;
    st = overflow ? SDPSR_OK
                  : block_diagonalize_impl(c, n, L, d, epsilon, &nb, &S, &S1, phase_ms ? pm_b : nullptr, SDPSR_MEM_DEVICE, labels_sym != 0,
                                           false, in_place);
    flush_deferred_tail(c);
    if (nblocks) *nblocks = nb;
    if (sum_sq) *sum_sq = S;
    if (sum_s) *sum_s = S1;
    bool images_done = false;
    if (st == SDPSR_OK && !overflow && blks && d * S <= blks_capacity && (!Q_hat || n * S1 <= qhat_capacity)) {
        st = sdpsr_block_images(c, blks, (Q_hat && n * S1 <= qhat_capacity) ? Q_hat : nullptr, phase_ms ? pm_i : nullptr, mem);
        images_done = st == SDPSR_OK;
    }
    if (in_place) {
        struct Forget {
            sdpsr_ctx* c;
            bool ok = false;
            ~Forget() {
                c->bd_labels_ext = nullptr;
                c->bd_trusted_symmetric = nullptr;
                if (!ok) c->bd_valid = false;
            }
        } forget{c};
        if (!images_done && c->bd_valid) {
            uint32_t* keep = (uint32_t*)ctx_buf(c, "bd_labels", (size_t)len * 4);
            if (!keep) return leave(SDPSR_OUT_OF_MEMORY);
            const hipError_t ek = hipMemcpyAsync(keep, P_out, (size_t)len * 4, hipMemcpyDeviceToDevice, s);
            if (ek != hipSuccess) return leave(ctx_fail(c, SDPSR_HIP_ERROR, std::string("hipMemcpyAsync: ") + hipGetErrorString(ek)));
        } else if (images_done) {
            c->bd_valid = false;
        }
        forget.ok = true;
    }
    if (!images_done) {
        flush_deferred_tail(c);
        const hipError_t e = ctx_sync_stream(c, s);
        if (e != hipSuccess && st == SDPSR_OK) st = ctx_fail(c, SDPSR_HIP_ERROR, std::string("hipStreamSynchronize: ") + hipGetErrorString(e));
    }
    if (c->deferred_verdict || c->initial_guess_pending) {
        const volatile uint32_t* ps = c->pinned_small;
        const uint32_t dv = c->deferred_verdict ? ps[PINNED_SMALL_DEFERRED_VERIFY.first] : 0u;
        const uint32_t dv_spec = c->deferred_verdict ? ps[PINNED_SMALL_DEFERRED_SPECULATIVE.first] : 0u;
        const uint32_t dv_init = c->initial_guess_pending ? initial_guess_violated(c) : 0u;
        c->deferred_verdict = false;
        c->initial_guess_pending = false;
        if (dv != 0 || dv_spec != 0 || dv_init != 0) {
            const int st2 = repeat_without_guesses(dv, dv_spec, dv_init);
            if (phase_ms)
                for (int i = 0; i < SDPSR_T_COUNT; ++i) phase_ms[i] += pm_a[i] + pm_b[i] + pm_i[i];
            return st2;
        }
    }
    if (phase_ms) {
        for (int i = 0; i < SDPSR_T_COUNT; ++i) phase_ms[i] = pm_a[i] + pm_b[i] + pm_i[i];
    }
    if (overflow && st == SDPSR_OK) return label_width_fail(c, "jordan_reduce: admissible_subspace", (uint64_t)d);
    if (st == SDPSR_OK && P_out && !in_place) st = labels_delivered(c);
    return st ? st : st_loop;
}
}

extern "C" int sdpsr_jordan_reduce(sdpsr_ctx* c, int64_t n, const double* CL, const double* X0L, const double* U, int64_t r,
                                   double atol, double epsilon, uint32_t* P_out, int64_t* dim_out, int32_t* iters_out,
                                   int32_t* nblocks, int64_t* sum_sq, int64_t* sum_s, double* blks, int64_t blks_capacity,
                                   double* Q_hat, int64_t qhat_capacity, double* phase_ms, int mem) {
    return jordan_reduce_impl(c, n, CL, X0L, U, r, atol, epsilon, P_out, dim_out, iters_out, nblocks, sum_sq, sum_s, blks, blks_capacity, Q_hat,
                              qhat_capacity, phase_ms, mem, mem);
}

extern "C" int sdpsr_problem_create(sdpsr_ctx* c, int64_t n, const double* CL, const double* X0L, const double* U, int64_t r, int hint, int mem,
                                    sdpsr_problem** out) {
    CHECK_CTX(c);
    if (!out || !CL || !X0L || n < 1 || r < 0 || (r > 0 && !U)) return ctx_fail(c, SDPSR_BAD_ARGUMENT, "bad arguments");
    *out = nullptr;
    const int64_t len = n * n;
    int st = check_len(c, len);
    if (st) return st;
    DeviceGuard dg(c->device);
    sdpsr_problem* p = new (std::nothrow) sdpsr_problem();
    if (!p) return SDPSR_OUT_OF_MEMORY;
    p->device = c->device;
    p->n = n;
    p->r = r;
    p->hint = hint & 3;
    const size_t vb = (size_t)len * 8;
    auto fail = [&](int code, const char* what) {
        sdpsr_problem_destroy(p);
        return ctx_fail(c, code, what);
    };
    if (hipMalloc((void**)&p->CL, vb) != hipSuccess || hipMalloc((void**)&p->X0, vb) != hipSuccess ||
        (r > 0 && hipMalloc((void**)&p->U, vb * (size_t)r) != hipSuccess))
        return fail(SDPSR_OUT_OF_MEMORY, "sdpsr_problem_create: device memory");
    const hipMemcpyKind kind = mem == SDPSR_MEM_DEVICE ? hipMemcpyDeviceToDevice : hipMemcpyHostToDevice;
    if (hipMemcpyAsync(p->CL, CL, vb, kind, c->stream) != hipSuccess || hipMemcpyAsync(p->X0, X0L, vb, kind, c->stream) != hipSuccess ||
        (r > 0 && hipMemcpyAsync(p->U, U, vb * (size_t)r, kind, c->stream) != hipSuccess))
        return fail(SDPSR_HIP_ERROR, "sdpsr_problem_create: copy");
    if (mem != SDPSR_MEM_DEVICE) c->h2d_bytes += vb * (size_t)(2 + r);
    if (ctx_sync_stream(c, c->stream) != hipSuccess) return fail(SDPSR_HIP_ERROR, "sdpsr_problem_create: synchronisation");
    *out = p;
    return SDPSR_OK;
}

extern "C" int sdpsr_problem_destroy(sdpsr_problem* p) {
    if (!p) return SDPSR_OK;
    DeviceGuard dg(p->device);
    if (p->CL) hipFree(p->CL);
    if (p->X0) hipFree(p->X0);
    if (p->U) hipFree(p->U);
    delete p;
    return SDPSR_OK;
}

extern "C" int sdpsr_problem_reduce(sdpsr_ctx* c, const sdpsr_problem* p, double atol, double epsilon, uint32_t* P_out, int64_t* dim_out,
                                    int32_t* iters_out, int32_t* nblocks, int64_t* sum_sq, int64_t* sum_s, double* blks, int64_t blks_capacity,
// ... 17 lines not shown
```

### sdpsymmetryreduction.jl_amd/csrc/sdpsr_internal.h

```cpp
#pragma once
#include <hip/hip_runtime.h>
#include <stdint.h>
#include <stddef.h>

#include <map>
#include <functional>
#include <string>
#include <string_view>
#include <vector>

#include "../../include/sdpsr.h"
#include "sdpsr_hash.h"

namespace sdpsr { struct SytrdGraphCache; }

struct DevBuf {
    void* p = nullptr;
    size_t bytes = 0;
};

namespace sdpsr {
enum { SIG_ARRAY = 0, SIG_PAIR = 1, SIG_PROJ = 2, SIG_CHAN_I32 = 3, SIG_CHAN_F32 = 4, SIG_JOINT_I32 = 5 };
struct SigSource {
    int kind = SIG_ARRAY;
    uint64_t* sig = nullptr;
    const double *a = nullptr, *b = nullptr;
    const double *U = nullptr, *coef = nullptr;
    const uint32_t* L = nullptr;
    int r = 0;
    uint64_t key = 0;
    double atol = 0, scale = 1;
    int64_t n = 0, ld = 0;
    int T = 0;
    const void* C = nullptr;
    int packed = 0;
    int lab_packed = 0;
    const uint8_t* L8 = nullptr;
};

struct DeferredSegment {
    const int8_t* X = nullptr;
    int32_t* C = nullptr;
    SigSource q;
    void* vref = nullptr;
    uint32_t* flag = nullptr;
    bool speculative = false;
};
constexpr int DEFERRED_SEGMENTS = 2;
struct DeferredTail {
    DeferredSegment seg[DEFERRED_SEGMENTS];
    int count = 0, next = 0;
    int64_t ld = 0, d = 0;
    int T = 0;
    const uint32_t* zero_flag = nullptr;
    const uint32_t* first = nullptr;
};
constexpr uint32_t DEFERRED_NEVER_RAN = 0xDEFE44EDu;
struct InitialRecord {
    bool valid = false;
    int64_t n = 0, d0 = 0;
    const uint32_t *Lp = nullptr, *first = nullptr;
    int sym = 0;
    bool narrow = false;
    const uint8_t* Lp8 = nullptr;
};
constexpr int STATUS_REPEAT_REDUCTION = -0x5250;
}

struct sdpsr_ctx {
    int device = 0;
    int num_cus = 256;
    uint64_t seed = 0;
    uint64_t stream_counter = 0;
    sdpsr_opts opts{};
    int label_width = 32;
    hipStream_t stream = nullptr;
    hipStream_t side_stream = nullptr;
    hipEvent_t ev_fork = nullptr, ev_join = nullptr, ev_wait = nullptr;
    hipEvent_t ev_bt_fork = nullptr, ev_bt_join = nullptr;
    hipStream_t main_shadow = nullptr;
    bool own_stream = false;
    std::string err;
    double dbg_last_ms = 0;
    std::map<std::string, DevBuf, std::less<>> bufs;
    void* pinned = nullptr;
    size_t pinned_bytes = 0;
    uint32_t* pinned_small = nullptr;
    void* h2d_ring = nullptr;
    int h2d_ring_next = 0;
    void* rocblas = nullptr;
    sdpsr::SytrdGraphCache* sytrd_graphs = nullptr;
    int64_t bd_n = 0, bd_d = 0;
    std::vector<int32_t> bd_sizes;
    int64_t bd_sum_s = 0, bd_sum_sq = 0;
    bool bd_valid = false;
    int64_t bdc_n = 0, bdc_d = 0, bdc_sum_s = 0, bdc_sum_sq = 0;
    std::vector<int32_t> bdc_sizes;
    bool bdc_valid = false;
    uint32_t bd_sym_epoch = 0;
    const uint32_t* bd_sym_labels = nullptr;
    const uint32_t* bd_labels_ext = nullptr;
    const uint32_t* bd_trusted_symmetric = nullptr;
    uint32_t epoch_counter = 0;
    const uint32_t* first_idx_labels = nullptr;
    int hint_symmetric_basis = 0;
    std::vector<int64_t> adm_dims;
    bool bd_q_valid = false;
    bool bd_labels_owned = false;
    bool bd_qrm_current = false;
    int table_log2_hint = 12;
    uint64_t refine_passes = 0;
    hipEvent_t ev[2 * SDPSR_T_COUNT] = {};
    void (*yield_fn)(void*) = nullptr;
    void* yield_arg = nullptr;
    std::vector<sdpsr_ctx*> batch_children;
    uint64_t h2d_bytes = 0, d2h_bytes = 0;
    bool predict_closed = false;
    int64_t predict_n = 0;
    uint64_t squares_launched = 0, squares_speculative = 0;
    uint64_t square_checks = 0, square_check_fallbacks = 0;
    int hint_used = 0;
    uint64_t host_waits = 0;
    uint32_t report_seq = 0;
    bool allow_deferred_verdict = false;
    bool deferred_verdict = false;
    sdpsr::DeferredTail deferred_tail;
    sdpsr::InitialRecord initial_record;
    bool initial_guess_pending = false;
    uint64_t initial_guesses = 0, initial_guesses_violated = 0;
    uint64_t label_narrowings = 0;
    bool symflag_zero = false;
};

struct sdpsr_problem {
    int device = 0;
    int64_t n = 0, r = 0;
    double *CL = nullptr, *X0 = nullptr, *U = nullptr;
    int hint = 0;
};

struct sdpsr_sparse {
    int device = 0;
    int64_t len = 0, m = 0, nnz = 0;
    int64_t* rowptr = nullptr;
    uint32_t* col = nullptr;
    double* val = nullptr;
    int rows_symmetric = 0;
};

struct sdpsr_blockop {
    int device = 0;
    int64_t d = 0, sum_sq = 0, nnz_full = 0;
    std::vector<int32_t> sizes;
    void* by_class = nullptr;
    void* by_pos = nullptr;
};

struct BlocksSyevJob {
    int64_t zoff, woff;
    int32_t n, pad;
};

inline hipError_t ctx_sync_stream(sdpsr_ctx* c, hipStream_t s) {
    if (c) ++c->host_waits;
    if (!c || !c->yield_fn) return hipStreamSynchronize(s);
    const hipError_t before = hipPeekAtLastError();
    for (;;) {
        const hipError_t e = hipStreamQuery(s);
        if (e != hipErrorNotReady) {
            if (hipPeekAtLastError() == hipErrorNotReady) (void)hipGetLastError();
            if (e == hipSuccess && before != hipSuccess && before != hipErrorNotReady) return before;
            return e;
        }
        c->yield_fn(c->yield_arg);
    }
}

inline hipError_t ctx_wait_word(sdpsr_ctx* c, hipStream_t s, const volatile uint32_t* w, uint32_t seq) {
    ++c->host_waits;
    const hipError_t before = hipPeekAtLastError();
    bool queried = false;
    hipError_t res = hipSuccess;
    for (unsigned spins = 1;; ++spins) {
        if (*w == seq) break;
        if (c->yield_fn || (spins & 2047u) == 0) {
            queried = true;
            const hipError_t e = hipStreamQuery(s);
            if (e != hipErrorNotReady) {
                res = e != hipSuccess ? e : (*w == seq ? hipSuccess : hipErrorUnknown);
                break;
            }
            if (c->yield_fn) c->yield_fn(c->yield_arg);
        } else {
            __builtin_ia32_pause();
        }
    }
    __atomic_thread_fence(__ATOMIC_ACQUIRE);
    if (queried && hipPeekAtLastError() == hipErrorNotReady) (void)hipGetLastError();
    if (res == hipSuccess && before != hipSuccess && before != hipErrorNotReady) return before;
    return res;
}

void* ctx_buf(sdpsr_ctx* c, const char* name, size_t bytes);
int ctx_fail(sdpsr_ctx* c, int status, const std::string& msg);

#define HIP_TRY(c, expr)                                                              \
    do {                                                                              \
        hipError_t _e = (expr);                                                       \
        if (_e != hipSuccess)                                                         \
            return ctx_fail((c), SDPSR_HIP_ERROR,                                     \
                            std::string(#expr) + ": " + hipGetErrorString(_e));       \
    } while (0)

namespace sdpsr {

void launch_fill_f64(hipStream_t s, int64_t len, const uint32_t* L, const double* values, int64_t d,
                     double* M, uint32_t* bad_flag);
void launch_randomize_f64(hipStream_t s, int64_t len, const uint32_t* L, uint64_t key, double* M);
void launch_clamp_round(hipStream_t s, int64_t len, double* a, double atol, double scale);
void launch_gather_i8(hipStream_t s, int64_t n, int64_t ld, int T, const uint32_t* L,
                      uint64_t key, int8_t* X, int64_t dmax = 0);
void launch_gather_f32(hipStream_t s, int64_t n, int64_t ld, int T, int vmax, const uint32_t* L,
                       uint64_t key, float* X);
void launch_gather_f64_padded(hipStream_t s, int64_t n, int64_t ld, const uint32_t* L,
                              uint64_t key, double* X);
void launch_gather_i8_sym_packed(hipStream_t s, int64_t n, int64_t ld, int T, const uint32_t* Lp, uint64_t key, int8_t* X,
                                 int64_t dmax, uint32_t* Lfull = nullptr, const uint8_t* Lp8 = nullptr);
void launch_unpad_mirror_lower_i32(hipStream_t s, int64_t n, int64_t ld, const int32_t* src, int32_t* dst);
void launch_pad_copy(hipStream_t s, int64_t n, int64_t ld, const void* src, void* dst,
                     int elem_bytes);
void launch_unpad_copy(hipStream_t s, int64_t n, int64_t ld, const void* src, void* dst,
                       int elem_bytes);

void launch_proj_coef(hipStream_t s, int64_t len, int64_t r, const double* U, const uint32_t* L,
                      uint64_t key, const double* xin, double* partial, int nblk, double* coef);
void launch_proj_coef_lower(hipStream_t s, int64_t n, int64_t r, const double* U, const uint32_t* L, int lab_packed,
                            uint64_t key, double* partial, int nblk, double* coef, const uint8_t* Lp8 = nullptr);
void launch_proj_coef_probe(hipStream_t s, int64_t len, int64_t n, int64_t r, const double* U, const uint32_t* L, uint64_t key,
                            double* partial, int nblk, double* coef);
void launch_proj_apply(hipStream_t s, int64_t len, int64_t r, const double* U, const uint32_t* L,
                       uint64_t key, const double* xin, const double* coef, double atol,
                       double scale, int do_round, double* yout, uint64_t* sig);

void launch_sig_f64(hipStream_t s, int64_t len, const uint32_t* L, const double* v, uint64_t* sig);
void launch_sig_f64_rounded(hipStream_t s, int64_t n, int64_t ld, const uint32_t* L,
                            const double* v, double atol, double scale, uint64_t* sig);
void launch_sig_u32(hipStream_t s, int64_t len, const uint32_t* L, const uint32_t* k,
                    uint64_t* sig);
void launch_sig_u64(hipStream_t s, int64_t len, const uint64_t* k, uint64_t* sig);
void launch_sig_i32(hipStream_t s, int64_t n, int64_t ld, int T, const uint32_t* L,
                    const int32_t* C, uint64_t* sig, int packed = 0, int lab_packed = 0);
void launch_sig_f32(hipStream_t s, int64_t n, int64_t ld, int T, const uint32_t* L,
                    const float* C, uint64_t* sig, int packed = 0, int lab_packed = 0);
bool sig_source_fusable(const SigSource& q);
bool launch_sig_materialize(hipStream_t s, int64_t len, const SigSource& q, uint64_t* sig);

struct RefSlot {
    unsigned long long sig;
    uint32_t min;
    uint32_t pad;
};
struct RefineWs {
    RefSlot* tab;
    uint32_t* tab_lab;
    uint32_t* blk_cnt;
    int insert_wgs_per_cu = 0;
    uint32_t* host_counters = nullptr;
    uint32_t host_seq = 0;
    int mid = 0;
    int expect_small = 0;
    uint32_t* first_idx = nullptr;
    void* rank_ws = nullptr;
    size_t rank_ws_bytes = 0;
    uint32_t* counters;
    int log2cap;
    int nblk;
};
size_t refine_block_entries();
size_t refine_counters_bytes();
uint32_t refine_small_k();
uint32_t refine_first_cap();
bool refine_mid_supports(const SigSource& q);
bool launch_refine(hipStream_t s, int64_t len, const SigSource& q, uint32_t* slot, uint32_t* labels_out,
                   const RefineWs& ws, int64_t sym_n = 0);

size_t verify_ref_bytes(int64_t d);
size_t uconst_ref_bytes(int64_t d, int64_t r);
int verify_lds_cap();
bool launch_basis_constant_on_classes(hipStream_t s, int64_t n, int64_t r, const double* U, const uint32_t* Lp, int64_t d,
                                      const uint32_t* first_idx, double atol, double scale, void* ref, uint32_t* flag);
bool launch_verify_no_split(hipStream_t s, const SigSource& q, int64_t d, const uint32_t* first_idx, void* ref, uint32_t* flag);
bool verify_no_split_supports(const SigSource& q, int64_t d);
bool launch_verify_pair(hipStream_t s, int64_t n, const double* a, const double* b, const uint32_t* Lp, int64_t d, const uint32_t* first_idx,
                        uint32_t* flag, const uint8_t* Lp8 = nullptr);
bool launch_verify_projection(hipStream_t s, const SigSource& q, int64_t d, const uint32_t* first_idx, uint32_t* flag);
constexpr int SQUARE_CHECK_MAX_CLASSES = 255;
constexpr int64_t SQUARE_CHECK_MAX_ORDER = 1 << 15;
struct SquareCheck {
    int64_t n = 0, d = 0;
    int G = 0, T = 0;
    uint64_t key[2] = {0, 0};
    const uint32_t* Lp = nullptr;
    const uint8_t* Lp8 = nullptr;
    const uint32_t* first_idx = nullptr;
    uint32_t* Lfull = nullptr;
    uint32_t* flag[2] = {nullptr, nullptr};
    int32_t *c = nullptr, *part_x = nullptr;
    int64_t *part_c = nullptr, *y = nullptr, *w = nullptr;
    uint64_t* esum = nullptr;
    uint32_t* bits = nullptr;
};
bool square_check_supports(int64_t n, int64_t d, int G, int T);
size_t square_check_ws_bytes(int64_t n, int64_t d, int G, int T);
size_t square_check_ws_carve(SquareCheck& q, void* ws, size_t gap = 0);
void launch_square_check_ref_and_pass(hipStream_t s, const SquareCheck& q);
void launch_square_check_verdict(hipStream_t s, const SquareCheck& q);
void flush_deferred_tail(sdpsr_ctx* c, int max_segments = DEFERRED_SEGMENTS);
inline bool deferred_tail_pending(const sdpsr_ctx* c) { return c->deferred_tail.next < c->deferred_tail.count; }
void launch_report_stamp(hipStream_t s, uint32_t* host_word, uint32_t seq);

size_t refine_bucketed_workspace_bytes(int64_t len);
bool refine_bucket_set_device_attributes();
bool launch_refine_bucketed(hipStream_t s, int64_t len, const uint64_t* sig, uint32_t* labels_out, void* ws, size_t ws_bytes,
                            uint32_t* counters, uint32_t* first_idx, uint32_t first_cap, uint32_t* host_counters = nullptr, uint32_t host_seq = 0);
size_t refine_rank_slots_workspace_bytes(int64_t len);
bool launch_rank_slots(hipStream_t s, int64_t len, int64_t cap, const RefSlot* tab, uint32_t* tab_lab,
                       uint32_t* counters, uint32_t small_k, uint32_t* first_idx, uint32_t first_cap, void* ws, size_t ws_bytes);
size_t refine_sample_workspace_bytes();
int64_t launch_refine_sample(hipStream_t s, int64_t len, const uint64_t* sig, void* ws, uint32_t* host_out);
size_t refine_sorted_workspace_bytes(int64_t len);
bool launch_refine_sorted(hipStream_t s, int64_t len, const uint64_t* sig, uint32_t* labels_out, void* ws, size_t ws_bytes,
                          uint32_t* counters);

void launch_max_pair_code(hipStream_t s, int64_t len, const uint32_t* p1, const uint32_t* p2, uint64_t d1, uint64_t* out);
void launch_transpose_labels(hipStream_t s, int64_t n, const uint32_t* L, uint32_t* Lt);
void launch_labels_checksum(hipStream_t s, int64_t len, const uint32_t* L, uint64_t* partial, uint64_t* out);
void launch_unpack_symmetric_labels(hipStream_t s, int64_t n, const uint32_t* Lp, uint32_t* L);
void launch_check_symmetric(hipStream_t s, int64_t n, const uint32_t* L, uint32_t* flag);
void launch_copy_check_symmetric(hipStream_t s, int64_t n, const uint32_t* src, uint32_t* dst, uint32_t* flag, uint32_t epoch);
void launch_copy_check_labels(hipStream_t s, int64_t n, const uint32_t* src, uint32_t* dst, uint32_t dmax, uint32_t* flag);

int64_t reduce_columns_chunk(int64_t len, int64_t m, int64_t d);
bool launch_reduce_columns(hipStream_t s, int64_t len, int64_t m, int64_t d, const uint32_t* L, const double* A,
                           double* partial, double* out, uint32_t* bad_flag);
void launch_transpose_rows(hipStream_t s, int64_t len, int64_t m, const double* A, double* R);
void launch_col_norms2(hipStream_t s, int64_t len, int64_t k, const double* V, double* partial, int nblk, double* out);
void launch_scale_copy(hipStream_t s, int64_t len, const double* v, double alpha, double* out);
void launch_rank1_update(hipStream_t s, int64_t len, int64_t m, double* R, const double* u, const double* dots);
void launch_sub_round(hipStream_t s, int64_t len, const double* a, const double* b, double atol, double scale, double* out);

void launch_symmetrize(hipStream_t s, int64_t m, int64_t ld, double* B);
void launch_tall_times_small(hipStream_t s, int64_t n, int64_t ldi, const double* In, int kk, const double* S,
                             int lds_, int ncols, double alpha, double beta, double* out, int64_t ldo);
struct LabelSpmmForm {
    int mfma, tile, z, cols_per_block;
};
bool label_spmm_select(int64_t n, int64_t d, int G, int w, LabelSpmmForm* f);
bool label_spmm_pair_select(int64_t n, int64_t d, int w, LabelSpmmForm* f);
size_t label_spmm_pair_partial_doubles(int64_t n);
bool launch_label_spmm_pair(hipStream_t s, int64_t n, const uint32_t* L, const uint64_t* keys, int64_t d, const double* W, int64_t ldw,
                            int w, double* partials, double* Y0, int64_t ldy0, double* Y1, int64_t ldy1);

bool gemm_set_device_attributes();
bool blockdiag_set_device_attributes();
bool module_set_device_attributes();
bool dense_setup_set_device_attributes();
bool insert_array_pair_set_device_attributes();
bool insert_proj_set_device_attributes();
bool insert_chan_set_device_attributes();
bool insert_joint_set_device_attributes();
bool sytrd_set_device_attributes();
bool small_syev_set_device_attributes();
bool stedc_set_device_attributes();
bool batched_set_device_attributes();
bool backtransform_set_device_attributes();
bool complex_set_device_attributes();
void launch_cx_embed(hipStream_t s, int64_t n, const double* Hr, const double* Hi, int64_t ld2, double* M);
void launch_cx_embed_adjoint(hipStream_t s, int64_t n, const double* Zr, const double* Zi, int64_t ld2, double* M);
void launch_cx_newton_schulz_factor(hipStream_t s, int64_t m, int64_t ld, double* K);
void launch_cx_unstack(hipStream_t s, int64_t n, int64_t cols, const double* E, int64_t ld2, double* Vr, double* Vi, int64_t ldv);
void launch_cx_rot(hipStream_t s, int64_t n, int64_t cols, int64_t ld2, const double* E, double* R);
void launch_cx_zero_pad(hipStream_t s, int64_t m, int64_t mc, int64_t ld, int64_t ldc, double* A);
void launch_cx_combine(hipStream_t s, int64_t n, int64_t ld2, const double* E, const int32_t* desc, const double* coef, double* Vr,
                       double* Vi);
void launch_cx_stack(hipStream_t s, int64_t n, int64_t cols, const double* Vr, const double* Vi, int64_t ldv, int64_t ld2, double* E);
void launch_cx_block_norms_general(hipStream_t s, int64_t n, int64_t ldn, const double* Gr, const double* Gi, const int32_t* space_of,
                                   int neig, unsigned long long* norms);
constexpr int64_t SDPSR_CX_MAX_N = 4096;
size_t cx_irreducible_general_lds_bytes(int64_t n);
bool launch_cx_irreducible_general(hipStream_t s, int64_t n, const double* Hr, const double* Hi, const double* Vr, const double* Vi,
                                   const int32_t* desc, int ncols, double atol, double* Qhat);
void launch_cx_basis_image_sorted(hipStream_t s, int64_t n, int64_t d, int64_t S, const uint32_t* ent, const int64_t* cls_ptr,
                                  const double* Qhat, const int32_t* descA, const int32_t* descB, double atol, double* out);
void launch_cx_gather_herm(hipStream_t s, int64_t n, const uint32_t* L, uint64_t key, double* Hr, double* Hi);
void launch_cx_heev(hipStream_t s, int64_t n, const double* Hr, const double* Hi, double* w, double* Vr, double* Vi, int* info);
void launch_cx_block_norms(hipStream_t s, int64_t n, const double* Hr, const double* Hi, const double* Vr, const double* Vi,
                           const int32_t* space_of, int neig, unsigned long long* norms);
void launch_cx_irreducible(hipStream_t s, int64_t n, const double* Hr, const double* Hi, const double* Vr, const double* Vi,
                           const int32_t* desc, int ncols, double atol, double* Qhat);
void launch_cx_basis_image(hipStream_t s, int64_t n, int64_t d, int64_t S, const uint32_t* L, const double* Qhat,
                           const int32_t* descA, const int32_t* descB, double atol, double* out);
void launch_cx_rowmajor(hipStream_t s, int64_t n, int64_t S1, const double* Qcm, double* Qrm);
void launch_cx_image_chunk(hipStream_t s, int64_t n, int64_t d, int64_t S1, int64_t S, const double* Qrm, const uint32_t* ent,
                           const int32_t* descA, const int32_t* descB, const int64_t* chunk_ptr, int64_t nchunks,
                           const int64_t* chunk_begin, const int64_t* chunk_end, double* partial, double* out, double atol);
bool cx_image_outer_supports(int max_s, int nblocks, int64_t d);
void launch_cx_image_outer(hipStream_t s, int64_t n, int64_t d, int64_t S1, int64_t S, int nblocks, int max_s, const double* Qrm,
                           const uint32_t* ent, const int64_t* cls_ptr, const int32_t* blk_col, const int32_t* blk_size,
                           const int64_t* blk_off, double atol, double* out);
void launch_eigdec_batched64(hipStream_t s, int64_t n, int64_t d, int64_t count, const uint32_t* L, const double* values,
                             uint64_t seed, uint64_t stream_base, double atol, int32_t* status, int32_t* neig,
                             int32_t* nclasses, int num_cus);
struct SytrdLookArgs {
    double* A;
    int64_t ld;
    int n;
    double* PT;
    double* PTc;
    double* P;
    double* acol;
    double* rec_norm;
    double* rec_dots;
    double* rec_vaz;
    int64_t vaz_cap;
    double *d, *e, *tau;
};
const void* sytrd_look_kernel_fn(int mode, int64_t ld);
void sytrd_graph_cache_destroy(SytrdGraphCache* g);
void sytrd_graph_cache_stats(const SytrdGraphCache* g, uint64_t* hits, uint64_t* misses, double* instantiate_ms);

void launch_gemm_tn_i8_sym(hipStream_t s, int64_t n, int64_t k, const int8_t* X, int64_t ldx, int32_t* C, int64_t ldc,
                           int batch, int64_t strideX, int64_t strideC, const uint32_t* nonsym_flag, int num_cus = 0,
                           int variant = 0);
bool launch_i8_symsquare(hipStream_t s, int64_t n, int64_t k, const int8_t* X, int64_t ldx, int32_t* C, int64_t ldc, int batch,
                         int64_t strideX, int64_t strideC, const uint32_t* nonsym_flag, int num_cus, int variant);
bool i8_symsquare_pays(int64_t n, int T, int num_cus);
bool gemm_sym_set_device_attributes();
void launch_gemm_tn_f32_sym(hipStream_t s, int64_t n, int64_t k, const float* X, int64_t ldx, float* C, int64_t ldc,
                            int batch, int64_t strideX, int64_t strideC, const uint32_t* nonsym_flag);
void launch_gemm_tn_i8(hipStream_t s, int64_t m, int64_t n, int64_t k, const int8_t* A,
                       int64_t lda, const int8_t* B, int64_t ldb, int32_t* C, int64_t ldc,
                       int batch, int64_t strideA, int64_t strideB, int64_t strideC);
void launch_gemm_tn_f32(hipStream_t s, int64_t m, int64_t n, int64_t k, const float* A,
                        int64_t lda, const float* B, int64_t ldb, float* C, int64_t ldc,
                        int batch, int64_t strideA, int64_t strideB, int64_t strideC);
void launch_gemm_tn_f64(hipStream_t s, int64_t m, int64_t n, int64_t k, const double* A,
                        int64_t lda, const double* B, int64_t ldb, double* C, int64_t ldc,
                        int batch, int64_t strideA, int64_t strideB, int64_t strideC);
void launch_gemm_tn_f64_sub(hipStream_t s, int64_t m, int64_t n, int64_t k, const double* A, int64_t lda, const double* B,
                            int64_t ldb, double* C, int64_t ldc);

void launch_small_qtaq_block_norms(hipStream_t s, int64_t n, int64_t ld, const double* A, const double* Q,
                                   const int32_t* space_of, int neig, unsigned long long* norms, double* Mout, double* Tout = nullptr);
size_t small_cluster_pack_bytes(int64_t n);
void launch_small_cluster_qtaq_block_norms(hipStream_t s, int64_t n, int64_t ld, const double* A, const double* Q,
                                           const double* evals, double atol, const int* einfo, char* pack, double* Tout);
void launch_coupling_symmetrize_minmax(hipStream_t s, int neig, unsigned long long* norms, const int32_t* dims, unsigned long long* stat);
void launch_coupling_count(hipStream_t s, int neig, const unsigned long long* norms, const double* edges17, unsigned long long* stat);
void launch_coupling_bits(hipStream_t s, int neig, const unsigned long long* norms, double thr, unsigned long long* bits);
void launch_block_norms(hipStream_t s, int64_t n, int64_t ld, const double* M,
                        const int32_t* space_of, int neig, unsigned long long* norms);
void launch_gemv_t(hipStream_t s, int64_t n, int64_t ld, const double* Q, int64_t col0,
                   int64_t m, const double* a, double* out);
void launch_gemv_n_scaled(hipStream_t s, int64_t n, int64_t ld, const double* Q, int64_t col0,
                          int64_t m, const double* w, const double* inv_norm, double* dst);
void launch_irreducible_pairs(hipStream_t s, int64_t n, int64_t ld, const double* Q, const double* Bf, int npairs,
                              int max_m2, const int32_t* desc, double* Qhat);
void launch_copy_cols(hipStream_t s, int64_t n, int64_t count, const int32_t* src_cols, const int32_t* dst_cols,
                      const double* src, int64_t ld_src, double* dst, int64_t ld_dst);
void launch_clamptol(hipStream_t s, int64_t len, double* a, double atol);
void launch_inv_norm(hipStream_t s, int64_t m, const double* v, double* out);
// ... 44 lines not shown
```

Measured before the change: 2034.

## Defer verdict and pair-check kernels into the deferred tail to ride host waits

Registers the square-check verdict, projection coefficient/verify kernels and the initial-guess pair verification as deferred segments instead of launching them inline. They are then launched by flush_deferred_tail, mostly during a later host wait in module growth. The intent is to take these checks off the loop's critical path and overlap them with host-side work. It adds flush calls at many boundaries, a flag to disable the behaviour, and steady-clock window instrumentation, which adds some host overhead and ordering risk.

```diff
diff --git a/include/sdpsr.h b/include/sdpsr.h
--- a/include/sdpsr.h
+++ b/include/sdpsr.h
@@ -61,7 +61,8 @@
     SDPSR_FLAG_WAIT_FOR_EVERY_VERDICT = 1u << 15,
     SDPSR_FLAG_WIDE_LOOP_LABELS = 1u << 16,
     SDPSR_FLAG_MODULE_SCRATCH_FILLS = 1u << 17,
-    SDPSR_FLAG_SQUARE_EVERY_VERDICT = 1u << 18
+    SDPSR_FLAG_SQUARE_EVERY_VERDICT = 1u << 18,
+    SDPSR_FLAG_CHECKS_IN_LOOP = 1u << 19
 };
 
 typedef struct sdpsr_opts {
diff --git a/include/sdpsr_prof.h b/include/sdpsr_prof.h
--- a/include/sdpsr_prof.h
+++ b/include/sdpsr_prof.h
@@ -38,6 +38,7 @@
                                 const void* C_host, uint32_t* L_inout, uint32_t* Lnew_inout, int64_t guard, int64_t prev_classes, int sym,
                                 uint64_t* sig_out, int64_t* nparts, uint32_t* first_out, int32_t* report);
 int sdpsr_profile_square_checks(sdpsr_ctx* ctx, int32_t restart, uint64_t* out);
+int sdpsr_profile_deferred_checks(sdpsr_ctx* ctx, int32_t restart, uint64_t* out);
 int sdpsr_profile_square_check(sdpsr_ctx* ctx, int64_t n, int64_t d, int G, int T, const uint64_t* keys, int width, int write_full,
                                const uint32_t* Lp_host, const uint32_t* first_idx_host, uint8_t* ws_inout, uint64_t* layout,
                                uint32_t* verdicts_out, uint32_t* L_inout, int64_t guard);
diff --git a/sdpsymmetryreduction.jl_amd/_lib.py b/sdpsymmetryreduction.jl_amd/_lib.py
--- a/sdpsymmetryreduction.jl_amd/_lib.py
+++ b/sdpsymmetryreduction.jl_amd/_lib.py
@@ -36,6 +36,7 @@
 FLAG_WIDE_LOOP_LABELS = 1 << 16
 FLAG_MODULE_SCRATCH_FILLS = 1 << 17
 FLAG_SQUARE_EVERY_VERDICT = 1 << 18
+FLAG_CHECKS_IN_LOOP = 1 << 19
 BASIS_IMAGE_KERNELS = {"auto": 0, "two_stage": 1, "outer": 2, "chunk": 3}
 BI_ROUTE_COMMUTATIVE, BI_ROUTE_BLOCKS, BI_ROUTE_TWO_STAGE, BI_ROUTE_OUTER, BI_ROUTE_CHUNK = 1, 2, 3, 4, 5
 BI_ROUTE_REPAIRED, BI_ROUTE_SHORTCUT_REFUSED = 0x100, 0x200
@@ -244,6 +245,8 @@
     lib.sdpsr_profile_verify_pair_w.argtypes = [vp, i64, i64, C.c_int, vp, vp, vp, vp, C.POINTER(C.c_uint32)]
     lib.sdpsr_profile_square_checks.restype = C.c_int
     lib.sdpsr_profile_square_checks.argtypes = [vp, C.c_int32, C.POINTER(C.c_uint64)]
+    lib.sdpsr_profile_deferred_checks.restype = C.c_int
+    lib.sdpsr_profile_deferred_checks.argtypes = [vp, C.c_int32, C.POINTER(C.c_uint64)]
     lib.sdpsr_profile_square_check.restype = C.c_int
     lib.sdpsr_profile_square_check.argtypes = [vp, i64, i64, C.c_int, C.c_int, vp, C.c_int, C.c_int, vp, vp, vp, vp, vp, vp, i64]
     lib.sdpsr_profile_proj_coef_lower.restype = C.c_int
diff --git a/sdpsymmetryreduction.jl_amd/csrc/compress.cpp b/sdpsymmetryreduction.jl_amd/csrc/compress.cpp
--- a/sdpsymmetryreduction.jl_amd/csrc/compress.cpp
+++ b/sdpsymmetryreduction.jl_amd/csrc/compress.cpp
@@ -28,6 +28,7 @@
     bool spec_b2 = false;
     bool sym_pre = false, sym_trusted = false, sym_checked = false;
     bool forked = false;
+    int window = 0;
     bool lean = false;
     int live = 0;
     bool parent_form() const { return (c->opts.flags & SDPSR_FLAG_MODULE_SCRATCH_FILLS) != 0; }
@@ -102,6 +103,7 @@
 }
 
 int Module::apply_generic(int wcols, double* dst) {
+    deferred_window_close(c);
     const uint64_t key = next_key(c);
     if (fused_product(wcols)) {
         double* part = (double*)ctx_buf(c, "cm_part", label_spmm_pair_partial_doubles(n) * 8);
@@ -122,6 +124,7 @@
 
 int Module::ortho_step(int mc, double tol, bool take_ref, const Rider* rider, Selection& sel) {
     const int64_t ap = round_up(w + mc, 128), mp = round_up(mc, 128);
+    deferred_window_close(c);
     double* hpin = (double*)ctx_pinned(c, (size_t)ap * mp * 8);
     bool host_filled = false;
     const bool ride = take_ref && hpin && deferred_tail_pending(c) && small_on_host() && gram_tn_is_skinny(w + mc, mc);
@@ -142,11 +145,13 @@
         const uint32_t seq = ++c->report_seq ? c->report_seq : ++c->report_seq;
         *(volatile uint32_t*)stamp = 0;
         launch_report_stamp(c->stream, stamp, seq);
-        flush_deferred_tail(c, 1);
+        flush_deferred_tail(c, 1, true);
         if (ctx_wait_word(c, c->stream, stamp, seq) != hipSuccess) return ctx_fail(c, SDPSR_HIP_ERROR, "report wait (module growth)");
+        deferred_window_open(c, window);
         memcpy(hG.data(), hpin, (size_t)ap * mc * 8);
     } else if (host_filled) {
         if (ctx_sync_stream(c, c->stream) != hipSuccess) return ctx_fail(c, SDPSR_HIP_ERROR, "hipStreamSynchronize (module growth)");
+        if (take_ref) deferred_window_open(c, window);
         memcpy(hG.data(), hpin, (size_t)ap * mc * 8);
     } else {
         st = d2h_sync(c, hG.data(), Cc, (size_t)ap * mc * 8);
@@ -209,6 +214,7 @@
         return SDPSR_OK;
     }
     launch_class_sums(c->stream, n, d, L, W, W + (size_t)w * ld, ld);
+    window = 0;
     int got;
     live = (int)d;
     return absorb((int)d, nullptr, got);
@@ -222,6 +228,8 @@
     const int m = G * w;
     double* Y = W + (size_t)w * ld;
     live = 0;
+    window = 1;
+    deferred_window_close(c);
     if (lean && !(fused && small_on_host())) {
         const int e0 = restore_fills();
         if (e0) return e0;
@@ -404,6 +412,7 @@
 
 int Module::lift(PhaseTimer& tm, const double* Qs_host, int64_t S1, double atol) {
     PhaseScope phase{tm, SDPSR_T_IRRED, false};
+    deferred_window_close(c);
     double* qs = (double*)ctx_buf(c, "cm_qsmall", (size_t)w * S1 * 8);
     double* Qhat = (double*)ctx_buf(c, "bd_qhat", (size_t)n * S1 * 8);
     if (!qs || !Qhat) return SDPSR_OUT_OF_MEMORY;
diff --git a/sdpsymmetryreduction.jl_amd/csrc/ctx.cpp b/sdpsymmetryreduction.jl_amd/csrc/ctx.cpp
--- a/sdpsymmetryreduction.jl_amd/csrc/ctx.cpp
+++ b/sdpsymmetryreduction.jl_amd/csrc/ctx.cpp
@@ -26,6 +26,7 @@
     if (nm == "adm_symflag") c->symflag_zero = false;
     if (nm == "bd_qhat" || nm == "bd_qrm") c->bd_qrm_current = false;
     if (b.p) {
+        flush_deferred_tail(c);
         ctx_sync_stream(c, c->stream);
         hipFree(b.p);
         b.p = nullptr;
@@ -48,6 +49,9 @@
 
 
 namespace sdpsr {
+uint64_t steady_ns() {
+    return (uint64_t)std::chrono::duration_cast<std::chrono::nanoseconds>(std::chrono::steady_clock::now().time_since_epoch()).count();
+}
 void* ctx_pinned(sdpsr_ctx* c, size_t bytes) {
     if (c->pinned_bytes >= bytes) return c->pinned;
     ctx_sync_stream(c, c->stream);
@@ -99,6 +103,7 @@
 constexpr size_t H2D_SLOT = 32 * 1024;
 constexpr int H2D_SLOTS = 32;
 int h2d_sync(sdpsr_ctx* c, void* dev, const void* host, size_t bytes) {
+    deferred_window_close(c);
     c->h2d_bytes += bytes;
     if (bytes <= H2D_SLOT) {
         if (!c->h2d_ring && hipHostMalloc(&c->h2d_ring, H2D_SLOT * H2D_SLOTS, hipHostMallocDefault) != hipSuccess) {
diff --git a/sdpsymmetryreduction.jl_amd/csrc/loop.cpp b/sdpsymmetryreduction.jl_amd/csrc/loop.cpp
--- a/sdpsymmetryreduction.jl_amd/csrc/loop.cpp
+++ b/sdpsymmetryreduction.jl_amd/csrc/loop.cpp
@@ -140,7 +140,10 @@
                square_check_supports(n, current, 2, T) && !(c->opts.flags & SDPSR_FLAG_SQUARE_EVERY_VERDICT) &&
                (proj_dead || r == 0 || current <= (int64_t)verify_lds_cap());
     }
-    int check_round(const SigSource& qj, uint64_t key2, Verdict* v) {
+    bool checks_deferrable() const {
+        return c->allow_deferred_verdict && c->pinned_small != nullptr && !tm.enabled && !(c->opts.flags & SDPSR_FLAG_CHECKS_IN_LOOP);
+    }
+    int check_round(const SigSource& qj, uint64_t key2, bool tail, Verdict* v) {
         SquareCheck q;
         q.n = n, q.d = current, q.G = 2, q.T = T;
         void* ws = ctx_buf(c, "adm_sqcheck", square_check_ws_bytes(n, current, 2, T));
@@ -154,11 +157,29 @@
         q.key[0] = key2, q.key[1] = next_key(c);
         q.Lp = lab.Lp, q.Lp8 = lab.shadow(), q.first_idx = first, q.Lfull = lab.full_from_gather();
         q.flag[0] = hv, q.flag[1] = hv2;
-        *(volatile uint32_t*)hv = 0u;
-        *(volatile uint32_t*)hv2 = 0u;
-        launch_square_check_ref_and_pass(s, q);
-        if (qj.kind == SIG_JOINT_I32 && r >= 1) launch_verify_projection(s, qj, current, first, hv);
-        launch_square_check_verdict(s, q);
+        const bool proj_verify = qj.kind == SIG_JOINT_I32 && r >= 1;
+        if (tail && !defer) return ctx_fail(c, SDPSR_BAD_STATE, "admissible_subspace: check segment asked for where the verdicts are read in the loop");
+        if (tail) {
+            *(volatile uint32_t*)hv = DEFERRED_NEVER_RAN;
+            *(volatile uint32_t*)hv2 = DEFERRED_NEVER_RAN;
+            launch_square_check_ref_and_pass(s, q);
+            DeferredTail& t = c->deferred_tail;
+            if (t.next == t.count) t.next = t.count = 0;
+            if (t.count >= DEFERRED_SEGMENTS) return ctx_fail(c, SDPSR_BAD_STATE, "admissible_subspace: no room for the round's check segment");
+            DeferredSegment& g = t.seg[t.count++] = DeferredSegment{};
+            g.kind = DEFERRED_CHECK, g.q = qj, g.n = n, g.d = current, g.first = first, g.flag = hv;
+            g.Lp = lab.Lp, g.Lp8 = lab.shadow();
+            g.proj_coef = !proj_dead, g.partial = partial, g.coef = coef, g.nblk = nblk;
+            g.proj_verify = proj_verify;
+            g.verdict = true, g.sq = q;
+            ++c->check_stats.registered;
+        } else {
+            *(volatile uint32_t*)hv = 0u;
+            *(volatile uint32_t*)hv2 = 0u;
+            launch_square_check_ref_and_pass(s, q);
+            if (proj_verify) launch_verify_projection(s, qj, current, first, hv);
+            launch_square_check_verdict(s, q);
+        }
         c->squares_launched += 2, ++c->squares_speculative, ++c->square_checks;
         if (defer) {
             c->deferred_verdict = true;
@@ -198,6 +219,7 @@
             launch_square(true, next_key(c), Xs, Cs, current, true, true);
             DeferredTail& t = c->deferred_tail;
             t.ld = ld, t.d = current, t.T = T, t.zero_flag = zero_flag, t.first = first;
+            t.seg[0] = t.seg[1] = DeferredSegment{};
             t.seg[0].X = (const int8_t*)Xp, t.seg[0].C = (int32_t*)Cp, t.seg[0].q = qv, t.seg[0].vref = vref, t.seg[0].flag = hv, t.seg[0].speculative = false;
             t.seg[1].X = Xs, t.seg[1].C = Cs, t.seg[1].q = qj, t.seg[1].vref = vref2, t.seg[1].flag = hv2, t.seg[1].speculative = true;
             t.seg[1].q.kind = SIG_CHAN_I32, t.seg[1].q.C = Cs;
@@ -240,28 +262,32 @@
         int st = SDPSR_OK;
         const bool jl = lab.packed();
         if (!jl) lab.need_full();
+        const bool defer_checks = checks_deferrable() && check_applies(false, jl);
+        if (!defer_checks) flush_deferred_tail(c);
         if (!proj_dead && it >= 2 && it <= 4 && r >= 1 && jl && c->first_idx_labels == lab.Lp && current >= 1 &&
             current <= (int64_t)refine_first_cap() && !(c->opts.flags & SDPSR_FLAG_ALWAYS_PROJECT)) {
             st = check_projection_dead();
             if (st) return st;
         }
-        if (!proj_dead) launch_proj_coef_lower(s, n, r, dU, lab.current(jl), jl ? 1 : 0, key, partial, nblk, coef, lab.shadow(jl));
+        if (!proj_dead && !defer_checks) launch_proj_coef_lower(s, n, r, dU, lab.current(jl), jl ? 1 : 0, key, partial, nblk, coef, lab.shadow(jl));
         tm.end();
         int64_t dj = current;
         bool confirming = false;
         for (;;) {
-            flush_deferred_tail(c);
+            if (confirming) flush_deferred_tail(c);
             tm.begin(SDPSR_T_SQUARE);
             const uint64_t key2 = next_key(c);
             const bool jl2 = lab.packed();
             const SigSource qj = joint_source(jl2);
             const bool check = check_applies(confirming, jl2);
+            if (defer_checks && !confirming && !check)
+                return ctx_fail(c, SDPSR_BAD_STATE, "admissible_subspace: the round that was to carry the dot products is not a checked round");
             const bool tail = !check && tail_applies(qj, confirming, jl2);
             if (!check) launch_square(jl2, key2, Xp, Cp, current, confirming && verify_applies(confirming, jl2), tail);
             tm.end();
             tm.begin(SDPSR_T_REFINE);
             Verdict v;
-            st = check ? check_round(qj, key2, &v) : verify_round(qj, confirming, jl2, tail, &v);
+            st = check ? check_round(qj, key2, defer_checks && !confirming, &v) : verify_round(qj, confirming, jl2, tail, &v);
             if (st) return st;
             if (v.unchanged) dj = current;
             else if (!(st = initial_guess_settled())) st = lab.refine_packed(qj, &dj);
@@ -321,6 +347,7 @@
     int separate_iteration(int64_t* d_out) {
         int st = SDPSR_OK;
         double* probe_host = nullptr;
+        flush_deferred_tail(c);
         const bool plab = packed_proj && lab.packed();
         if (!plab) lab.need_full();
         if (packed_proj) {
@@ -384,7 +411,20 @@
                 ++c->label_narrowings;
             }
         }
-        if (guess && launch_verify_pair(s, n, dCL, dX0, lab.Lp, guess->d0, guess->first, c->pinned_small + PINNED_SMALL_DEFERRED_INITIAL.first, Lp8)) {
+        bool pair_registered = false;
+        if (guess && checks_deferrable() && !(c->opts.flags & SDPSR_FLAG_SQUARE_EVERY_VERDICT) && n < (int64_t(1) << 31) && guess->d0 >= 1 &&
+            guess->d0 <= (int64_t)verify_lds_cap()) {
+            flush_deferred_tail(c);
+            DeferredTail& t = c->deferred_tail;
+            DeferredSegment& g = t.seg[0] = DeferredSegment{};
+            g.kind = DEFERRED_CHECK, g.pair = true, g.n = n, g.a = dCL, g.b = dX0, g.Lp = lab.Lp, g.Lp8 = Lp8, g.d = guess->d0, g.first = guess->first;
+            g.flag = c->pinned_small + PINNED_SMALL_DEFERRED_INITIAL.first;
+            *(volatile uint32_t*)g.flag = DEFERRED_NEVER_RAN;
+            t.next = 0, t.count = 1;
+            ++c->check_stats.registered;
+            pair_registered = true;
+        }
+        if (guess && (pair_registered || launch_verify_pair(s, n, dCL, dX0, lab.Lp, guess->d0, guess->first, c->pinned_small + PINNED_SMALL_DEFERRED_INITIAL.first, Lp8))) {
             c->initial_guess_pending = true;
             ++c->initial_guesses;
             HIP_TRY(c, hipGetLastError());
@@ -398,6 +438,7 @@
     }
     int initial_guess_settled() {
         if (!c->initial_guess_pending) return SDPSR_OK;
+        flush_deferred_tail(c);
         HIP_TRY(c, ctx_sync_stream(c, s));
         HIP_TRY(c, hipGetLastError());
         if (initial_guess_violated(c) != 0) return STATUS_REPEAT_REDUCTION;
@@ -422,10 +463,24 @@
 }
 
 namespace sdpsr {
-void flush_deferred_tail(sdpsr_ctx* c, int max_segments) {
+void flush_deferred_tail(sdpsr_ctx* c, int max_segments, bool in_ride) {
     DeferredTail& t = c->deferred_tail;
+    if (!in_ride && t.next < t.count) deferred_window_close(c);
     for (; max_segments > 0 && t.next < t.count; --max_segments, ++t.next) {
         const DeferredSegment& g = t.seg[t.next];
+        if (g.kind == DEFERRED_CHECK) {
+            if (g.pair) {
+                launch_verify_pair(c->stream, g.n, g.a, g.b, g.Lp, g.d, g.first, g.flag, g.Lp8);
+            } else {
+                *(volatile uint32_t*)g.sq.flag[0] = 0u;
+                *(volatile uint32_t*)g.sq.flag[1] = 0u;
+                if (g.proj_coef) launch_proj_coef_lower(c->stream, g.n, g.q.r, g.q.U, g.Lp, 1, g.q.key, g.partial, g.nblk, g.coef, g.Lp8);
+                if (g.proj_verify) launch_verify_projection(c->stream, g.q, g.d, g.first, g.flag);
+                if (g.verdict) launch_square_check_verdict(c->stream, g.sq);
+            }
+            ++(in_ride ? c->check_stats.in_ride : c->check_stats.outside_ride);
+            continue;
+        }
         launch_gemm_tn_i8_sym(c->stream, t.ld, t.ld, g.X, t.ld, g.C, t.ld, t.T, t.ld * t.ld, t.ld * t.ld, t.zero_flag, c->num_cus, c->opts.square_kernel);
         ++c->squares_launched;
         if (g.speculative) ++c->squares_speculative;
diff --git a/sdpsymmetryreduction.jl_amd/csrc/prof/prof.cpp b/sdpsymmetryreduction.jl_amd/csrc/prof/prof.cpp
--- a/sdpsymmetryreduction.jl_amd/csrc/prof/prof.cpp
+++ b/sdpsymmetryreduction.jl_amd/csrc/prof/prof.cpp
@@ -354,6 +354,16 @@
     const sdpsr_ctx* ci = restart == 0 ? c : c->batch_children[restart - 1];
     out[0] = ci->square_checks;
     out[1] = ci->square_check_fallbacks;
+    return SDPSR_OK;
+}
+
+extern "C" int sdpsr_profile_deferred_checks(sdpsr_ctx* c, int32_t restart, uint64_t* out) {
+    CHECK_CTX(c);
+    if (!out || restart < 0 || restart > (int32_t)c->batch_children.size()) return ctx_fail(c, SDPSR_BAD_ARGUMENT, "bad arguments");
+    const DeferredCheckStats& t = (restart == 0 ? c : c->batch_children[restart - 1])->check_stats;
+    out[0] = t.registered, out[1] = t.in_ride, out[2] = t.outside_ride;
+    out[3] = t.window_ns[0], out[4] = t.window_count[0], out[5] = t.window_ns[1], out[6] = t.window_count[1];
+    out[7] = t.voided[0], out[8] = t.voided[1], out[9] = t.voided[2];
     return SDPSR_OK;
 }
 
diff --git a/sdpsymmetryreduction.jl_amd/csrc/reduce.cpp b/sdpsymmetryreduction.jl_amd/csrc/reduce.cpp
--- a/sdpsymmetryreduction.jl_amd/csrc/reduce.cpp
+++ b/sdpsymmetryreduction.jl_amd/csrc/reduce.cpp
@@ -34,12 +34,17 @@
     c->initial_guess_pending = false;
     struct DropTail {
         sdpsr_ctx* c;
-        ~DropTail() { c->deferred_tail.count = c->deferred_tail.next = 0; }
+        ~DropTail() {
+            c->deferred_tail.count = c->deferred_tail.next = 0;
+            c->check_stats.window_open = -1;
+        }
     } drop_tail{c};
+    c->check_stats.window_open = -1;
     auto repeat_without_guesses = [&](uint32_t dv, uint32_t dv_spec, uint32_t dv_init) -> int {
         c->predict_closed = false;
         c->initial_record = InitialRecord{};
         if (dv_init != 0) ++c->initial_guesses_violated;
+        c->check_stats.voided[0] = dv, c->check_stats.voided[1] = dv_spec, c->check_stats.voided[2] = dv_init;
         if (dbg_on())
             fprintf(stderr, "[sdpsr] jordan_reduce: %s%s%s (deferred verdicts: verify %u, speculative %u, initial partition %u): reduction repeated\n",
                     dv_init != 0 ? "the initial partition was not the recorded one" : "", dv_init != 0 && (dv != 0 || dv_spec != 0) ? "; " : "",
diff --git a/sdpsymmetryreduction.jl_amd/csrc/sdpsr_internal.h b/sdpsymmetryreduction.jl_amd/csrc/sdpsr_internal.h
--- a/sdpsymmetryreduction.jl_amd/csrc/sdpsr_internal.h
+++ b/sdpsymmetryreduction.jl_amd/csrc/sdpsr_internal.h
@@ -38,13 +38,45 @@
     const uint8_t* L8 = nullptr;
 };
 
+constexpr int SQUARE_CHECK_MAX_CLASSES = 255;
+constexpr int64_t SQUARE_CHECK_MAX_ORDER = 1 << 15;
+struct SquareCheck {
+    int64_t n = 0, d = 0;
+    int G = 0, T = 0;
+    uint64_t key[2] = {0, 0};
+    const uint32_t* Lp = nullptr;
+    const uint8_t* Lp8 = nullptr;
+    const uint32_t* first_idx = nullptr;
+    uint32_t* Lfull = nullptr;
+    uint32_t* flag[2] = {nullptr, nullptr};
+    int32_t *c = nullptr, *part_x = nullptr;
+    int64_t *part_c = nullptr, *y = nullptr, *w = nullptr;
+    uint64_t* esum = nullptr;
+    uint32_t* bits = nullptr;
+};
+
+enum { DEFERRED_SQUARE = 0, DEFERRED_CHECK = 1 };
 struct DeferredSegment {
+    int kind = DEFERRED_SQUARE;
     const int8_t* X = nullptr;
     int32_t* C = nullptr;
     SigSource q;
     void* vref = nullptr;
     uint32_t* flag = nullptr;
     bool speculative = false;
+    bool pair = false;
+    const double *a = nullptr, *b = nullptr;
+    const uint32_t* Lp = nullptr;
+    const uint8_t* Lp8 = nullptr;
+    int64_t n = 0, d = 0;
+    const uint32_t* first = nullptr;
+    bool proj_coef = false;
+    double* partial = nullptr;
+    double* coef = nullptr;
+    int nblk = 0;
+    bool proj_verify = false;
+    bool verdict = false;
+    SquareCheck sq;
 };
 constexpr int DEFERRED_SEGMENTS = 2;
 struct DeferredTail {
@@ -54,6 +86,13 @@
     int T = 0;
     const uint32_t* zero_flag = nullptr;
     const uint32_t* first = nullptr;
+};
+struct DeferredCheckStats {
+    uint64_t registered = 0, in_ride = 0, outside_ride = 0;
+    uint64_t window_ns[2] = {0, 0}, window_count[2] = {0, 0};
+    int window_open = -1;
+    uint64_t window_t0 = 0;
+    uint32_t voided[3] = {0, 0, 0};
 };
 constexpr uint32_t DEFERRED_NEVER_RAN = 0xDEFE44EDu;
 struct InitialRecord {
@@ -125,6 +164,7 @@
     bool allow_deferred_verdict = false;
     bool deferred_verdict = false;
     sdpsr::DeferredTail deferred_tail;
+    sdpsr::DeferredCheckStats check_stats;
     sdpsr::InitialRecord initial_record;
     bool initial_guess_pending = false;
     uint64_t initial_guesses = 0, initial_guesses_violated = 0;
@@ -294,29 +334,21 @@
 bool launch_verify_pair(hipStream_t s, int64_t n, const double* a, const double* b, const uint32_t* Lp, int64_t d, const uint32_t* first_idx,
                         uint32_t* flag, const uint8_t* Lp8 = nullptr);
 bool launch_verify_projection(hipStream_t s, const SigSource& q, int64_t d, const uint32_t* first_idx, uint32_t* flag);
-constexpr int SQUARE_CHECK_MAX_CLASSES = 255;
-constexpr int64_t SQUARE_CHECK_MAX_ORDER = 1 << 15;
-struct SquareCheck {
-    int64_t n = 0, d = 0;
-    int G = 0, T = 0;
-    uint64_t key[2] = {0, 0};
-    const uint32_t* Lp = nullptr;
-    const uint8_t* Lp8 = nullptr;
-    const uint32_t* first_idx = nullptr;
-    uint32_t* Lfull = nullptr;
-    uint32_t* flag[2] = {nullptr, nullptr};
-    int32_t *c = nullptr, *part_x = nullptr;
-    int64_t *part_c = nullptr, *y = nullptr, *w = nullptr;
-    uint64_t* esum = nullptr;
-    uint32_t* bits = nullptr;
-};
 bool square_check_supports(int64_t n, int64_t d, int G, int T);
 size_t square_check_ws_bytes(int64_t n, int64_t d, int G, int T);
 size_t square_check_ws_carve(SquareCheck& q, void* ws, size_t gap = 0);
 void launch_square_check_ref_and_pass(hipStream_t s, const SquareCheck& q);
 void launch_square_check_verdict(hipStream_t s, const SquareCheck& q);
-void flush_deferred_tail(sdpsr_ctx* c, int max_segments = DEFERRED_SEGMENTS);
+void flush_deferred_tail(sdpsr_ctx* c, int max_segments = DEFERRED_SEGMENTS, bool in_ride = false);
 inline bool deferred_tail_pending(const sdpsr_ctx* c) { return c->deferred_tail.next < c->deferred_tail.count; }
+uint64_t steady_ns();
+inline void deferred_window_open(sdpsr_ctx* c, int which) { c->check_stats.window_open = which, c->check_stats.window_t0 = steady_ns(); }
+inline void deferred_window_close(sdpsr_ctx* c) {
+    DeferredCheckStats& t = c->check_stats;
+    if (t.window_open < 0) return;
+    t.window_ns[t.window_open] += steady_ns() - t.window_t0, ++t.window_count[t.window_open];
+    t.window_open = -1;
+}
 void launch_report_stamp(hipStream_t s, uint32_t* host_word, uint32_t seq);
 
 size_t refine_bucketed_workspace_bytes(int64_t len);
```

After: 2330 (median of 6 runs). +14.5%, better.
